# mmaker/c-lwe-snarks

Hardware: AMD Instinct MI355X
Metric: snark_proofs_per_sec (higher is better)
Workload: dtype u32 limbs (704-bit integers mod 2^704) + AES-256 bytes; int8 digits on the matrix cores, int32 accumulation (exact)

## Files before the change

c-lwe-snarks_amd/__init__.py:

```python
from __future__ import annotations

import ctypes
import os
from dataclasses import dataclass

import numpy as np

_HERE = os.path.dirname(os.path.abspath(__file__))
LIB_PATH = os.environ.get("MFHIP_LIB") or os.path.join(_HERE, "libmfhip.so")
P = 0xFFFFFFFB


class MfhError(RuntimeError):
    pass


@dataclass(frozen=True)
class Params:

    n: int = 1470
    logq: int = 736
    d: int = 1 << 15
    m: int = 21845

    @property
    def L(self):
        return (self.logq + 63) // 64

    @property
    def K(self):
        return self.logq // 64

    @property
    def lanes(self):
        return (64 * self.K + 55) // 56

    @property
    def ctb(self):
        return self.logq // 8

    @property
    def ctr_ct(self):
        return self.ctb * self.n

    @property
    def ctr_s(self):
        return 0

    @property
    def ctr_as(self):
        return self.ctr_ct * self.d

    @property
    def ctr_bt(self):
        return 2 * self.ctr_ct * self.d

    @property
    def ctr_bv(self):
        return 2 * self.ctr_ct * self.d + self.ctr_ct

    @property
    def ct_limbs(self):
        return (self.n + 1) * self.L


DEBUG = Params(d=256, m=64)
DEFAULT = Params()


class _CParams(ctypes.Structure):
    _fields_ = [("n", ctypes.c_uint32), ("logq", ctypes.c_uint32), ("d", ctypes.c_uint32), ("m", ctypes.c_uint32)]


_lib = None

EXPORTS = [
    "mfh_ctx_create", "mfh_ctx_destroy", "mfh_set_stream", "mfh_sync", "mfh_scrub_staging", "mfh_last_error", "mfh_set_seed",
    "mfh_keystream", "mfh_sample_rows", "mfh_ct_add", "mfh_ct_mul_ui", "mfh_ct_addmul_ui", "mfh_eval_rows",
    "mfh_encrypt_rows", "mfh_decrypt", "mfh_ct_smudge", "mfh_ssp_upload", "mfh_witness_poly", "mfh_version",
    "mfh_workspace_bytes", "mfh_last_kernel_ms", "mfh_set_timing", "mfh_set_overlap", "mfh_eval_rows_multi", "mfh_prove_batch", "mfh_crs_mm_image_bytes", "mfh_crs_expand_mm", "mfh_crs_set_resident_mm", "mfh_witness_poly_multi", "mfh_witness_poly_mm", "mfh_poly_h_multi", "mfh_poly_mul", "mfh_poly_add", "mfh_poly_prepare_t",
    "mfh_ssp_prepare", "mfh_poly_h", "mfh_setup_messages", "mfh_setup", "mfh_setup_image", "mfh_crs_image_set_b", "mfh_prove",
    "mfh_prove_partial", "mfh_prove_finish", "mfh_ct_to_lanes", "mfh_ct_from_lanes", "mfh_lanes_per_value", "mfh_digest128", "mfh_timing_drain", "mfh_timing_busy_ms", "mfh_timing_work_rows", "mfh_set_batch_image", "mfh_set_batch_slabs", "mfh_set_expand_path", "mfh_set_encrypt_path", "mfh_set_batch_launch", "mfh_set_batch_bw", "mfh_set_mm_chunk_rows", "mfh_set_mm_pack", "mfh_set_poly_exact", "mfh_poly_exact_fallbacks", "mfh_poly_exact_points", "mfh_set_poly_exact_points", "mfh_set_mm_stream", "mfh_add_dotp", "mfh_set_encrypt_chunks", "mfh_set_witness_per", "mfh_set_eval_path", "mfh_set_decrypt_path", "mfh_decrypt_rows",
    "mfh_crs_mm_share_bytes", "mfh_crs_expand_mm_share", "mfh_crs_set_resident_mm_share", "mfh_batch_chain", "mfh_batch_witness_cols", "mfh_batch_chain_from_w", "mfh_witness_poly_mm_cols", "mfh_prove_batch_partial", "mfh_prove_batch_finish",
    "mfh_resident_row_bytes", "mfh_crs_expand", "mfh_eval_rows_resident", "mfh_crs_set_resident",
    "mfh_witness_lanes", "mfh_witness_from_lanes", "mfh_prove_partial_w", "mfh_verify",
    "mfh_ssp_set_prg", "mfh_ssp_prg_make_t", "mfh_ssp_prg_fill",
    "mfh_resident_share_rows", "mfh_crs_expand_share", "mfh_crs_set_resident_share", "mfh_crs_set_resident_prefix",
    "mfh_prove_batch_supergroup", "mfh_prove_batch_stream_wait", "mfh_set_mm_width",
    "mfh_setup_public", "mfh_prove_public", "mfh_prove_batch_public", "mfh_vk_derive", "mfh_verify_public",
    "mfh_ssp_from_rows", "mfh_ssp_set_rows", "mfh_ssp_rows_fill", "mfh_ssp_rows_violations", "mfh_circuit_create", "mfh_circuit_destroy", "mfh_circuit_assign",
    "mfh_circuit_create_global", "mfh_circuit_create_ex", "mfh_circuit_create_out", "mfh_circuit_create_sum",
    "mfh_merkle_create", "mfh_merkle_destroy", "mfh_merkle_set_leaves", "mfh_merkle_root", "mfh_merkle_nodes", "mfh_merkle_paths",
    "mfh_sha256_records", "mfh_merkle_set_records", "mfh_merkle_update_rows",
]


def load_library():
    global _lib
    if _lib is not None:
        return _lib
    if not os.path.exists(LIB_PATH):
        raise MfhError(f"{LIB_PATH} is missing: run `python -c 'import __graft_entry__ as g; g.build()'` "
                       "(hipcc --offload-arch=gfx950).  There is no CPU fallback.")
    lib = ctypes.CDLL(LIB_PATH)
    vp, u64, sz, i32, u32 = ctypes.c_void_p, ctypes.c_uint64, ctypes.c_size_t, ctypes.c_int, ctypes.c_uint32
    sig = {
        "mfh_ctx_create": (i32, [ctypes.POINTER(vp), i32, ctypes.POINTER(_CParams)]),
        "mfh_ctx_destroy": (None, [vp]),
        "mfh_set_stream": (i32, [vp, vp]),
        "mfh_sync": (i32, [vp]),
        "mfh_scrub_staging": (i32, [vp]),
        "mfh_last_error": (ctypes.c_char_p, [vp]),
        "mfh_set_seed": (i32, [vp, ctypes.c_char_p]),
        "mfh_keystream": (i32, [vp, u64, vp, sz]),
        "mfh_sample_rows": (i32, [vp, u64, sz, vp]),
        "mfh_ct_add": (i32, [vp, vp, vp, vp, sz]),
        "mfh_ct_mul_ui": (i32, [vp, vp, vp, u32, sz]),
        "mfh_ct_addmul_ui": (i32, [vp, vp, vp, u32, sz]),
        "mfh_eval_rows": (i32, [vp, u64, sz, vp, vp, vp, vp, vp, i32]),
        "mfh_encrypt_rows": (i32, [vp, u64, sz, vp, vp, vp, vp]),
        "mfh_decrypt": (i32, [vp, vp, vp, sz, vp]),
        "mfh_ct_smudge": (i32, [vp, vp, sz, ctypes.c_char_p, sz, ctypes.c_char_p]),
        "mfh_ssp_upload": (i32, [vp, vp, vp, sz, sz]),
        "mfh_witness_poly": (i32, [vp, vp, ctypes.c_char_p, u32, vp]),
        "mfh_version": (ctypes.c_char_p, []),
        "mfh_workspace_bytes": (sz, [vp]),
        "mfh_last_kernel_ms": (ctypes.c_float, [vp, ctypes.c_char_p]),
        "mfh_set_timing": (i32, [vp, i32]),
        "mfh_set_overlap": (i32, [vp, i32]),
        "mfh_eval_rows_multi": (i32, [vp, u64, sz, vp, vp, u32, u32, vp, i32]),
        "mfh_poly_h_multi": (i32, [vp, vp, vp, u32]),
        "mfh_witness_poly_mm": (i32, [vp, vp, u32, ctypes.c_char_p, sz, vp, vp]),
        "mfh_witness_poly_multi": (i32, [vp, vp, u32, ctypes.c_char_p, sz, vp, vp]),
        "mfh_crs_mm_image_bytes": (sz, [vp]),
        "mfh_crs_expand_mm": (i32, [vp, vp, vp]),
        "mfh_crs_set_resident_mm": (i32, [vp, vp]),
        "mfh_prove_batch": (i32, [vp, vp, vp, u32, ctypes.c_char_p, sz, vp, ctypes.c_char_p, sz, ctypes.c_char_p, vp]),
        "mfh_prove_batch_supergroup": (u32, [vp]),
        "mfh_set_mm_width": (i32, [vp, u32, i32]),
        "mfh_prove_batch_stream_wait": (i32, [vp, u32, vp]),
        "mfh_poly_mul": (i32, [vp, vp, sz, vp, sz, vp]),
        "mfh_poly_add": (i32, [vp, vp, vp, sz, vp]),
        "mfh_poly_prepare_t": (i32, [vp, vp]),
        "mfh_ssp_prepare": (i32, [vp, vp]),
        "mfh_poly_h": (i32, [vp, vp, vp]),
        "mfh_setup_messages": (i32, [vp, vp, u32, u32, u32, vp]),
        "mfh_setup": (i32, [vp, vp, u32, u32, u32, vp, vp, vp]),
        "mfh_setup_image": (i32, [vp, vp, u32, u32, u32, vp, vp, vp, vp]),
        "mfh_prove": (i32, [vp, vp, vp, ctypes.c_char_p, u32, ctypes.c_char_p, sz, ctypes.c_char_p, vp]),
        "mfh_prove_partial": (i32, [vp, vp, vp, ctypes.c_char_p, u32, u32, u32, vp]),
        "mfh_prove_finish": (i32, [vp, vp, ctypes.c_char_p, sz, ctypes.c_char_p]),
        "mfh_lanes_per_value": (u32, [vp]),
        "mfh_digest128": (i32, [vp, vp, sz, vp]),
        "mfh_ct_to_lanes": (i32, [vp, vp, sz, vp]),
        "mfh_ct_from_lanes": (i32, [vp, vp, sz, vp]),
        "mfh_add_dotp": (i32, [vp, vp, vp, vp, sz]),
        "mfh_crs_set_resident_prefix": (i32, [vp, vp, sz]),
        "mfh_resident_share_rows": (sz, [vp, u32, u32]),
        "mfh_crs_expand_share": (i32, [vp, vp, u32, u32, vp]),
        "mfh_crs_set_resident_share": (i32, [vp, vp, u32, u32]),
        "mfh_ssp_set_prg": (i32, [vp, u64, vp]),
        "mfh_ssp_prg_make_t": (i32, [vp, u64, ctypes.c_char_p, vp]),
        "mfh_ssp_prg_fill": (i32, [vp, u64, sz, sz, vp]),
        "mfh_verify": (i32, [vp, vp, u32, u32, u32, vp, vp, sz, vp]),
        "mfh_witness_lanes": (i32, [vp, vp, ctypes.c_char_p, u32, u32, vp]),
        "mfh_witness_from_lanes": (i32, [vp, vp, vp, u32, vp]),
        "mfh_prove_partial_w": (i32, [vp, vp, vp, ctypes.c_char_p, u32, u32, u32, vp, vp]),
        "mfh_resident_row_bytes": (sz, [vp]),
        "mfh_crs_expand": (i32, [vp, u64, sz, vp, vp]),
        "mfh_crs_image_set_b": (i32, [vp, sz, sz, vp, vp]),
        "mfh_eval_rows_resident": (i32, [vp, vp, sz, sz, vp, vp, vp, vp, i32]),
        "mfh_crs_set_resident": (i32, [vp, vp]),
        "mfh_timing_drain": (i32, [vp, ctypes.c_char_p, ctypes.POINTER(u64), ctypes.POINTER(ctypes.c_double), ctypes.POINTER(u64),
                                   ctypes.POINTER(ctypes.c_float)]),
        "mfh_timing_busy_ms": (ctypes.c_double, [vp]),
        "mfh_timing_work_rows": (u64, [vp]),
        "mfh_set_batch_image": (i32, [vp, i32]),
        "mfh_set_mm_chunk_rows": (i32, [vp, u32]),
        "mfh_set_mm_pack": (i32, [vp, i32]),
        "mfh_set_poly_exact": (i32, [vp, i32]),
        "mfh_poly_exact_fallbacks": (ctypes.c_long, [vp]),
        "mfh_poly_exact_points": (i32, [vp, ctypes.POINTER(u32)]),
        "mfh_set_poly_exact_points": (i32, [vp, ctypes.POINTER(u32)]),
        "mfh_set_mm_stream": (i32, [vp, i32, i32, i32, u32]),
        "mfh_set_batch_launch": (i32, [vp, u32, i32]),
        "mfh_set_batch_bw": (i32, [vp, i32]),
        "mfh_set_encrypt_path": (i32, [vp, i32]),
        "mfh_set_expand_path": (i32, [vp, i32]),
        "mfh_set_batch_slabs": (i32, [vp, u32]),
        "mfh_set_encrypt_chunks": (i32, [vp, u32]),
        "mfh_set_eval_path": (i32, [vp, i32]),
        "mfh_set_decrypt_path": (i32, [vp, i32]),
        "mfh_decrypt_rows": (i32, [vp, u64, sz, vp, vp, vp]),
        "mfh_set_witness_per": (i32, [vp, u32]),
        "mfh_crs_mm_share_bytes": (sz, [vp, u32, u32]),
        "mfh_crs_expand_mm_share": (i32, [vp, vp, u32, u32, vp]),
        "mfh_crs_set_resident_mm_share": (i32, [vp, vp, u32, u32]),
        "mfh_batch_chain": (i32, [vp, vp, u32, ctypes.c_char_p, sz, vp, vp, vp, vp]),
        "mfh_batch_witness_cols": (i32, [vp, vp, u32, ctypes.c_char_p, sz, vp, u32, u32, vp, sz]),
        "mfh_batch_chain_from_w": (i32, [vp, vp, u32, vp, vp, vp]),
        "mfh_witness_poly_mm_cols": (i32, [vp, vp, u32, ctypes.c_char_p, sz, vp, u32, u32, vp, sz]),
        "mfh_prove_batch_partial": (i32, [vp, vp, u32, u32, u32, ctypes.c_char_p, sz, vp, vp, vp, sz, vp]),
        "mfh_prove_batch_finish": (i32, [vp, vp, u32, vp, ctypes.c_char_p, sz, ctypes.c_char_p, vp]),
        "mfh_setup_public": (i32, [vp, vp, u32, u32, u32, u32, vp, vp, vp, vp]),
        "mfh_prove_public": (i32, [vp, vp, vp, u32, ctypes.c_char_p, u32, ctypes.c_char_p, sz, ctypes.c_char_p, vp]),
        "mfh_prove_batch_public": (i32, [vp, vp, vp, u32, u32, ctypes.c_char_p, sz, vp, ctypes.c_char_p, sz, ctypes.c_char_p, vp]),
        "mfh_vk_derive": (i32, [vp, vp, u32, u32, vp]),
        "mfh_verify_public": (i32, [vp, vp, u32, u32, u32, vp, vp, ctypes.c_char_p, sz, sz, vp]),
        "mfh_ssp_from_rows": (i32, [vp, u32, vp, vp, vp, vp]),
        "mfh_ssp_set_rows": (i32, [vp, u32, vp, vp, vp, u32]),
        "mfh_ssp_rows_fill": (i32, [vp, sz, sz, vp]),
        "mfh_ssp_rows_violations": (i32, [vp, u32, vp, sz, vp, vp]),
        "mfh_circuit_create": (i32, [vp, u32, u32, vp, u32, vp, ctypes.POINTER(vp)]),
        "mfh_circuit_create_global": (i32, [vp, u32, u32, vp, u32, vp, ctypes.POINTER(vp)]),
        "mfh_circuit_create_ex": (i32, [vp, u32, u32, vp, u32, vp, u32, vp, u32, ctypes.POINTER(vp)]),
        "mfh_circuit_create_out": (i32, [vp, u32, u32, vp, u32, vp, u32, vp, u32, vp, u32, ctypes.POINTER(vp)]),
        "mfh_circuit_create_sum": (i32, [vp, u32, u32, vp, u32, vp, u32, vp, u32, vp, u32, vp, u32, ctypes.POINTER(vp)]),
        "mfh_circuit_destroy": (None, [vp]),
        "mfh_circuit_assign": (i32, [vp, vp, u32, vp, sz, vp, sz, vp]),
        "mfh_merkle_create": (i32, [vp, u32, ctypes.POINTER(vp)]),
        "mfh_merkle_destroy": (None, [vp]),
        "mfh_merkle_set_leaves": (i32, [vp, vp, u32, u32, vp]),
        "mfh_merkle_root": (i32, [vp, vp, vp]),
        "mfh_merkle_nodes": (i32, [vp, u32, ctypes.POINTER(vp)]),
        "mfh_merkle_paths": (i32, [vp, vp, u32, vp, vp, sz]),
        "mfh_sha256_records": (i32, [vp, vp, sz, u32, u32, vp]),
        "mfh_merkle_set_records": (i32, [vp, vp, u32, u32, vp, sz, u32]),
        "mfh_merkle_update_rows": (i32, [vp, vp, u32, vp, vp, vp, sz, vp]),
    }
    for name, (res, args) in sig.items():
        fn = getattr(lib, name)
        fn.restype = res
        fn.argtypes = args
    _lib = lib
    return lib


def rows_to_csr(rows):
    if isinstance(rows, tuple) and len(rows) == 3 and all(isinstance(a, np.ndarray) for a in rows):
        row_ptr, wire, coef = rows
    else:
        lens = [len(r) for r in rows]
        row_ptr = np.zeros(len(lens) + 1, dtype=np.int64)
        np.cumsum(lens, out=row_ptr[1:])
        flat = [(int(w), int(a) % P) for r in rows for (w, a) in r]
        wire = np.array([w for w, _ in flat], dtype=np.int64)
        coef = np.array([a for _, a in flat], dtype=np.int64)
    if len(row_ptr) == 0 or min(np.min(row_ptr), np.min(wire, initial=0), np.min(coef, initial=0)) < 0:
        raise MfhError("rows: row_ptr needs nrows + 1 entries, and no entry may be negative")
    if max(np.max(row_ptr), np.max(wire, initial=0), np.max(coef, initial=0)) > 0xFFFFFFFF:
        raise MfhError("rows: entries must fit 32 bits")
    return tuple(np.ascontiguousarray(a, dtype=np.uint32) for a in (row_ptr, wire, coef))


def _ptr(t):
    return ctypes.c_void_p(t.data_ptr()) if t is not None else ctypes.c_void_p(0)


CIRCUIT_MAX_WIRES = 32767
CIRCUIT_GLOBAL = 1


class CircuitProgram:

    def __init__(self, ctx, nin, ngates, handle, state="lds", extended=False, outputs=0, sums=False):
        self._ctx, self.nin, self.ngates, self._h, self.state, self.extended, self.outputs = ctx, nin, ngates, handle, state, extended, outputs
        self.sums = sums

    def close(self):
        if self._h:
            self._ctx.lib.mfh_circuit_destroy(self._h)
            self._h = ctypes.c_void_p()

    def __del__(self):
        try:
            self.close()
        except Exception:
            pass


class _DeviceBytes:

    def __init__(self, ptr, n, owner):
        self.owner = owner
        self.__cuda_array_interface__ = {"shape": (n, 32), "typestr": "|u1", "data": (ptr, False), "version": 2, "strides": None}


def _records(ctx, records, who):
    if isinstance(records, ctx.torch.Tensor):
        t = records
        if t.dtype != ctx.torch.uint8 or t.device != ctx.device or t.dim() != 2:
            raise MfhError(f"{who}: a device tensor of records is uint8 [n, length] on the context's device")
        n, length = int(t.shape[0]), int(t.shape[1])
        if (length > 1 and t.stride(1) != 1) or (n > 1 and t.stride(0) < length):
            raise MfhError(f"{who}: a device tensor of records has stride(1) == 1 and stride(0) >= length")
        return t, (int(t.stride(0)) if n > 1 else length), length, n, False
    a = np.asarray(records)
    if a.dtype != np.uint8 or a.ndim != 2:
        raise MfhError(f"{who}: records are a uint8 array [n, length]")
    n, length = a.shape
    return ctx.to_device(a).reshape(n, length), length, length, n, True


class MerkleTree:

    def __init__(self, ctx, depth, handle):
        self._ctx, self.depth, self._h = ctx, depth, handle
        self.nin = 256 + 256 * (depth + 1) + depth
        self._keep = []

    def close(self):
        if self._h:
            self._ctx.lib.mfh_merkle_destroy(self._h)
            self._h = ctypes.c_void_p()
            self._keep = []

    def __del__(self):
        try:
            self.close()
        except Exception:
            pass

    def set_leaves(self, first, leaves):
        c = self._ctx
        if isinstance(leaves, c.torch.Tensor):
            t = leaves
            if t.dtype != c.torch.uint8 or t.device != c.device or not t.is_contiguous():
                raise MfhError("set_leaves: a device tensor of leaves is contiguous uint8 on the context's device")
        else:
            a = np.frombuffer(leaves, dtype=np.uint8) if isinstance(leaves, (bytes, bytearray, memoryview)) else np.asarray(leaves)
            if a.dtype != np.uint8:
                raise MfhError("set_leaves: leaves are bytes or uint8")
            t = c.to_device(a)
            self._keep.append(t)
        if t.numel() % 32:
            raise MfhError("set_leaves: leaves are 32 bytes each")
        c._chk(c.lib.mfh_merkle_set_leaves(c._h, self._h, int(first), t.numel() // 32, _ptr(t)))

    def set_records(self, first, records):
        c = self._ctx
        t, stride, length, n, host = _records(c, records, "set_records")
        if host:
            self._keep.append(t)
        c._chk(c.lib.mfh_merkle_set_records(c._h, self._h, int(first), n, _ptr(t), stride, length))

    def root(self):
        out = (ctypes.c_uint8 * 32)()
        self._ctx._chk(self._ctx.lib.mfh_merkle_root(self._ctx._h, self._h, out))
        self._keep = []
        return bytes(out)

    def nodes(self, level):
        p = ctypes.c_void_p()
        self._ctx._chk(self._ctx.lib.mfh_merkle_nodes(self._h, int(level), ctypes.byref(p)))
# ... 15 lines not shown
        if isinstance(records, np.ndarray):
            rec = records
        else:
            rec = [np.frombuffer(bytes(r), dtype=np.uint8) for r in records]
            if len({len(r) for r in rec}) > 1:
                raise MfhError("record_rows: the records are of one length")
            rec = np.stack(rec) if rec else np.zeros((0, 0), dtype=np.uint8)
        if rec.dtype != np.uint8 or rec.ndim != 2 or len(rec) != len(paths):
            raise MfhError("record_rows: records are uint8 [nb, length], one per index")
        return np.concatenate([np.zeros((len(paths), 32), dtype=np.uint8), rec, paths[:, 64:]], axis=1)

    def record_bits(self, records, indices):
        rows = self.record_rows(records, indices)
        length = rows.shape[1] - 32 - 32 * self.depth - (self.depth + 7) // 8
        return np.unpackbits(rows, axis=1, bitorder="little")[:, : 256 + 8 * length + 257 * self.depth]

    def path_bits(self, indices):
        return np.unpackbits(self.path_rows(indices), axis=1, bitorder="little")[:, : self.nin]

    def update_rows(self, indices, new_leaves, roots=False):
        c = self._ctx
        idx = np.ascontiguousarray(indices, dtype=np.int64).reshape(-1)
        if len(idx) and (idx.min() < 0 or idx.max() > 0xFFFFFFFF):
            raise MfhError("update_rows: indices are in [0, 2^depth)")
        idx = idx.astype(np.uint32)
        if isinstance(new_leaves, c.torch.Tensor):
            t = new_leaves
            if t.dtype != c.torch.uint8 or t.device != c.device or not t.is_contiguous():
                raise MfhError("update_rows: a device tensor of leaves is contiguous uint8 on the context's device")
            if t.data_ptr() & 15:
                t = t.clone()
        else:
            a = np.frombuffer(new_leaves, dtype=np.uint8) if isinstance(new_leaves, (bytes, bytearray, memoryview)) else np.asarray(new_leaves)
            if a.dtype != np.uint8:
                raise MfhError("update_rows: leaves are bytes or uint8")
            t = c.to_device(a)
        if t.numel() != 32 * len(idx):
            raise MfhError("update_rows: one leaf of 32 bytes per index")
        rows = np.zeros((len(idx), 128 + 32 * self.depth + (self.depth + 7) // 8), dtype=np.uint8)
        r = np.zeros((len(idx) + 1, 32), dtype=np.uint8) if roots else None
        c._chk(c.lib.mfh_merkle_update_rows(c._h, self._h, len(idx), ctypes.c_void_p(idx.ctypes.data), _ptr(t) if len(idx) else None,
                                            ctypes.c_void_p(rows.ctypes.data), rows.shape[1], ctypes.c_void_p(r.ctypes.data) if roots else None))
        self._keep = []
        if roots and not len(idx):
            r[0] = np.frombuffer(self.root(), dtype=np.uint8)
        return (rows, r) if roots else rows

    def update_bits(self, indices, new_leaves, roots=False):
        out = self.update_rows(indices, new_leaves, roots)
        bits = np.unpackbits(out[0] if roots else out, axis=1, bitorder="little")[:, : 1024 + 257 * self.depth]
        return (bits, out[1]) if roots else bits


class Context:

    def __init__(self, params: Params = DEFAULT, device: int = 0, own_stream: bool = False):
        import torch

        if not torch.cuda.is_available():
            raise MfhError("no HIP device visible: the MI355X path has no CPU fallback")
        self.torch = torch
        self.lib = load_library()
        self.params = params
        self.device = torch.device("cuda", device)
        self._h = ctypes.c_void_p()
        cp = _CParams(params.n, params.logq, params.d, params.m)
        rc = self.lib.mfh_ctx_create(ctypes.byref(self._h), device, ctypes.byref(cp))
        if rc != 0:
            raise MfhError(f"mfh_ctx_create failed ({rc})")
        if not own_stream:
            self.set_stream(torch.cuda.current_stream(self.device))

    def close(self):
        if self._h:
            self.lib.mfh_ctx_destroy(self._h)
            self._h = ctypes.c_void_p()

    def __del__(self):
        try:
            self.close()
        except Exception:
            pass

    def _chk(self, rc):
        if rc != 0:
            raise MfhError(f"libmfhip error {rc}: {self.lib.mfh_last_error(self._h).decode()}")

    def empty(self, nbytes):
        return self.torch.empty(int(nbytes), dtype=self.torch.uint8, device=self.device)

    def zeros(self, nbytes):
        return self.torch.zeros(int(nbytes), dtype=self.torch.uint8, device=self.device)

    def to_device(self, arr):
        a = np.ascontiguousarray(arr)
        if not a.flags.writeable:
            import warnings

            with warnings.catch_warnings():
                warnings.simplefilter("ignore", UserWarning)
                return self.torch.from_numpy(a.view(np.uint8).reshape(-1)).to(self.device)
        return self.torch.from_numpy(a.view(np.uint8).reshape(-1)).to(self.device)

    def to_host(self, t, dtype=np.uint8):
        return t.cpu().numpy().view(dtype)

    def sync(self):
        self._chk(self.lib.mfh_sync(self._h))

    def set_stream(self, stream):
        self._chk(self.lib.mfh_set_stream(self._h, ctypes.c_void_p(stream.cuda_stream if stream is not None else 0)))

    def scrub_staging(self):
        rc = self.lib.mfh_scrub_staging(self._h)
        self._chk(rc)
        return rc

    def workspace_bytes(self):
        return int(self.lib.mfh_workspace_bytes(self._h))

    def set_timing(self, on=True):
        self._chk(self.lib.mfh_set_timing(self._h, 1 if on else 0))

    def set_overlap(self, mode=1):
        self._chk(self.lib.mfh_set_overlap(self._h, int(mode)))

    def set_batch_image(self, on=True):
        self._chk(self.lib.mfh_set_batch_image(self._h, 1 if on else 0))

    def set_batch_slabs(self, nslabs=0):
        self._chk(self.lib.mfh_set_batch_slabs(self._h, int(nslabs)))

    def set_expand_path(self, path=0):
        self._chk(self.lib.mfh_set_expand_path(self._h, int(path)))

    def set_encrypt_path(self, path=0):
        self._chk(self.lib.mfh_set_encrypt_path(self._h, int(path)))

    def set_eval_path(self, path=0):
        self._chk(self.lib.mfh_set_eval_path(self._h, int(path)))

    def set_encrypt_chunks(self, chunks=0):
        self._chk(self.lib.mfh_set_encrypt_chunks(self._h, int(chunks)))

    def set_witness_per(self, statements=0):
        self._chk(self.lib.mfh_set_witness_per(self._h, int(statements)))

    def set_batch_launch(self, groups_per_launch=4, merge_regions=True):
        self._chk(self.lib.mfh_set_batch_launch(self._h, int(groups_per_launch), 1 if merge_regions else 0))

    def set_batch_bw(self, merged=True):
        self._chk(self.lib.mfh_set_batch_bw(self._h, 1 if merged else 0))

    def set_mm_stream(self, map=0, persistent=False, sync_mode=0, spin_max=64):
        self._chk(self.lib.mfh_set_mm_stream(self._h, int(map), int(persistent), int(sync_mode), int(spin_max)))

    def set_mm_width(self, per_xcd=32, early_chain=False):
        self._chk(self.lib.mfh_set_mm_width(self._h, int(per_xcd), 1 if early_chain else 0))

    def set_mm_pack(self, on=True):
        self._chk(self.lib.mfh_set_mm_pack(self._h, 1 if on else 0))

    def set_poly_exact(self, mode=1):
        self._chk(self.lib.mfh_set_poly_exact(self._h, int(mode)))

    def poly_exact_fallbacks(self):
        return int(self.lib.mfh_poly_exact_fallbacks(self._h))

    def exact_points(self):
        out = (ctypes.c_uint32 * 4)()
        self._chk(self.lib.mfh_poly_exact_points(self._h, out))
        return [int(x) for x in out]

    def set_exact_points(self, pts):
        if pts is None:
            self._chk(self.lib.mfh_set_poly_exact_points(self._h, None))
            return
        pts = [int(x) for x in pts]
        if len(pts) != 4 or not all(0 <= x < 2**32 for x in pts):
            raise MfhError(f"set_exact_points: four uint32 values, got {pts!r}")
        self._chk(self.lib.mfh_set_poly_exact_points(self._h, (ctypes.c_uint32 * 4)(*pts)))

    def set_mm_chunk_rows(self, rows=0):
        self._chk(self.lib.mfh_set_mm_chunk_rows(self._h, int(rows)))

    def timing_drain(self, which):
        n, rows, ms, last = ctypes.c_uint64(), ctypes.c_uint64(), ctypes.c_double(), ctypes.c_float()
        self._chk(self.lib.mfh_timing_drain(self._h, which.encode(), ctypes.byref(n), ctypes.byref(ms), ctypes.byref(rows), ctypes.byref(last)))
        return n.value, ms.value, rows.value

    def timing_busy_ms(self):
        return float(self.lib.mfh_timing_busy_ms(self._h))

    def timing_work_rows(self):
        return int(self.lib.mfh_timing_work_rows(self._h))

    def last_kernel_ms(self, which):
        return float(self.lib.mfh_last_kernel_ms(self._h, which.encode()))

    def set_seed(self, seed: bytes):
        assert len(seed) == 40
        self._chk(self.lib.mfh_set_seed(self._h, bytes(seed)))

    def keystream(self, off, nbytes, out=None):
        out = self.empty(nbytes) if out is None else out
        self._chk(self.lib.mfh_keystream(self._h, off, _ptr(out), nbytes))
        return out

    def sample_rows(self, off, nrows):
        p = self.params
        out = self.empty(nrows * p.n * p.L * 8)
        self._chk(self.lib.mfh_sample_rows(self._h, off, nrows, _ptr(out)))
        return out

    def ct_add(self, a, b, count=1, out=None):
        out = self.empty(a.numel()) if out is None else out
        self._chk(self.lib.mfh_ct_add(self._h, _ptr(out), _ptr(a), _ptr(b), count))
        return out

    def ct_mul_ui(self, a, x, count=1, out=None):
        out = self.empty(a.numel()) if out is None else out
        self._chk(self.lib.mfh_ct_mul_ui(self._h, _ptr(out), _ptr(a), x, count))
        return out

    def ct_addmul_ui(self, rop, a, x, count=1):
        self._chk(self.lib.mfh_ct_addmul_ui(self._h, _ptr(rop), _ptr(a), x, count))
        return rop

    def eval_rows(self, off, nrows, c8, coeff0, coeff1=None, rop0=None, rop1=None, accumulate=False):
        p = self.params
        if rop0 is None:
            rop0 = self.empty(p.ct_limbs * 8)
        if coeff1 is not None and rop1 is None:
            rop1 = self.empty(p.ct_limbs * 8)
        self._chk(self.lib.mfh_eval_rows(self._h, off, nrows, _ptr(c8), _ptr(coeff0), _ptr(coeff1), _ptr(rop0), _ptr(rop1),
                                         1 if accumulate else 0))
        return rop0, rop1

    def eval_rows_multi(self, off, nrows, c8, coeffs, nvec, out=None, accumulate=False, coeff_bytes=4):
        out = self.empty(nvec * self.params.ct_limbs * 8) if out is None else out
        self._chk(self.lib.mfh_eval_rows_multi(self._h, off, nrows, _ptr(c8), _ptr(coeffs), nvec, coeff_bytes, _ptr(out), 1 if accumulate else 0))
        return out

    def encrypt_rows(self, off, nrows, sk, msg, err, out=None):
        p = self.params
        out = self.empty(nrows * p.ctb) if out is None else out
        self._chk(self.lib.mfh_encrypt_rows(self._h, off, nrows, _ptr(sk), _ptr(msg), _ptr(err), _ptr(out)))
        return out

    def decrypt(self, sk, cts, count, out=None):
        out = self.empty(4 * count) if out is None else out
        self._chk(self.lib.mfh_decrypt(self._h, _ptr(sk), _ptr(cts), count, _ptr(out)))
        return out

    def set_decrypt_path(self, path=0):
        self._chk(self.lib.mfh_set_decrypt_path(self._h, int(path)))

    def decrypt_rows(self, off, nrows, sk, c8, out=None):
        out = self.empty(4 * nrows) if out is None else out
        self._chk(self.lib.mfh_decrypt_rows(self._h, off, nrows, _ptr(sk), _ptr(c8), _ptr(out)))
        return out

    def ct_smudge(self, cts, count, mag: bytes, maglen, sign: bytes):
        self._chk(self.lib.mfh_ct_smudge(self._h, _ptr(cts), count, bytes(mag), maglen, bytes(sign)))
        return cts

    def ssp_upload(self, ssp_host_u64: np.ndarray, d_ssp=None, first_slot=0, nslots=None):
        p = self.params
        nslots = p.m + 3 if nslots is None else nslots
        if d_ssp is None:
            d_ssp = self.empty((p.m + 3) * p.d * 4)
        a = np.ascontiguousarray(ssp_host_u64)
        self._chk(self.lib.mfh_ssp_upload(self._h, ctypes.c_void_p(a.ctypes.data), _ptr(d_ssp), first_slot, nslots))
        return d_ssp

    def ssp_from_rows(self, rows, d_ssp=None):
        p = self.params
        row_ptr, wire, coef = rows_to_csr(rows)
        if d_ssp is None:
            d_ssp = self.empty((p.m + 3) * p.d * 4)
        self._chk(self.lib.mfh_ssp_from_rows(self._h, len(row_ptr) - 1, ctypes.c_void_p(row_ptr.ctypes.data), ctypes.c_void_p(wire.ctypes.data),
                                             ctypes.c_void_p(coef.ctypes.data), _ptr(d_ssp)))
        return d_ssp

    def ssp_set_rows(self, rows, lu_max=0):
        if rows is None:
            self._chk(self.lib.mfh_ssp_set_rows(self._h, 0, None, None, None, 0))
            return
        row_ptr, wire, coef = rows_to_csr(rows)
        self._chk(self.lib.mfh_ssp_set_rows(self._h, len(row_ptr) - 1, ctypes.c_void_p(row_ptr.ctypes.data), ctypes.c_void_p(wire.ctypes.data),
                                            ctypes.c_void_p(coef.ctypes.data), int(lu_max)))

    def ssp_rows_fill(self, first_slot, nslots):
        out = self.empty(max(nslots, 1) * self.params.d * 4)
        self._chk(self.lib.mfh_ssp_rows_fill(self._h, first_slot, nslots, _ptr(out)))
        return out

    def ssp_rows_violations(self, witness_bits_list):
        nb = len(witness_bits_list)
        count, first = np.zeros(nb, dtype=np.uint32), np.full(nb, 0xFFFFFFFF, dtype=np.uint32)
        bits, stride = self._pack_bits(witness_bits_list)
        self._chk(self.lib.mfh_ssp_rows_violations(self._h, nb, bits if nb else None, stride, ctypes.c_void_p(count.ctypes.data), ctypes.c_void_p(first.ctypes.data)))
        return count, first

    def circuit_load(self, compiled, state="lds"):
        if state not in ("lds", "global", "auto"):
            raise MfhError(f"circuit_load: state must be 'lds', 'global' or 'auto', got {state!r}")
        gates = np.ascontiguousarray(compiled.gates, dtype=np.uint32).reshape(-1, 3)
        asserts = np.ascontiguousarray(compiled.asserts, dtype=np.uint32).reshape(-1, 2)
        program = np.ascontiguousarray(getattr(compiled, "program", np.zeros((0, 4))), dtype=np.uint32).reshape(-1, 4)
        equal = np.ascontiguousarray(getattr(compiled, "equal", np.zeros((0, 2))), dtype=np.uint32).reshape(-1, 2)
        outputs = np.ascontiguousarray(getattr(compiled, "outputs", np.zeros((0, 2))), dtype=np.uint32).reshape(-1, 2)
        terms = np.ascontiguousarray(getattr(compiled, "terms", np.zeros((0, 2))), dtype=np.uint32).reshape(-1, 2)
        sums = bool((program[:, 0] == 8).any())
        extended = len(equal) > 0 or len(outputs) > 0 or bool((program[:, 0] > 3).any())
        nin = compiled.nwires - len(gates)
        if state == "auto":
            state = "lds" if compiled.nwires <= CIRCUIT_MAX_WIRES else "global"
        h = ctypes.c_void_p()

        def arr(x):
            return ctypes.c_void_p(x.ctypes.data)

        flags = CIRCUIT_GLOBAL if state == "global" else 0
        ex = [self._h, nin, len(program), arr(program), len(asserts), arr(asserts), len(equal), arr(equal)]
        if sums:
            self._chk(self.lib.mfh_circuit_create_sum(*ex, len(outputs), arr(outputs), len(terms), arr(terms), flags, ctypes.byref(h)))
        elif len(outputs):
            self._chk(self.lib.mfh_circuit_create_out(*ex, len(outputs), arr(outputs), flags, ctypes.byref(h)))
        elif extended:
            self._chk(self.lib.mfh_circuit_create_ex(*ex, flags, ctypes.byref(h)))
        else:
            create = self.lib.mfh_circuit_create if state == "lds" else self.lib.mfh_circuit_create_global
            self._chk(create(self._h, nin, len(gates), arr(gates), len(asserts), arr(asserts), ctypes.byref(h)))
        return CircuitProgram(self, nin, len(gates), h, state, extended, len(outputs), sums)

    def circuit_assign(self, prog, bits):
        bits = np.asarray(bits, dtype=np.uint8)
        if bits.ndim != 2 or bits.shape[1] != prog.nin:
            raise MfhError(f"circuit_assign: bits must be [nb, {prog.nin}] (public then private bits), got {bits.shape}")
        nb = bits.shape[0]
        packed = np.ascontiguousarray(np.packbits(bits & 1, axis=1, bitorder="little"))
        stride = (self.params.m + 7) // 8
        witness = np.zeros((nb, stride), dtype=np.uint8)
        holds = np.zeros(nb, dtype=np.uint8)
        self._chk(self.lib.mfh_circuit_assign(self._h, prog._h, nb, ctypes.c_void_p(packed.ctypes.data), packed.shape[1], ctypes.c_void_p(witness.ctypes.data),
                                              stride, ctypes.c_void_p(holds.ctypes.data)))
        return witness, holds.astype(bool)

    def sha256_records(self, records):
        t, stride, length, n, host = _records(self, records, "sha256_records")
        out = self.torch.empty((n, 32), dtype=self.torch.uint8, device=self.device)
        self._chk(self.lib.mfh_sha256_records(self._h, _ptr(t), stride, length, n, _ptr(out)))
        if host:
            self.sync()
        return out

    def merkle_tree(self, depth):
        h = ctypes.c_void_p()
        self._chk(self.lib.mfh_merkle_create(self._h, int(depth), ctypes.byref(h)))
        return MerkleTree(self, int(depth), h)

    def ssp_to_host_u64(self, d_ssp):
        p = self.params
        return self.to_host(d_ssp[: (p.m + 3) * p.d * 4], np.uint32).astype(np.uint64)

    def witness_poly(self, d_ssp, witness_bits: bytes, delta):
        out = self.empty(self.params.d * 4)
        self._chk(self.lib.mfh_witness_poly(self._h, _ptr(d_ssp), bytes(witness_bits), delta, _ptr(out)))
        return out

    def poly_mul(self, a, la, b, lb):
        out = self.empty((la + lb - 1) * 4)
        self._chk(self.lib.mfh_poly_mul(self._h, _ptr(a), la, _ptr(b), lb, _ptr(out)))
        return out

    def poly_add(self, a, b, count):
        out = self.empty(count * 4)
        self._chk(self.lib.mfh_poly_add(self._h, _ptr(a), _ptr(b), count, _ptr(out)))
        return out

    def ssp_prepare(self, d_ssp):
        self._chk(self.lib.mfh_ssp_prepare(self._h, _ptr(d_ssp)))

    def poly_prepare_t(self, d_t):
        self._chk(self.lib.mfh_poly_prepare_t(self._h, _ptr(d_t)))

    def poly_h(self, d_v):
        out = self.empty(self.params.d * 4)
        self._chk(self.lib.mfh_poly_h(self._h, _ptr(d_v), _ptr(out)))
        return out

    def poly_h_many(self, d_v, nb):
        out = self.empty(nb * self.params.d * 4)
        self._chk(self.lib.mfh_poly_h_multi(self._h, _ptr(d_v), _ptr(out), nb))
        return out

    def setup_messages(self, d_ssp, alpha, beta, s):
        p = self.params
        out = self.empty((2 * p.d + p.m) * 4)
        self._chk(self.lib.mfh_setup_messages(self._h, _ptr(d_ssp), alpha, beta, s, _ptr(out)))
        return out

    def setup(self, d_ssp, alpha, beta, s, d_sk, d_err, out=None):
        p = self.params
        out = self.empty((2 * p.d + p.m) * p.ctb) if out is None else out
        self._chk(self.lib.mfh_setup(self._h, _ptr(d_ssp), alpha, beta, s, _ptr(d_sk), _ptr(d_err), _ptr(out)))
        return out

    def setup_image(self, d_ssp, alpha, beta, s, d_sk, d_err, out=None, rows=None):
        p = self.params
        out = self.empty((2 * p.d + p.m) * p.ctb) if out is None else out
        rows = self.empty((2 * p.d + p.m) * self.resident_row_bytes()) if rows is None else rows
        self._chk(self.lib.mfh_setup_image(self._h, _ptr(d_ssp), alpha, beta, s, _ptr(d_sk), _ptr(d_err), _ptr(out), _ptr(rows)))
        return out, rows

    def prove(self, d_crs, d_ssp, witness_bits: bytes, delta, smudge_mag: bytes, smudge_sign: bytes, maglen=80, out=None):
        p = self.params
        out = self.empty(5 * p.ct_limbs * 8) if out is None else out
        assert len(smudge_mag) == 5 * maglen and len(smudge_sign) == 5
        self._chk(self.lib.mfh_prove(self._h, _ptr(d_crs), _ptr(d_ssp), bytes(witness_bits), delta, bytes(smudge_mag), maglen,
                                     bytes(smudge_sign), _ptr(out)))
        return out

    def crs_expand_mm(self, d_crs, out=None):
        out = self.empty(int(self.lib.mfh_crs_mm_image_bytes(self._h))) if out is None else out
        self._chk(self.lib.mfh_crs_expand_mm(self._h, _ptr(d_crs), _ptr(out)))
        return out

    def set_resident_mm(self, image):
        self._resident_mm = image
        self._chk(self.lib.mfh_crs_set_resident_mm(self._h, _ptr(image)))

    def witness_poly_many(self, d_ssp, witness_bits_list, deltas, mm=True):
        p = self.params
        nb = len(witness_bits_list)
        stride = (p.m + 6) // 8
        bits = b"".join(bytes(w[:stride]).ljust(stride, b"\0") for w in witness_bits_list)
        dl = (ctypes.c_uint32 * nb)(*[int(x) for x in deltas])
        out = self.empty(nb * p.d * 4)
        fn = self.lib.mfh_witness_poly_mm if mm else self.lib.mfh_witness_poly_multi
        self._chk(fn(self._h, _ptr(d_ssp), nb, bits, stride, ctypes.cast(dl, ctypes.c_void_p), _ptr(out)))
        return out

    def prove_batch(self, d_crs, d_ssp, witness_bits_list, deltas, smudge_mags, smudge_signs, maglen=80, out=None):
        p = self.params
        nb = len(witness_bits_list)
        stride = (p.m + 6) // 8
        bits = b"".join(bytes(w[:stride]).ljust(stride, b"\0") for w in witness_bits_list)
        dl = (ctypes.c_uint32 * nb)(*[int(x) for x in deltas])
        mags = b"".join(bytes(x) for x in smudge_mags)
        signs = b"".join(bytes(x) for x in smudge_signs)
        assert len(mags) == nb * 5 * maglen and len(signs) == nb * 5
        out = self.empty(nb * 5 * p.ct_limbs * 8) if out is None else out
        self._chk(self.lib.mfh_prove_batch(self._h, _ptr(d_crs), _ptr(d_ssp), nb, bits, stride, ctypes.cast(dl, ctypes.c_void_p), mags, maglen,
                                           signs, _ptr(out)))
        return out

    def prove_batch_supergroup(self):
        return int(self.lib.mfh_prove_batch_supergroup(self._h))

    def prove_batch_stream_wait(self, upto, stream):
        self._chk(self.lib.mfh_prove_batch_stream_wait(self._h, int(upto), ctypes.c_void_p(stream.cuda_stream)))

    def _pack_bits(self, witness_bits_list):
        stride = (self.params.m + 6) // 8
        return b"".join(bytes(w[:stride]).ljust(stride, b"\0") for w in witness_bits_list), stride

    def crs_expand_mm_share(self, d_crs, rank, world, out=None):
        out = self.empty(int(self.lib.mfh_crs_mm_share_bytes(self._h, rank, world))) if out is None else out
        self._chk(self.lib.mfh_crs_expand_mm_share(self._h, _ptr(d_crs), rank, world, _ptr(out)))
        return out

    def set_resident_mm_share(self, image, rank, world):
        self._resident_mm = image
        self._chk(self.lib.mfh_crs_set_resident_mm_share(self._h, _ptr(image), rank, world))

    def batch_chain(self, d_ssp, witness_bits_list, deltas, out=None):
        p = self.params
        nb = len(witness_bits_list)
        out = self.torch.empty((3, nb, p.d), dtype=self.torch.int32, device=self.device) if out is None else out
        if nb == 0:
            return out
        bits, stride = self._pack_bits(witness_bits_list)
        dl = (ctypes.c_uint32 * nb)(*[int(x) for x in deltas])
        self._chk(self.lib.mfh_batch_chain(self._h, _ptr(d_ssp), nb, bits, stride, ctypes.cast(dl, ctypes.c_void_p), _ptr(out[0]), _ptr(out[1]), _ptr(out[2])))
        return out

    def batch_witness_cols(self, d_ssp, witness_bits_list, deltas, col0, ncols, out=None):
        nb = len(witness_bits_list)
        out = self.torch.empty((nb, ncols), dtype=self.torch.int32, device=self.device) if out is None else out
        if nb == 0 or ncols == 0:
            return out
        bits, stride = self._pack_bits(witness_bits_list)
        dl = (ctypes.c_uint32 * nb)(*[int(x) for x in deltas])
        self._chk(self.lib.mfh_batch_witness_cols(self._h, _ptr(d_ssp), nb, bits, stride, ctypes.cast(dl, ctypes.c_void_p), int(col0), int(ncols), _ptr(out), int(ncols)))
        return out

    def batch_chain_from_w(self, d_ssp, whv):
        n = whv.shape[1]
        if n:
            self._chk(self.lib.mfh_batch_chain_from_w(self._h, _ptr(d_ssp), n, _ptr(whv[0]), _ptr(whv[1]), _ptr(whv[2])))
        return whv

    def prove_batch_partial(self, d_crs, rank, world, witness_bits_list, d_w, d_h, d_v, coef_stride, out=None):
        p = self.params
        nb = len(witness_bits_list)
        need = nb * 5 * p.ct_limbs * 8
        out = self.empty(need) if out is None else out
        if out.numel() * out.element_size() < need:
            raise MfhError(f"prove_batch_partial: `out` holds {out.numel() * out.element_size()} bytes, {nb} statements need {need}")
        bits, stride = self._pack_bits(witness_bits_list)
        self._chk(self.lib.mfh_prove_batch_partial(self._h, _ptr(d_crs), rank, world, nb, bits, stride, _ptr(d_w), _ptr(d_h), _ptr(d_v), int(coef_stride),
                                                   _ptr(out)))
        return out

    def prove_batch_finish(self, d_crs, deltas, smudge_mags, smudge_signs, d_proofs, maglen=80):
        nb = len(deltas)
        if nb == 0:
            return d_proofs
        dl = (ctypes.c_uint32 * nb)(*[int(x) for x in deltas])
        mags = b"".join(bytes(x) for x in smudge_mags)
        signs = b"".join(bytes(x) for x in smudge_signs)
        assert len(mags) == nb * 5 * maglen and len(signs) == nb * 5
        self._chk(self.lib.mfh_prove_batch_finish(self._h, _ptr(d_crs), nb, ctypes.cast(dl, ctypes.c_void_p), mags, maglen, signs, _ptr(d_proofs)))
        return d_proofs

    def prove_partial(self, d_crs, d_ssp, witness_bits: bytes, delta, rank, world, out=None):
        p = self.params
        out = self.empty(5 * p.ct_limbs * 8) if out is None else out
        self._chk(self.lib.mfh_prove_partial(self._h, _ptr(d_crs), _ptr(d_ssp), bytes(witness_bits), delta, rank, world, _ptr(out)))
        return out

    def prove_finish(self, d_proof, smudge_mag: bytes, smudge_sign: bytes, maglen=80):
        self._chk(self.lib.mfh_prove_finish(self._h, _ptr(d_proof), bytes(smudge_mag), maglen, bytes(smudge_sign)))
        return d_proof

    def digest128(self, d_buf, nbytes=None):
        h = (ctypes.c_uint64 * 2)()
        n = d_buf.numel() * d_buf.element_size() if nbytes is None else int(nbytes)
        self._chk(self.lib.mfh_digest128(self._h, _ptr(d_buf), n, ctypes.cast(h, ctypes.c_void_p)))
        return int(h[0]), int(h[1])

    def ct_to_lanes(self, d_cts, count, out=None):
        p = self.params
        out = self.torch.empty(count * (p.n + 1) * p.lanes, dtype=self.torch.int64, device=self.device) if out is None else out
        self._chk(self.lib.mfh_ct_to_lanes(self._h, _ptr(d_cts), count, _ptr(out)))
        return out

    def ct_from_lanes(self, d_lanes, count, out=None):
        p = self.params
        out = self.empty(count * p.ct_limbs * 8) if out is None else out
        self._chk(self.lib.mfh_ct_from_lanes(self._h, _ptr(d_lanes), count, _ptr(out)))
        return out

    def add_dotp(self, rop, a, b, length):
        self._chk(self.lib.mfh_add_dotp(self._h, _ptr(rop), _ptr(a), _ptr(b), length))
        return rop

    def resident_row_bytes(self):
        return int(self.lib.mfh_resident_row_bytes(self._h))

    def crs_expand(self, off, nrows, c8, out=None):
        out = self.empty(nrows * self.resident_row_bytes()) if out is None else out
        self._chk(self.lib.mfh_crs_expand(self._h, off, nrows, _ptr(c8), _ptr(out)))
        return out

    def crs_image_set_b(self, image, first_row, nrows, c8):
        self._chk(self.lib.mfh_crs_image_set_b(self._h, int(first_row), int(nrows), _ptr(c8), _ptr(image)))
        return image

    def eval_rows_resident(self, rows, first_row, nrows, coeff0, coeff1=None, rop0=None, rop1=None, accumulate=False):
        p = self.params
        if rop0 is None:
            rop0 = self.empty(p.ct_limbs * 8)
        if coeff1 is not None and rop1 is None:
            rop1 = self.empty(p.ct_limbs * 8)
        self._chk(self.lib.mfh_eval_rows_resident(self._h, _ptr(rows), first_row, nrows, _ptr(coeff0), _ptr(coeff1), _ptr(rop0), _ptr(rop1),
                                                  1 if accumulate else 0))
        return rop0, rop1

    def set_resident(self, rows):
        self._resident = rows
        self._chk(self.lib.mfh_crs_set_resident(self._h, _ptr(rows)))

    def witness_lanes(self, d_ssp, witness_bits: bytes, rank, world, out=None):
        out = self.torch.empty(self.params.d, dtype=self.torch.int64, device=self.device) if out is None else out
        self._chk(self.lib.mfh_witness_lanes(self._h, _ptr(d_ssp), bytes(witness_bits), rank, world, _ptr(out)))
        return out

    def prove_partial_w(self, d_crs, d_ssp, witness_bits: bytes, delta, rank, world, wlanes, out=None):
        p = self.params
        out = self.empty(5 * p.ct_limbs * 8) if out is None else out
        self._chk(self.lib.mfh_prove_partial_w(self._h, _ptr(d_crs), _ptr(d_ssp), bytes(witness_bits), delta, rank, world, _ptr(wlanes), _ptr(out)))
        return out

    def verify(self, d_ssp, alpha, beta, s, d_sk, d_proofs, count=1):
# ... 75 lines not shown
```

c-lwe-snarks_amd/csrc/ctx.hpp:

```cpp
#pragma once
#include <hip/hip_runtime.h>

#include <stdint.h>
#include <string.h>

#include <string>
#include <vector>

#include "aes_dev.hpp"
#include "mfhip.h"
#include "ssp_prg.hpp"

#define HIP_TRY(ctx, expr)                                                        \
  do {                                                                            \
    hipError_t e_ = (expr);                                                       \
    if (e_ != hipSuccess) {                                                       \
      (ctx)->err = std::string(#expr) + ": " + hipGetErrorString(e_);             \
      return MFH_EDEVICE;                                                         \
    }                                                                             \
  } while (0)

struct PolyState;
struct SspInterp;
struct SspRows;
struct RowsTree;

struct PinBuf {
  void *p = nullptr;
  size_t cap = 0;
  hipEvent_t ev = nullptr;
  bool pending = false;
  size_t used = 0;
};

struct DevBuf {
  void *p = nullptr;
  size_t cap = 0;
  template <class T> T *as() const { return static_cast<T *>(p); }
};

struct mfh_ctx {
  mfh_params P{};
  int device = 0;
  hipStream_t own_stream = nullptr;
  hipStream_t stream = nullptr;
  mf::AesKey key{};
  bool have_seed = false;
  uint32_t *d_t0 = nullptr;
  DevBuf ws;
  DevBuf ws2;
  int mm_ws_sel = 0;
  DevBuf ws3;
  std::vector<hipEvent_t> ev_cdone, ev_rdone, ev_wdone;
  std::vector<hipEvent_t> ev_round;
  std::vector<hipEvent_t> ev_sgdone;
  uint32_t last_batch_sg = 0, last_batch_n = 0;
  DevBuf wws;
  DevBuf lazy;
  uint32_t *lazy_cnt = nullptr;
  bool eval_dense = false;
  bool overlap = true;
  int overlap_mode = 1;
  hipStream_t side = nullptr, side2 = nullptr;
  hipEvent_t ev_fork = nullptr, ev_join = nullptr;
  hipEvent_t ev_chain = nullptr, ev_chain_done = nullptr;
  std::string err;
  bool timing = false;
  struct Timed {
    hipEvent_t e0, e1;
    int kind;
    uint64_t rows;
    uint64_t work;
    int sub;
  };
  std::vector<Timed> timed;
  double last_busy_ms = 0;
  uint64_t last_work_rows = 0;
  std::vector<hipEvent_t> ev_pool;
  PolyState *poly = nullptr;
  DevBuf aux;
  DevBuf d_msg;
  DevBuf d_prover;
  std::vector<uint32_t> h_cw;
  const uint8_t *mm_image = nullptr;
  uint32_t mm_rank = 0, mm_world = 1;
  uint64_t mm_off[3] = {0, 0, 0}, mm_rows[3] = {0, 0, 0};
  size_t mm_base[3] = {0, 0, 0};
  DevBuf ssp_frag;
  const uint32_t *ssp_frag_src = nullptr;
  SspInterp *interp = nullptr;
  DevBuf circ_io;
  DevBuf circ_state;
  DevBuf d_batch;
  DevBuf batch_img;
  int batch_image = 1;
  int mm_map = 1;
  bool mm_persist = true;
  bool mm_wave1 = false;
  uint32_t mm_sync_mode = 0, mm_spin = 64;
  uint32_t mm_width = 32;
  size_t early_ws_half = 0;
  bool batch_early_chain = false;
  uint32_t *mm_sync = nullptr;
  int poly_exact = 1;
  bool poly_pts_pinned = false;
  uint32_t poly_pts[4] = {0, 0, 0, 0};
  bool mm_pack = true;
  uint32_t mm_chunk_rows = 131071;
  int expand_path = 0;
  int enc_path = 0;
  uint32_t ncu = 256;
  int dec_path = 0;
  int eval_path = 0;
  uint32_t enc_chunks = 0;
  uint32_t witness_per = 0;
  uint32_t batch_slabs = 0;
  int batch_bw_merged = 1;
  int batch_merge = 1;
  uint32_t batch_ngl = 8;
  PinBuf pin_rows, pin_cw, pin_smudge;
  PinBuf pin_pub;
  DevBuf d_pub;
  PinBuf pin_wring[8];
  uint32_t pin_wnext = 0;
  hipEvent_t ev_sample = nullptr;
  DevBuf sample_tmp;
  void *uploader = nullptr;
  bool prg_on = false;
  uint64_t prg_seed = 0;
  const uint32_t *prg_t = nullptr;
  SspRows *rows = nullptr;
  RowsTree *rows_tree = nullptr;
  const uint32_t *rows_prefix = nullptr;
  uint32_t rows_lu_max = 0;
  const uint8_t *resident_rows = nullptr;
  uint64_t resident_nrows = ~0ull;
  bool resident_sharded = false;
  uint32_t res_rank = 0, res_world = 1;
};

struct Timer {
  mfh_ctx *c;
  mfh_ctx::Timed t{};
  bool on;
  Timer(mfh_ctx *c_, int kind, uint64_t rows, uint64_t work = 0, int sub = 0) : c(c_), on(c_->timing) {
    if (!on) return;
    auto get = [&]() {
      hipEvent_t e;
      if (!c->ev_pool.empty()) { e = c->ev_pool.back(); c->ev_pool.pop_back(); }
      else hipEventCreate(&e);
      return e;
    };
    t.e0 = get(); t.e1 = get(); t.kind = kind; t.rows = rows; t.work = work ? work : rows; t.sub = sub;
    hipEventRecord(t.e0, c->stream);
  }
  ~Timer() {
    if (!on) return;
    hipEventRecord(t.e1, c->stream);
    c->timed.push_back(t);
  }
};

inline void *pin_acquire(mfh_ctx *c, PinBuf &b, size_t bytes) {
  if (b.pending) { hipEventSynchronize(b.ev); b.pending = false; }
  if (bytes > b.cap) {
    if (b.p) hipHostFree(b.p);
    b.cap = (bytes + 4095) & ~(size_t)4095;
    if (hipHostMalloc(&b.p, b.cap, hipHostMallocDefault) != hipSuccess) { b.p = nullptr; b.cap = 0; c->err = "hipHostMalloc failed"; return nullptr; }
  }
  if (!b.ev) hipEventCreateWithFlags(&b.ev, hipEventDisableTiming);
  b.used = bytes;
  return b.p;
}
inline void pin_release(mfh_ctx *c, PinBuf &b) {
  hipEventRecord(b.ev, c->stream);
  b.pending = true;
}
inline void pin_scrub(PinBuf &b) {
  if (b.pending) { hipEventSynchronize(b.ev); b.pending = false; }
  if (b.p && b.used) {
    volatile unsigned char *q = (volatile unsigned char *)b.p;
    memset((void *)q, 0, b.used);
    __asm__ __volatile__("" : : "r"(b.p) : "memory");
  }
  b.used = 0;
}
inline void pin_free(PinBuf &b) {
  if (b.pending) hipEventSynchronize(b.ev);
  if (b.p) hipHostFree(b.p);
  if (b.ev) hipEventDestroy(b.ev);
  b = PinBuf();
}

enum class DevWait { stream, device };
inline void dev_free(DevBuf &b) {
  if (b.p) hipFree(b.p);
  b = DevBuf();
}
inline bool dev_alloc(DevBuf &b, size_t bytes) {
  if (hipMalloc(&b.p, bytes) != hipSuccess) {
    b = DevBuf();
    return false;
  }
  b.cap = bytes;
  return true;
}
inline int dev_reserve(mfh_ctx *c, DevBuf &b, size_t bytes, DevWait wait = DevWait::stream, size_t gran = 1) {
  if (bytes <= b.cap) return MFH_OK;
  if (b.p) {
    if (wait == DevWait::device) hipDeviceSynchronize();
    else hipStreamSynchronize(c->stream);
    dev_free(b);
  }
  if (!dev_alloc(b, (bytes + gran - 1) & ~(gran - 1))) {
    c->err = "hipMalloc(device scratch) failed";
    return MFH_ENOMEM;
  }
  return MFH_OK;
}
inline int batch_img_drop(mfh_ctx *c) {
  if (!c->batch_img.p) return MFH_OK;
  const hipError_t e = hipDeviceSynchronize();
  dev_free(c->batch_img);
  if (e != hipSuccess) {
    c->err = std::string("hipDeviceSynchronize(): ") + hipGetErrorString(e);
    return MFH_EDEVICE;
  }
  return MFH_OK;
}
inline int work_reserve(mfh_ctx *c, DevBuf &b, size_t bytes) { return dev_reserve(c, b, bytes, DevWait::stream, (size_t)1 << 20); }
inline int lazy_reserve(mfh_ctx *c, size_t bytes) {
  if (bytes + 256 <= c->lazy.cap || !bytes) return MFH_OK;
  bytes = ((bytes + 255) & ~(size_t)255) + 256;
  if (int rc = dev_reserve(c, c->lazy, bytes)) return rc;
  if (hipMemsetAsync(c->lazy.p, 0, bytes, c->stream) != hipSuccess) return MFH_EDEVICE;
  c->lazy_cnt = reinterpret_cast<uint32_t *>(c->lazy.as<uint8_t>() + bytes - 256);
  return MFH_OK;
}
inline int ws_reserve(mfh_ctx *c, size_t bytes) { return work_reserve(c, c->ws, bytes); }
inline int wws_reserve(mfh_ctx *c, size_t bytes) { return work_reserve(c, c->wws, bytes); }
inline int ws2_reserve(mfh_ctx *c, size_t bytes) { return work_reserve(c, c->ws2, bytes); }
inline int aux_reserve(mfh_ctx *c, size_t bytes) { return dev_reserve(c, c->aux, bytes); }

inline int ssp_src(mfh_ctx *c, const uint32_t *d_ssp, mf::SspSrc &src, bool rows_ok = false) {
  if (d_ssp) { src = mf::SspSrc{d_ssp, d_ssp, 0}; return MFH_OK; }
  if (c->rows_prefix) {
    if (!rows_ok) { c->err = "this entry point does not take the row SSP (mfh_ssp_set_rows): pass a dense d_ssp"; return MFH_EUNSUPPORTED; }
    src = mf::SspSrc{c->rows_prefix, c->rows_prefix, 0, c->rows_lu_max + 2};
    return MFH_OK;
  }
  if (!c->prg_on || !c->prg_t) { c->err = "d_ssp is NULL and no generator-defined SSP is registered (mfh_ssp_set_prg)"; return MFH_EINVAL; }
  src = mf::SspSrc{nullptr, c->prg_t, c->prg_seed};
  return MFH_OK;
}

void mfh_poly_destroy(mfh_ctx *c);
void ssp_interp_free(mfh_ctx *c);
void ssp_rows_free(mfh_ctx *c, bool tree);
int ssp_rows_check(mfh_ctx *c, const char *who, uint32_t nrows, const uint32_t *h_row_ptr, const uint32_t *h_wire, const uint32_t *h_coef);
int ssp_rows_tree(mfh_ctx *c, const char *who, const uint32_t *&d_t, const uint32_t *&h_w);
int ssp_rows_witness(mfh_ctx *c, uint32_t nstmt, const uint8_t *h_bits, size_t bits_stride, const uint32_t *h_delta, uint32_t *d_w, size_t w_stride);
int ssp_rows_msg_evals(mfh_ctx *c, uint32_t s, uint32_t beta, uint32_t *d_msg_evals);
inline bool ssp_is_rows(const mfh_ctx *c, const uint32_t *d_ssp) { return !d_ssp && c->rows_prefix; }
inline int ssp_rows_lu_check(mfh_ctx *c, const uint32_t *d_ssp, uint32_t lu) {
  if (ssp_is_rows(c, d_ssp) && lu > c->rows_lu_max) { c->err = "lu exceeds the lu_max the row SSP was registered with (mfh_ssp_set_rows)"; return MFH_EINVAL; }
  return MFH_OK;
}
extern "C" int mfh_witness_poly_mm(mfh_ctx *c, const uint32_t *d_ssp, uint32_t nstmt, const uint8_t *h_bits, size_t bits_stride, const uint32_t *h_delta,
                                   uint32_t *d_w);
extern "C" int mfh_witness_poly_mm_cols(mfh_ctx *c, const uint32_t *d_ssp, uint32_t nstmt, const uint8_t *h_bits, size_t bits_stride, const uint32_t *h_delta,
                                        uint32_t col0, uint32_t ncols, uint32_t *d_w, size_t w_stride);
extern "C" int mfh_poly_h_multi(mfh_ctx *c, const uint32_t *d_v, uint32_t *d_h, uint32_t nb);
int expand_mm_region(mfh_ctx *c, uint64_t off, uint32_t nrows, const uint8_t *c8, uint8_t *image);
int encrypt_rows_mm(mfh_ctx *c, uint64_t off, size_t nrows, const uint64_t *sk, const uint32_t *msg, const uint64_t *err, uint8_t *c8);
int decrypt_mm(mfh_ctx *c, const uint64_t *sk, const uint64_t *cts, size_t count, uint32_t *out);
int decrypt_rows_mm(mfh_ctx *c, uint64_t off, size_t nrows, const uint64_t *sk, const uint8_t *c8, uint32_t *out);

struct MmIo {
  const uint32_t *coef[2];
  uint32_t csplit;
  uint64_t *out[2];
  uint32_t osplit;
  uint64_t ostride;
  const uint8_t *bits;
  uint32_t bits_stride;
  int64_t *sc_zeroed;
  uint64_t cstride;
  uint32_t bits_row0;
  const uint64_t *add_ct;
  const uint32_t *add_scale;
  uint32_t sa_from1;
};
int eval_rows_multi_io(mfh_ctx *c, uint64_t off, size_t nrows, const uint8_t *d_c8, const MmIo &io, uint32_t nvec, uint32_t coeff_bytes, int accumulate);
int eval_rows_multi_io_set(mfh_ctx *c, uint64_t off, size_t nrows, const uint8_t *d_c8, const MmIo *ios, const uint32_t *nvecs, uint32_t ng,
                           uint32_t coeff_bytes);
struct MmRegion { uint64_t off; const uint8_t *c8; };
int eval_rows_multi_io_regions(mfh_ctx *c, const MmRegion *regs, uint32_t nreg, size_t nrows, const MmIo *ios, const uint32_t *nvecs, uint32_t ng,
                               uint32_t coeff_bytes, int accumulate);
bool mm_image_covers(const mfh_ctx *c, uint64_t off, size_t nrows);
struct MmsPlan {
  uint32_t ng, ngt, ND, nrows, nchunks, rpc, rpad, ntiles, mtiles;
  size_t cd_bytes, part_bytes;
  const uint8_t *img[2];
  int8_t *cd;
  int *part;
};
bool mms_plan(mfh_ctx *c, const MmRegion *regs, uint32_t nreg, size_t nrows, const MmIo *ios, const uint32_t *nvecs, uint32_t ng, uint32_t coeff_bytes,
              MmsPlan &P);
size_t mms_ws_bytes(const MmsPlan &P);
void mms_bind(MmsPlan &P, void *ws);
int mms_digits(mfh_ctx *c, const MmsPlan &P, const MmIo *ios, const uint32_t *nvecs);
int mms_stream(mfh_ctx *c, const MmsPlan &P);
int mms_finish(mfh_ctx *c, const MmsPlan &P, const MmIo *ios, const uint32_t *nvecs, int accumulate);
```

c-lwe-snarks_amd/csrc/mfhip.hip:

```cpp
#include <hip/hip_runtime.h>

#include <stdint.h>
#include <stdio.h>
#include <string.h>

#include <algorithm>
#include <string>
#include <thread>
#include <vector>

#include "aes_dev.hpp"
#include "mfhip.h"

using mf::AesKey;

template <int LOGQ>
struct PS {
  static constexpr int CTB = LOGQ / 8;
  static constexpr int EW = CTB / 4;
  static constexpr int L = (LOGQ + 63) / 64;
  static constexpr int K = LOGQ / 64;
  static constexpr int KW = 2 * K;
  static constexpr int TILE = LOGQ == 736 ? 512 : 256;
  static constexpr int ROWS = 2;
// ... 806 lines not shown
__global__ void k_ssp_reduce(const uint64_t *__restrict__ in, uint32_t *__restrict__ out, uint64_t ncoef) {
  for (uint64_t i = (uint64_t)blockIdx.x * blockDim.x + threadIdx.x; i < ncoef; i += (uint64_t)gridDim.x * blockDim.x)
    out[i] = (uint32_t)(in[i] % MFH_P);
}

extern "C" {

const char *mfh_version(void) { return "mfhip 0.1 (gfx950)"; }

int mfh_ctx_create(mfh_ctx **out, int device, const mfh_params *P) {
  if (!out || !P) return MFH_EINVAL;
  *out = nullptr;
  if (P->logq != 736 && P->logq != 1472) return MFH_EUNSUPPORTED;
  if (P->n == 0 || P->n > (1u << 20)) return MFH_EINVAL;
  int ndev = 0;
  if (hipGetDeviceCount(&ndev) != hipSuccess || ndev <= 0 || device < 0 || device >= ndev) return MFH_EDEVICE;
  if (hipSetDevice(device) != hipSuccess) return MFH_EDEVICE;
  mfh_ctx *c = new mfh_ctx();
  c->P = *P;
  c->device = device;
  {
    int ncu = 0;
    if (hipDeviceGetAttribute(&ncu, hipDeviceAttributeMultiprocessorCount, device) == hipSuccess && ncu > 0) c->ncu = (uint32_t)ncu;
  }
  if (hipStreamCreateWithFlags(&c->own_stream, hipStreamNonBlocking) != hipSuccess) {
    delete c;
    return MFH_EDEVICE;
  }
  c->stream = c->own_stream;
  uint32_t t0[512];
  mf::make_t0_le(t0);
  for (int a = 0; a < 256; a++) t0[256 + a] = (t0[a] << 24) | (t0[a] >> 8);
  if (hipMalloc(&c->d_t0, sizeof t0) != hipSuccess || hipMemcpy(c->d_t0, t0, sizeof t0, hipMemcpyHostToDevice) != hipSuccess) {
    mfh_ctx_destroy(c);
    return MFH_EDEVICE;
  }
  *out = c;
  return MFH_OK;
}

void mfh_ctx_destroy(mfh_ctx *c) {
  if (!c) return;
  hipSetDevice(c->device);
  if (c->stream) hipStreamSynchronize(c->stream);
  mfh_poly_destroy(c);
  ssp_interp_free(c);
  ssp_rows_free(c, true);
  upload_free(c);
  if (c->ev_sample) hipEventDestroy(c->ev_sample);
  pin_free(c->pin_rows);
  for (auto &b : c->pin_wring) pin_free(b);
  pin_free(c->pin_cw);
  pin_free(c->pin_smudge);
  pin_free(c->pin_pub);
  if (c->side) hipStreamSynchronize(c->side);
  if (c->mm_sync) hipFree(c->mm_sync);
  for (hipEvent_t e : c->ev_round) hipEventDestroy(e);
  for (hipEvent_t e : c->ev_sgdone) hipEventDestroy(e);
  for (hipEvent_t e : c->ev_cdone) hipEventDestroy(e);
  for (hipEvent_t e : c->ev_rdone) hipEventDestroy(e);
  for (hipEvent_t e : c->ev_wdone) hipEventDestroy(e);
  if (c->ev_fork) hipEventDestroy(c->ev_fork);
  if (c->ev_join) hipEventDestroy(c->ev_join);
  if (c->ev_chain) hipEventDestroy(c->ev_chain);
  if (c->ev_chain_done) hipEventDestroy(c->ev_chain_done);
  if (c->side) hipStreamDestroy(c->side);
  if (c->side2) hipStreamDestroy(c->side2);
  for (DevBuf *b : {&c->ws, &c->ws2, &c->ws3, &c->wws, &c->lazy, &c->aux, &c->d_msg, &c->d_prover, &c->d_pub, &c->d_batch, &c->batch_img, &c->circ_io,
                    &c->circ_state, &c->ssp_frag, &c->sample_tmp})
    dev_free(*b);
  if (c->d_t0) hipFree(c->d_t0);
  for (auto &t : c->timed) { hipEventDestroy(t.e0); hipEventDestroy(t.e1); }
  for (auto e : c->ev_pool) hipEventDestroy(e);
  if (c->own_stream) hipStreamDestroy(c->own_stream);
  delete c;
}

int mfh_set_stream(mfh_ctx *c, void *s) {
  if (!c) return MFH_EINVAL;
  c->stream = (hipStream_t)s;
  return MFH_OK;
}

int mfh_sync(mfh_ctx *c) {
  if (!c) return MFH_EINVAL;
  HIP_TRY(c, hipStreamSynchronize(c->stream));
  return MFH_OK;
}

int mfh_scrub_staging(mfh_ctx *c) {
  if (!c) return MFH_EINVAL;
  pin_scrub(c->pin_rows);
  pin_scrub(c->pin_cw);
  pin_scrub(c->pin_smudge);
  for (auto &b : c->pin_wring) pin_scrub(b);
  return MFH_OK;
}

const char *mfh_last_error(const mfh_ctx *c) { return c ? c->err.c_str() : "null context"; }
size_t mfh_workspace_bytes(const mfh_ctx *c) { return c ? c->ws.cap : 0; }
int mfh_set_overlap(mfh_ctx *c, int en) {
  if (!c) return MFH_EINVAL;
  c->overlap = en != 0;
  c->overlap_mode = en > 1 ? en : 1;
  return MFH_OK;
}

int mfh_set_expand_path(mfh_ctx *c, int path) {
  if (!c || path < 0 || path > 1) return MFH_EINVAL;
  c->expand_path = path;
  return MFH_OK;
}

int mfh_set_encrypt_path(mfh_ctx *c, int path) {
  if (!c || path < 0 || path > 2) return MFH_EINVAL;
  c->enc_path = path;
  return MFH_OK;
}

int mfh_set_eval_path(mfh_ctx *c, int path) {
  if (!c || path < 0 || path > 1) return MFH_EINVAL;
  c->eval_path = path;
  return MFH_OK;
}
int mfh_set_encrypt_chunks(mfh_ctx *c, uint32_t chunks) {
  if (!c || chunks > 64) return MFH_EINVAL;
  c->enc_chunks = chunks;
  return MFH_OK;
}
int mfh_set_witness_per(mfh_ctx *c, uint32_t statements) {
  if (!c || (statements && (statements < 32 || statements > 256))) return MFH_EINVAL;
  c->witness_per = statements;
  return MFH_OK;
}
int mfh_set_batch_slabs(mfh_ctx *c, uint32_t nslabs) {
  if (!c || nslabs > 256) return MFH_EINVAL;
  c->batch_slabs = nslabs;
  return MFH_OK;
}

int mfh_set_batch_launch(mfh_ctx *c, uint32_t groups_per_launch, int merge_regions) {
  if (!c || groups_per_launch < 1 || groups_per_launch > 8) return MFH_EINVAL;
  c->batch_ngl = groups_per_launch;
  c->batch_merge = merge_regions != 0;
  return MFH_OK;
}

int mfh_set_batch_bw(mfh_ctx *c, int merged) {
  if (!c) return MFH_EINVAL;
  c->batch_bw_merged = merged != 0;
  return MFH_OK;
}

int mfh_set_batch_image(mfh_ctx *c, int en) {
  if (!c) return MFH_EINVAL;
  c->batch_image = en != 0;
  return en ? MFH_OK : batch_img_drop(c);
}

int mfh_set_timing(mfh_ctx *c, int en) {
  if (!c) return MFH_EINVAL;
  c->timing = en != 0;
  return MFH_OK;
}
static int timing_kind(const char *which) {
  if (!strcmp(which, "keystream")) return 0;
  if (!strcmp(which, "eval1")) return 1;
  if (!strcmp(which, "eval2")) return 2;
  if (!strcmp(which, "encrypt")) return 3;
  if (!strcmp(which, "eval")) return 12;
  if (!strcmp(which, "expand")) return 4;
  if (!strcmp(which, "mac1")) return 5;
  if (!strcmp(which, "mac2")) return 6;
  if (!strcmp(which, "evalmm")) return 7;
  if (!strcmp(which, "evalmm_resident")) return 8;
  if (!strcmp(which, "expandmm")) return 9;
  if (!strcmp(which, "decrypt")) return 11;
  if (!strcmp(which, "decrypt_rows")) return 13;
  if (!strcmp(which, "mmstream_bw")) return 14;
  if (!strcmp(which, "mmstream_rounds")) return 10;
  if (!strcmp(which, "mmstream_rounds_persistent")) return 110;
  if (!strcmp(which, "mmstream_bw_persistent")) return 114;
  if (!strcmp(which, "ssp_interp")) return 15;
  if (!strcmp(which, "circuit_assign")) return 16;
  if (!strcmp(which, "circuit_assign_global")) return 17;
  if (!strcmp(which, "circuit_assign_ex")) return 18;
  if (!strcmp(which, "circuit_assign_global_ex")) return 19;
  if (!strcmp(which, "circuit_assign_out")) return 20;
  if (!strcmp(which, "circuit_assign_global_out")) return 21;
  if (!strcmp(which, "circuit_assign_sum")) return 22;
  if (!strcmp(which, "circuit_assign_global_sum")) return 23;
  if (!strcmp(which, "ssp_rows_violations")) return 24;
  if (!strcmp(which, "merkle_level")) return 25;
  if (!strcmp(which, "merkle_paths")) return 26;
  if (!strcmp(which, "sha256_records")) return 27;
  if (!strcmp(which, "merkle_updates")) return 28;
  return -1;
}

int mfh_timing_drain(mfh_ctx *c, const char *which, uint64_t *count, double *total_ms, uint64_t *total_rows, float *last_ms) {
  if (!c || !which) return MFH_EINVAL;
  const int kind = timing_kind(which);
  if (kind < 0) return MFH_EINVAL;
  HIP_TRY(c, hipStreamSynchronize(c->stream));
  if (c->side) HIP_TRY(c, hipStreamSynchronize(c->side));
  uint64_t n = 0, rows = 0, work = 0;
  double tot = 0;
  float last = -1.f;
  std::vector<mfh_ctx::Timed> keep;
  std::vector<std::pair<float, float>> spans;
  hipEvent_t base = nullptr;
  for (auto &t : c->timed) {
    const bool match = t.kind == kind || (kind == 12 && (t.kind == 1 || t.kind == 2)) || (kind == 8 && (t.kind == 10 || t.kind == 14)) || (kind >= 100 && t.kind == kind - 100 && t.sub == 1);
    if (!match) { keep.push_back(t); continue; }
    float ms = 0;
    if (hipEventElapsedTime(&ms, t.e0, t.e1) == hipSuccess) {
      n++; tot += ms; rows += t.rows; work += t.work; last = ms;
      if (!base) base = t.e0;
      float s0 = 0;
      if (hipEventElapsedTime(&s0, base, t.e0) == hipSuccess) spans.emplace_back(s0, s0 + ms);
    }
  }
  std::sort(spans.begin(), spans.end());
  double busy = 0;
  float hi = -1e30f;
  for (auto &sp : spans) {
    if (sp.second <= hi) continue;
    busy += sp.second - std::max(sp.first, hi);
    hi = sp.second;
  }
  c->last_busy_ms = busy;
  c->last_work_rows = work;
  for (auto &t : c->timed) {
    const bool match = t.kind == kind || (kind == 12 && (t.kind == 1 || t.kind == 2)) || (kind == 8 && (t.kind == 10 || t.kind == 14)) || (kind >= 100 && t.kind == kind - 100 && t.sub == 1);
    if (!match) continue;
    c->ev_pool.push_back(t.e0);
    c->ev_pool.push_back(t.e1);
  }
  c->timed.swap(keep);
  if (count) *count = n;
  if (total_ms) *total_ms = tot;
  if (total_rows) *total_rows = rows;
  if (last_ms) *last_ms = last;
  return MFH_OK;
}

double mfh_timing_busy_ms(const mfh_ctx *c) { return c ? c->last_busy_ms : -1.0; }
uint64_t mfh_timing_work_rows(const mfh_ctx *c) { return c ? c->last_work_rows : 0; }

float mfh_last_kernel_ms(mfh_ctx *c, const char *which) {
  float last = -1.f;
  if (mfh_timing_drain(c, which, nullptr, nullptr, nullptr, &last) != MFH_OK) return -1.f;
  return last;
}

int mfh_set_seed(mfh_ctx *c, const uint8_t seed[40]) {
  if (!c || !seed) return MFH_EINVAL;
  mf::expand_key(c->key, seed);
  c->have_seed = true;
  return MFH_OK;
}

#define NEED_SEED(c)                                  \
  do {                                                \
    if (!(c)->have_seed) {                            \
      (c)->err = "mfh_set_seed has not been called";  \
      return MFH_EINVAL;                              \
    }                                                 \
  } while (0)

#define DISPATCH_LOGQ(c, CALL736, CALL1472) \
  do {                                      \
    if ((c)->P.logq == 736) {               \
      CALL736;                              \
    } else {                                \
      CALL1472;                             \
    }                                       \
  } while (0)

int mfh_digest128(mfh_ctx *c, const void *d_buf, size_t nbytes, uint64_t h_digest[2]) {
  if (!c || (!d_buf && nbytes) || !h_digest || (reinterpret_cast<uintptr_t>(d_buf) & 3)) return MFH_EINVAL;
  HIP_TRY(c, hipSetDevice(c->device));
  int rc = aux_reserve(c, 16);
  if (rc) return rc;
  HIP_TRY(c, hipMemsetAsync(c->aux.p, 0, 16, c->stream));
  const uint64_t nwords = (nbytes + 3) / 4;
  const uint32_t grid = (uint32_t)std::min<uint64_t>(2048, (nwords + 255) / 256);
  if (grid) hipLaunchKernelGGL(k_digest128, dim3(grid), dim3(256), 0, c->stream, (const uint8_t *)d_buf, (uint64_t)nbytes, c->aux.as<unsigned long long>());
  HIP_TRY(c, hipGetLastError());
  HIP_TRY(c, hipMemcpyAsync(h_digest, c->aux.p, 16, hipMemcpyDeviceToHost, c->stream));
  HIP_TRY(c, hipStreamSynchronize(c->stream));
  return MFH_OK;
}

int mfh_keystream(mfh_ctx *c, uint64_t off, void *d_out, size_t nbytes) {
  if (!c || (!d_out && nbytes)) return MFH_EINVAL;
  NEED_SEED(c);
  if (!nbytes) return MFH_OK;
  HIP_TRY(c, hipSetDevice(c->device));
  uint64_t nblk = ((off & 15) + nbytes + 15) >> 4;
  uint32_t grid = (uint32_t)std::min<uint64_t>((nblk + 1023) / 1024, 256 * 2);
  {
    Timer t(c, 0, nblk);
    hipLaunchKernelGGL(k_keystream, dim3(grid), dim3(1024), 0, c->stream, c->key, c->d_t0, off, (uint8_t *)d_out, (uint64_t)nbytes);
  }
  HIP_TRY(c, hipGetLastError());
// ... 521 lines not shown
```

c-lwe-snarks_amd/csrc/snark.hip:

```cpp
#include <algorithm>
#include <cstdlib>
#include <cstring>
#include <vector>

#include "ctx.hpp"
#include "p32.hpp"

namespace {

__device__ __forceinline__ uint32_t ssp_coef(const mf::SspSrc &src, uint32_t slot, uint32_t rowkey, uint32_t d, uint32_t k) {
  if (src.dense) return src.dense[(uint64_t)slot * d + k];
  return slot == 0 ? src.t[k] : mf::ssp_prg_coeff(rowkey, k);
}

__global__ void k_powers(uint32_t s, uint32_t d, uint32_t *__restrict__ pw) {
  uint32_t k = blockIdx.x * blockDim.x + threadIdx.x;
  if (k >= d) return;
  uint32_t r = 1, b = s, e = k;
  while (e) {
    if (e & 1) r = mulp(r, b);
    b = mulp(b, b);
    e >>= 1;
  }
  pw[k] = r;
// ... 772 lines not shown
    }
    for (uint32_t r = 0; r < R; r++) {
      rc = mms_stream(c, plan[r]);
      if (rc) return rc;
      if (early) {
        while (c->ev_round.size() <= r) {
          hipEvent_t e;
          HIP_TRY(c, hipEventCreateWithFlags(&e, hipEventDisableTiming));
          c->ev_round.push_back(e);
        }
        HIP_TRY(c, hipEventRecord(c->ev_round[r], main_stream));
        HIP_TRY(c, hipStreamWaitEvent(side_stream, c->ev_round[r], 0));
        OnStream side(c, side_stream);
        rc = mms_finish(c, plan[r], io[r], nv[r], accumulate);
        if (rc) return rc;
        continue;
      }
      rc = mms_finish(c, plan[r], io[r], nv[r], accumulate);
      if (rc) return rc;
    }
    if (early) {
      *tail_on_side = true;
      return MFH_OK;
    }
  } else {
    for (uint32_t g0 = 0; g0 < sg; g0 += NGL * BG) {
      MmIo io[2 * NGLMAX];
      uint32_t nv[2 * NGLMAX], ng = 0;
      for (uint32_t k = 0; k < NGL && g0 + k * BG < sg; k++) ng++;
      for (uint32_t k = 0; k < ng; k++) {
        const uint32_t gg = g0 + k * BG, g = std::min(BG, sg - gg);
        uint64_t *proofs = sproofs + (size_t)gg * 5 * ctl;
        const uint64_t o = (uint64_t)gg * co.stride;
        io[k] = MmIo{{co.w + o, co.h + o}, g, {proofs + 3 * ctl, proofs}, g, pstride, nullptr, 0, B.SCZ + 256 * slot++, co.stride, 0};
        io[ng + k] = MmIo{{co.h + o, co.v + o}, g, {proofs + ctl, proofs + 2 * ctl}, g, pstride, nullptr, 0, B.SCZ + 256 * slot++, co.stride, 0};
        nv[k] = nv[ng + k] = 2 * g;
      }
      rc = eval_rows_multi_io_regions(c, regs, 1, cS, io, nv, ng, 4, accumulate);
      if (rc) return rc;
      {
        OnSide side(c, side_stream);
        rc = eval_rows_multi_io_regions(c, regs + 1, 1, cS, io + ng, nv + ng, ng, 4, accumulate);
        if (rc) return rc;
      }
    }
  }
  HIP_TRY(c, hipEventRecord(c->ev_join, side_stream));
  HIP_TRY(c, hipStreamWaitEvent(main_stream, c->ev_join, 0));
  return MFH_OK;
}

int batch_smudge(mfh_ctx *c, uint64_t *sproofs, uint32_t sg, const uint8_t *h_smudge_mag, size_t maglen, const uint8_t *h_smudge_sign) {
  std::vector<uint8_t> mags((size_t)sg * 5 * maglen), signs((size_t)sg * 5);
  for (int pass = 0; pass < 2; pass++) {
    std::fill(mags.begin(), mags.end(), 0);
    std::fill(signs.begin(), signs.end(), 0);
    for (uint32_t b = 0; b < sg; b++) {
      const uint8_t *pm = h_smudge_mag + (size_t)b * 5 * maglen, *ps = h_smudge_sign + (size_t)b * 5;
      if (pass == 0) {
        memcpy(&mags[(size_t)b * 5 * maglen], pm, 4 * maglen);
        memcpy(&signs[(size_t)b * 5], ps, 4);
      } else {
        memcpy(&mags[((size_t)b * 5 + 3) * maglen], pm + 4 * maglen, maglen);
        signs[(size_t)b * 5 + 3] = ps[4];
      }
    }
    int rc = mfh_ct_smudge(c, sproofs, (size_t)sg * 5, mags.data(), maglen, signs.data());
    if (rc) return rc;
  }
  return MFH_OK;
}

int batch_ct_t(mfh_ctx *c, const uint8_t *d_crs_c8, const BatchScratch &B) {
  const uint32_t d = c->P.d, ctb = c->P.logq / 8;
  HIP_TRY(c, hipMemsetD32Async((hipDeviceptr_t)B.ONE, 1, 1, c->stream));
  return mfh_eval_rows(c, (uint64_t)ctb * c->P.n * 2 * d, 1, d_crs_c8 + (size_t)2 * d * ctb, B.ONE, nullptr, B.CT_T, nullptr, 0);
}

struct ImageGuard {
  mfh_ctx *c;
  bool on;
  ~ImageGuard() { if (on) mfh_crs_set_resident_mm(c, nullptr); }
};
int batch_transient_image(mfh_ctx *c, const uint8_t *d_crs_c8, uint32_t nproofs, uint32_t rank, uint32_t world, ImageGuard &guard) {
  const uint32_t ctb = c->P.logq / 8;
  if (c->mm_image || !c->batch_image || nproofs <= BG || (((uint64_t)c->P.n * ctb) & 7)) return MFH_OK;
  const size_t ib = mfh_crs_mm_share_bytes(c, rank, world);
  if (c->batch_img.cap < ib) {
    (void)batch_img_drop(c);
    size_t mem_free = 0, mem_total = 0;
    if (hipMemGetInfo(&mem_free, &mem_total) != hipSuccess) mem_free = 0;
    if (ib > mem_free / 4 * 3 || !dev_alloc(c->batch_img, ib)) (void)hipGetLastError();
  }
  if (!c->batch_img.p) return MFH_OK;
  int rc = mfh_crs_expand_mm_share(c, d_crs_c8, rank, world, c->batch_img.as<uint8_t>());
  if (rc) return rc;
  mfh_crs_set_resident_mm_share(c, c->batch_img.as<uint8_t>(), rank, world);
  guard.on = true;
  return MFH_OK;
}

int prove_batch_impl(mfh_ctx *c, const uint8_t *d_crs_c8, const uint32_t *d_ssp, uint32_t nproofs, const uint8_t *h_witness_bits,
                     size_t bits_stride, const uint32_t *h_delta, const uint8_t *h_smudge_mag, size_t maglen, const uint8_t *h_smudge_sign,
                     uint64_t *d_proofs, const PubBatch *pub) {
  if (!c) return MFH_EINVAL;
  if (!nproofs) return MFH_OK;
  if (!d_crs_c8 || !h_witness_bits || !h_delta || !h_smudge_mag || !h_smudge_sign || !d_proofs) return MFH_EINVAL;
  if (c->resident_rows) { c->err = "mfh_prove_batch regenerates the keystream: clear the resident CRS image first"; return MFH_EUNSUPPORTED; }
  if (c->mm_image && c->mm_world != 1) { c->err = "mfh_prove_batch: the registered matrix-core image holds one rank's row shares (use mfh_prove_batch_partial)"; return MFH_EINVAL; }
  mf::SspSrc src;
  {
    int rc0 = ssp_src(c, d_ssp, src, true);
    if (rc0) return rc0;
    if (pub && (rc0 = ssp_rows_lu_check(c, d_ssp, pub->lu))) return rc0;
  }
  const uint32_t d = c->P.d, m = c->P.m, n = c->P.n;
  if (bits_stride < (m + 6) / 8) { c->err = "bits_stride shorter than the m - 1 witness bits"; return MFH_EINVAL; }
  for (uint32_t b = 0; b < nproofs; b++)
    if (h_delta[b] >= P32) { c->err = "delta must be < p"; return MFH_EINVAL; }
  if (maglen + 4 > (size_t)(c->P.logq / 64) * 8) { c->err = "smudge magnitude too wide"; return MFH_EINVAL; }
  const size_t ctl = (size_t)(n + 1) * ((c->P.logq + 63) / 64);
  HIP_TRY(c, hipSetDevice(c->device));
  const bool will_stream = c->mm_image || (c->batch_image && nproofs > BG && (((uint64_t)n * (c->P.logq / 8)) & 7) == 0);
  const uint32_t SG = will_stream ? BSG : BSG_REGEN;
  const uint32_t nsg = (nproofs + SG - 1) / SG;
  uint32_t nsl = 1;
  const uint32_t ctb0 = c->P.logq / 8;
  const bool slabs_ok = !c->mm_image && c->batch_image && nproofs > BG && (((uint64_t)n * ctb0) & 7) == 0;
  if (slabs_ok && c->batch_slabs) nsl = std::min(c->batch_slabs, std::max(1u, std::min(d, m)));
  else if (slabs_ok) {
    size_t mem_free = 0, mem_total = 0;
    if (hipMemGetInfo(&mem_free, &mem_total) == hipSuccess) {
      const size_t ib = mfh_crs_mm_image_bytes(c), avail = mem_free + c->batch_img.cap + c->d_batch.cap;
      if (ib > avail / 4 * 3) {
        const size_t budget = std::max<size_t>(avail / 3, (size_t)1 << 30);
        nsl = (uint32_t)std::min<size_t>(256, (ib + budget - 1) / budget);
        const size_t area = (size_t)3 * BSG * d * 4, maxsg = std::max<size_t>(1, avail / 4 / area);
        if (nsg > maxsg) {
          const size_t ctl0 = (size_t)(n + 1) * ((c->P.logq + 63) / 64);
          for (uint32_t s0 = 0; s0 < nproofs; s0 += (uint32_t)maxsg * SG) {
            const uint32_t cnt = std::min<uint32_t>((uint32_t)maxsg * SG, nproofs - s0);
            const PubBatch sub = pub ? pub->at(s0) : PubBatch{};
            int r = prove_batch_impl(c, d_crs_c8, d_ssp, cnt, h_witness_bits + (size_t)s0 * bits_stride, bits_stride, h_delta + s0,
                                     h_smudge_mag + (size_t)s0 * 5 * maglen, maglen, h_smudge_sign + (size_t)s0 * 5, d_proofs + (size_t)s0 * 5 * ctl0,
                                     pub ? &sub : nullptr);
            if (r) return r;
          }
          c->last_batch_sg = 0;
          return MFH_OK;
        }
      }
    }
  }
  const uint32_t nbuf = nsl > 1 ? nsg : 2;
  while (c->ev_sgdone.size() < nsg) {
    hipEvent_t e;
    HIP_TRY(c, hipEventCreateWithFlags(&e, hipEventDisableTiming));
    c->ev_sgdone.push_back(e);
  }
  c->last_batch_sg = 0;
  BatchScratch B;
  int rc = batch_scratch(c, nproofs, nbuf, B, nsl > 1 ? 1 : nsg, nsl > 1 ? 0 : nproofs);
  if (rc) return rc;
  size_t slot = 0;
  HIP_TRY(c, hipMemsetAsync(B.SCZ, 0, B.nslots * 2048, c->stream));
  rc = batch_streams(c);
  if (rc) return rc;
  while (c->ev_cdone.size() < nbuf) {
    hipEvent_t e0, e1, e2;
    HIP_TRY(c, hipEventCreateWithFlags(&e0, hipEventDisableTiming));
    HIP_TRY(c, hipEventCreateWithFlags(&e1, hipEventDisableTiming));
    HIP_TRY(c, hipEventCreateWithFlags(&e2, hipEventDisableTiming));
    c->ev_cdone.push_back(e0);
    c->ev_rdone.push_back(e1);
    c->ev_wdone.push_back(e2);
  }
  hipStream_t const main_stream = c->stream, chain_stream = c->side2;
  auto whv_of = [&](uint32_t sgi, uint32_t *&W, uint32_t *&H, uint32_t *&V) {
    W = B.WHV + (size_t)(sgi % nbuf) * 3 * BSG * d;
    H = W + (size_t)BSG * d;
    V = H + (size_t)BSG * d;
  };
  auto launch_chain = [&](uint32_t sgi) -> int {
    const uint32_t s0 = sgi * SG, sg = std::min(SG, nproofs - s0);
    uint32_t *WALL, *HALL, *VALL;
    whv_of(sgi, WALL, HALL, VALL);
    OnStream chain(c, chain_stream);
    const PubBatch psg = pub ? pub->at(s0) : PubBatch{};
    int r = batch_chain_launch(c, src, d_ssp, sg, h_witness_bits + (size_t)s0 * bits_stride, bits_stride, h_delta + s0, WALL, HALL, VALL, c->ev_wdone[sgi % nbuf],
                               pub ? &psg : nullptr);
    if (r) return r;
    HIP_TRY(c, hipEventRecord(c->ev_cdone[sgi % nbuf], chain_stream));
    return MFH_OK;
  };
  HIP_TRY(c, hipEventRecord(c->ev_chain, main_stream));
  HIP_TRY(c, hipStreamWaitEvent(chain_stream, c->ev_chain, 0));
  rc = launch_chain(0);
  if (rc) return rc;
  if (nsl > 1) {
    for (uint32_t k = 1; k < nsg; k++) {
      rc = launch_chain(k);
      if (rc) return rc;
    }
    for (;;) {
      size_t ib = 0;
      for (uint32_t r = 0; r < nsl; r++) ib = std::max(ib, mfh_crs_mm_share_bytes(c, r, nsl));
      if (c->batch_img.cap >= ib) break;
      (void)batch_img_drop(c);
      size_t mem_free = 0, mem_total = 0;
      const bool fits = hipMemGetInfo(&mem_free, &mem_total) != hipSuccess || ib + ((size_t)8 << 30) <= mem_free;
      if (fits && dev_alloc(c->batch_img, ib)) break;
      (void)hipGetLastError();
      const uint32_t cap = std::min<uint32_t>(256u, std::max(1u, std::min(d, m)));
      if (nsl >= cap || c->batch_slabs) { c->err = "mfh_prove_batch: no room for a row slab of the CRS image"; return MFH_ENOMEM; }
      nsl = std::min(cap, nsl * 2);
    }
    rc = batch_ct_t(c, d_crs_c8, B);
    if (rc) return rc;
    ImageGuard slab{c, true};
    for (uint32_t r = 0; r < nsl; r++) {
      rc = mfh_crs_expand_mm_share(c, d_crs_c8, r, nsl, c->batch_img.as<uint8_t>());
      if (rc) return rc;
      mfh_crs_set_resident_mm_share(c, c->batch_img.as<uint8_t>(), r, nsl);
      HIP_TRY(c, hipMemsetAsync(B.SCZ, 0, B.nslots * 2048, c->stream));
      slot = 0;
      const uint32_t loS = (uint32_t)((uint64_t)d * r / nsl);
      for (uint32_t s0 = 0, sgi = 0; s0 < nproofs; s0 += SG, sgi++) {
        const uint32_t sg = std::min(SG, nproofs - s0);
        uint32_t *WALL, *HALL, *VALL;
        whv_of(sgi, WALL, HALL, VALL);
        const BatchCoef co = {WALL + loS, HALL + loS, VALL + loS, d};
        rc = batch_rows_supergroup(c, d_crs_c8, r, nsl, sg, h_witness_bits + (size_t)s0 * bits_stride, bits_stride, co, d_proofs + (size_t)s0 * 5 * ctl, B, slot,
                                   r == 0 ? h_delta + s0 : nullptr, r == 0 ? c->ev_cdone[sgi % nbuf] : nullptr, r > 0);
        if (rc) return rc;
      }
    }
    for (uint32_t s0 = 0; s0 < nproofs; s0 += SG) {
      rc = batch_smudge(c, d_proofs + (size_t)s0 * 5 * ctl, std::min(SG, nproofs - s0), h_smudge_mag + (size_t)s0 * 5 * maglen, maglen, h_smudge_sign + (size_t)s0 * 5);
      if (rc) return rc;
      HIP_TRY(c, hipEventRecord(c->ev_sgdone[s0 / SG], c->stream));
    }
    c->last_batch_sg = SG;
    c->last_batch_n = nproofs;
    return MFH_OK;
  }
  ImageGuard transient{c, false};
  rc = batch_transient_image(c, d_crs_c8, nproofs, 0, 1, transient);
  if (rc) return rc;
  rc = batch_stage_host(c, B, nproofs, h_witness_bits, bits_stride, h_delta, h_smudge_mag, maglen, h_smudge_sign, SG);
  if (rc) return rc;
  rc = batch_ct_t(c, d_crs_c8, B);
  if (rc) return rc;
  bool bw_done = false;
  if (c->batch_bw_merged && nsg > 1 && mm_image_covers(c, (uint64_t)ctb0 * n * 2 * d, m)) {
    const uint64_t ctr_ct = (uint64_t)ctb0 * n, pstride = 5 * ctl;
    const uint32_t bstride = (m + 6) / 8;
    const MmRegion reg = {ctr_ct * 2 * d, d_crs_c8 + (size_t)2 * d * ctb0};
    for (uint32_t g0 = 0; g0 < nsg; g0 += 8) {
      MmIo ios[8];
      uint32_t nvs[8];
      const uint32_t ng = std::min(8u, nsg - g0);
      for (uint32_t k = 0; k < ng; k++) {
        const uint32_t sgi = g0 + k, s0 = sgi * SG, sg = std::min(SG, nproofs - s0);
        const uint8_t *d_cw = B.CW + (size_t)sgi * B.cw_stride;
        ios[k] = MmIo{{nullptr, nullptr}, sg, {d_proofs + (size_t)s0 * 5 * ctl + 4 * ctl, nullptr}, sg, pstride, d_cw, bstride, B.SCZ + 256 * slot++};
        ios[k].add_ct = B.CT_T;
        ios[k].add_scale = (const uint32_t *)(d_cw + B.cw_delta_off);
        nvs[k] = sg;
      }
      rc = ng > 1 ? eval_rows_multi_io_regions(c, &reg, 1, m, ios, nvs, ng, 1, 0) : eval_rows_multi_io(c, reg.off, m, reg.c8, ios[0], nvs[0], 1, 0);
      if (rc) return rc;
    }
    bw_done = true;
  }
  const bool early = c->batch_early_chain && bw_done;
  bool any_on_side = false;
  for (uint32_t s0 = 0, sgi = 0; s0 < nproofs; s0 += SG, sgi++) {
    const uint32_t sg = std::min(SG, nproofs - s0);
    uint64_t *sproofs = d_proofs + (size_t)s0 * 5 * ctl;
    uint32_t *WALL, *HALL, *VALL;
    whv_of(sgi, WALL, HALL, VALL);
    const BatchCoef co = {WALL, HALL, VALL, d};
    if (early && sgi + 1 < nsg) {
      if (sgi >= 1) HIP_TRY(c, hipStreamWaitEvent(chain_stream, c->ev_rdone[(sgi - 1) % nbuf], 0));
      rc = launch_chain(sgi + 1);
      if (rc) return rc;
    }
    if (early && sgi >= 2) HIP_TRY(c, hipStreamWaitEvent(main_stream, c->ev_sgdone[sgi - 2], 0));
    HIP_TRY(c, hipStreamWaitEvent(main_stream, c->ev_wdone[sgi % nbuf], 0));
    bool on_side = false;
    rc = batch_rows_supergroup(c, d_crs_c8, 0, 1, sg, h_witness_bits + (size_t)s0 * bits_stride, bits_stride, co, sproofs, B, slot, h_delta + s0,
                               c->ev_cdone[sgi % nbuf], 0, B.CW + (size_t)sgi * B.cw_stride, bw_done, sgi, early ? &on_side : nullptr);
    if (rc) return rc;
    if (early) HIP_TRY(c, hipEventRecord(c->ev_rdone[sgi % nbuf], main_stream));
    else if (sgi + 1 < nsg) {
      HIP_TRY(c, hipEventRecord(c->ev_rdone[sgi % nbuf], main_stream));
      HIP_TRY(c, hipStreamWaitEvent(chain_stream, c->ev_rdone[sgi % nbuf], 0));
      rc = launch_chain(sgi + 1);
      if (rc) return rc;
    }
    {
      OnStream tail(c, on_side ? c->side : main_stream);
      rc = batch_smudge_staged(c, B, sproofs, s0, sg);
      if (rc) return rc;
      HIP_TRY(c, hipEventRecord(c->ev_sgdone[sgi], c->stream));
    }
    any_on_side = any_on_side || on_side;
  }
  if (any_on_side) {
    HIP_TRY(c, hipEventRecord(c->ev_join, c->side));
    HIP_TRY(c, hipStreamWaitEvent(main_stream, c->ev_join, 0));
  }
  c->last_batch_sg = SG;
  c->last_batch_n = nproofs;
  return MFH_OK;
}

}

extern "C" {

int mfh_prove_batch(mfh_ctx *c, const uint8_t *d_crs_c8, const uint32_t *d_ssp, uint32_t nproofs, const uint8_t *h_witness_bits,
                    size_t bits_stride, const uint32_t *h_delta, const uint8_t *h_smudge_mag, size_t maglen, const uint8_t *h_smudge_sign,
                    uint64_t *d_proofs) {
  return prove_batch_impl(c, d_crs_c8, d_ssp, nproofs, h_witness_bits, bits_stride, h_delta, h_smudge_mag, maglen, h_smudge_sign, d_proofs, nullptr);
}

int mfh_prove_batch_public(mfh_ctx *c, const uint8_t *d_crs_c8, const uint32_t *d_ssp, uint32_t lu, uint32_t nproofs, const uint8_t *h_bits,
                           size_t bits_stride, const uint32_t *h_delta, const uint8_t *h_smudge_mag, size_t maglen, const uint8_t *h_smudge_sign,
                           uint64_t *d_proofs) {
  if (!c) return MFH_EINVAL;
  if (lu >= c->P.m) { c->err = "lu must be < m (the m - 1 wires of the SSP)"; return MFH_EINVAL; }
  if (!lu) return mfh_prove_batch(c, d_crs_c8, d_ssp, nproofs, h_bits, bits_stride, h_delta, h_smudge_mag, maglen, h_smudge_sign, d_proofs);
  if (!nproofs) return MFH_OK;
  if (!h_bits) return MFH_EINVAL;
  const uint32_t m = c->P.m, bstride = (m + 6) / 8, ub = (lu + 7) / 8;
  if (bits_stride < bstride) { c->err = "bits_stride shorter than the m - 1 witness bits"; return MFH_EINVAL; }
  std::vector<uint8_t> priv((size_t)nproofs * bstride), pubb;
  std::vector<uint32_t> zero;
  for (uint32_t b = 0; b < nproofs; b++) {
    uint8_t *x = priv.data() + (size_t)b * bstride;
    memcpy(x, h_bits + (size_t)b * bits_stride, bstride);
    memset(x, 0, lu >> 3);
    if (lu & 7) x[lu >> 3] &= (uint8_t)(0xffu << (lu & 7));
  }
  if (lu > kPubDirect) {
    pubb.assign((size_t)nproofs * bstride, 0);
    zero.assign(nproofs, 0);
    for (uint32_t b = 0; b < nproofs; b++) {
      uint8_t *x = pubb.data() + (size_t)b * bstride;
      memcpy(x, h_bits + (size_t)b * bits_stride, ub);
      if (lu & 7) x[ub - 1] &= (uint8_t)((1u << (lu & 7)) - 1);
    }
  }
  HIP_TRY(c, hipSetDevice(c->device));
  const size_t need = (size_t)nproofs * ub;
  if (int rc = dev_reserve(c, c->d_pub, need, DevWait::device)) return rc;
  uint8_t *st = (uint8_t *)pin_acquire(c, c->pin_pub, need);
  if (!st) return MFH_ENOMEM;
  for (uint32_t b = 0; b < nproofs; b++) memcpy(st + (size_t)b * ub, h_bits + (size_t)b * bits_stride, ub);
  HIP_TRY(c, hipMemcpyAsync(c->d_pub.p, st, need, hipMemcpyHostToDevice, c->stream));
  pin_release(c, c->pin_pub);
  const PubBatch pb{lu, c->d_pub.as<uint8_t>(), ub, lu > kPubDirect ? pubb.data() : nullptr, bstride, lu > kPubDirect ? zero.data() : nullptr};
  return prove_batch_impl(c, d_crs_c8, d_ssp, nproofs, priv.data(), bstride, h_delta, h_smudge_mag, maglen, h_smudge_sign, d_proofs, &pb);
}

uint32_t mfh_prove_batch_supergroup(const mfh_ctx *c) { return c ? c->last_batch_sg : 0; }

int mfh_prove_batch_stream_wait(mfh_ctx *c, uint32_t upto, void *hip_stream) {
  if (!c) return MFH_EINVAL;
  if (!c->last_batch_sg || !upto || upto > c->last_batch_n) { c->err = "mfh_prove_batch_stream_wait: no such statements in the last mfh_prove_batch call"; return MFH_EINVAL; }
  HIP_TRY(c, hipStreamWaitEvent((hipStream_t)hip_stream, c->ev_sgdone[(upto - 1) / c->last_batch_sg], 0));
  return MFH_OK;
}

int mfh_batch_chain(mfh_ctx *c, const uint32_t *d_ssp, uint32_t nstmt, const uint8_t *h_witness_bits, size_t bits_stride, const uint32_t *h_delta,
                    uint32_t *d_w, uint32_t *d_h, uint32_t *d_v) {
  if (!c) return MFH_EINVAL;
  if (!nstmt) return MFH_OK;
  if (!h_witness_bits || !h_delta || !d_w || !d_h || !d_v) return MFH_EINVAL;
  mf::SspSrc src;
  int rc = ssp_src(c, d_ssp, src, true);
  if (rc) return rc;
  const uint32_t d = c->P.d, m = c->P.m;
  if (bits_stride < (m + 6) / 8) { c->err = "bits_stride shorter than the m - 1 witness bits"; return MFH_EINVAL; }
  for (uint32_t b = 0; b < nstmt; b++)
    if (h_delta[b] >= P32) { c->err = "delta must be < p"; return MFH_EINVAL; }
  HIP_TRY(c, hipSetDevice(c->device));
  for (uint32_t s0 = 0; s0 < nstmt; s0 += BSG) {
    const size_t o = (size_t)s0 * d;
    rc = batch_chain_launch(c, src, d_ssp, std::min(BSG, nstmt - s0), h_witness_bits + (size_t)s0 * bits_stride, bits_stride, h_delta + s0, d_w + o, d_h + o,
                            d_v + o);
    if (rc) return rc;
  }
  return MFH_OK;
}

int mfh_batch_witness_cols(mfh_ctx *c, const uint32_t *d_ssp, uint32_t nstmt, const uint8_t *h_witness_bits, size_t bits_stride, const uint32_t *h_delta,
                           uint32_t col0, uint32_t ncols, uint32_t *d_w, size_t w_stride) {
  if (!c) return MFH_EINVAL;
  if (!nstmt || !ncols) return MFH_OK;
  if (!h_witness_bits || !h_delta || !d_w) return MFH_EINVAL;
  if (bits_stride < (c->P.m + 6) / 8) { c->err = "bits_stride shorter than the m - 1 witness bits"; return MFH_EINVAL; }
  for (uint32_t s0 = 0; s0 < nstmt; s0 += BSG) {
    int rc = mfh_witness_poly_mm_cols(c, d_ssp, std::min(BSG, nstmt - s0), h_witness_bits + (size_t)s0 * bits_stride, bits_stride, h_delta + s0, col0, ncols,
                                      d_w + (size_t)s0 * w_stride, w_stride);
    if (rc) return rc;
  }
  return MFH_OK;
}
int mfh_batch_chain_from_w(mfh_ctx *c, const uint32_t *d_ssp, uint32_t nstmt, const uint32_t *d_w, uint32_t *d_h, uint32_t *d_v) {
  if (!c) return MFH_EINVAL;
  if (!nstmt) return MFH_OK;
  if (!d_w || !d_h || !d_v) return MFH_EINVAL;
  mf::SspSrc src;
  int rc = ssp_src(c, d_ssp, src, true);
  if (rc) return rc;
  const uint32_t d = c->P.d;
  HIP_TRY(c, hipSetDevice(c->device));
  for (uint32_t s0 = 0; s0 < nstmt; s0 += BSG) {
    const uint32_t sg = std::min(BSG, nstmt - s0);
    const size_t o = (size_t)s0 * d;
    hipLaunchKernelGGL(k_add_slot_multi, dim3((d + 255) / 256, sg), dim3(256), 0, c->stream, d_w + o, src, 1u, d, d_v + o);
    HIP_TRY(c, hipGetLastError());
    rc = mfh_poly_h_multi(c, d_v + o, d_h + o, sg);
    if (rc) return rc;
  }
  return MFH_OK;
}

int mfh_prove_batch_partial(mfh_ctx *c, const uint8_t *d_crs_c8, uint32_t rank, uint32_t world, uint32_t nstmt, const uint8_t *h_witness_bits,
                            size_t bits_stride, const uint32_t *d_w, const uint32_t *d_h, const uint32_t *d_v, size_t coef_stride, uint64_t *d_partial) {
  if (!c || !world || rank >= world) return MFH_EINVAL;
  if (!nstmt) return MFH_OK;
  if (!d_crs_c8 || !h_witness_bits || !d_w || !d_h || !d_v || !d_partial) return MFH_EINVAL;
  if (c->resident_rows) { c->err = "mfh_prove_batch_partial: clear the single-proof resident CRS image first"; return MFH_EUNSUPPORTED; }
  if (c->mm_image && (c->mm_rank != rank || c->mm_world != world)) {
    c->err = "the registered matrix-core image holds the row shares of a different (rank, world)";
    return MFH_EINVAL;
  }
  const uint32_t d = c->P.d, m = c->P.m, n = c->P.n;
  const uint32_t cS = (uint32_t)((uint64_t)d * (rank + 1) / world) - (uint32_t)((uint64_t)d * rank / world);
  if (bits_stride < (m + 6) / 8) { c->err = "bits_stride shorter than the m - 1 witness bits"; return MFH_EINVAL; }
  if (coef_stride < cS) { c->err = "coef_stride shorter than the rank's share of the S / AS rows"; return MFH_EINVAL; }
  const size_t ctl = (size_t)(n + 1) * ((c->P.logq + 63) / 64);
  HIP_TRY(c, hipSetDevice(c->device));
  BatchScratch B;
// ... 76 lines not shown
```

c-lwe-snarks_amd/csrc/witness.hip:

```cpp
#include <algorithm>
#include <type_traits>

#include "ctx.hpp"

namespace {

typedef int v4i __attribute__((ext_vector_type(4)));
typedef int v16i __attribute__((ext_vector_type(16)));

__device__ __forceinline__ uint64_t partial_sum(const uint64_t *__restrict__ partial, uint32_t G, uint32_t d, uint32_t k, uint64_t s) {
  for (uint32_t g = 0; g < G; g++) s = (s + partial[(uint64_t)g * d + k] % MFH_P) % MFH_P;
  return s;
}
__device__ __forceinline__ uint32_t byte_plane(uint32_t x0, uint32_t x1, uint32_t x2, uint32_t x3, int w) {
  return __builtin_amdgcn_perm(x1, x0, 0x0c0c0400u + 0x00000101u * w)
         | __builtin_amdgcn_perm(x3, x2, 0x04000c0cu + 0x01010000u * w);
}
__device__ __forceinline__ constexpr uint32_t acc_row(uint32_t e, uint32_t h) { return (e & 3) + 8 * (e >> 2) + 4 * h; }

__global__ __launch_bounds__(256) void k_witness_partial(const uint32_t *__restrict__ ssp, const uint32_t *__restrict__ rows, uint32_t nsel,
                                                         uint32_t d, uint64_t *__restrict__ partial) {
  const uint32_t k4 = blockIdx.x * blockDim.x + threadIdx.x;
  if (k4 * 4 >= d) return;
  const uint32_t G = gridDim.y, g = blockIdx.y;
  uint64_t s0 = 0, s1 = 0, s2 = 0, s3 = 0;
  for (uint32_t i = g; i < nsel; i += G) {
    const uint4 v = *reinterpret_cast<const uint4 *>(ssp + (uint64_t)rows[i] * d + (uint64_t)k4 * 4);
    s0 += v.x; s1 += v.y; s2 += v.z; s3 += v.w;
  }
  uint64_t *o = partial + (uint64_t)g * d + (uint64_t)k4 * 4;
  o[0] = s0; o[1] = s1; o[2] = s2; o[3] = s3;
}

__global__ __launch_bounds__(256) void k_witness_partial_prg(uint64_t seed, const uint32_t *__restrict__ rows, uint32_t nsel, uint32_t d,
                                                             uint64_t *__restrict__ partial) {
  const uint32_t k4 = blockIdx.x * blockDim.x + threadIdx.x;
  if (k4 * 4 >= d) return;
  const uint32_t G = gridDim.y, g = blockIdx.y;
  const uint32_t k = k4 * 4;
  uint64_t s0 = 0, s1 = 0, s2 = 0, s3 = 0;
  for (uint32_t i = g; i < nsel; i += G) {
    const uint32_t rk = mf::ssp_prg_rowkey(seed, rows[i]);
    s0 += mf::ssp_prg_raw(rk, k);
    s1 += mf::ssp_prg_raw(rk, k + 1);
    s2 += mf::ssp_prg_raw(rk, k + 2);
    s3 += mf::ssp_prg_raw(rk, k + 3);
  }
  uint64_t *o = partial + (uint64_t)g * d + k;
  o[0] = s0; o[1] = s1; o[2] = s2; o[3] = s3;
}
template <int NB>
__global__ __launch_bounds__(256) void k_witness_partial_multi(const uint32_t *__restrict__ ssp, const uint2 *__restrict__ list, uint32_t nsel,
                                                               uint32_t d, uint64_t *__restrict__ partial) {
  const uint32_t k4 = blockIdx.x * blockDim.x + threadIdx.x;
  if (k4 * 4 >= d) return;
  const uint32_t G = gridDim.y, g = blockIdx.y;
  uint64_t acc[NB][4];
#pragma unroll
  for (int b = 0; b < NB; b++) acc[b][0] = acc[b][1] = acc[b][2] = acc[b][3] = 0;
  auto add = [&](const uint4 &v, uint32_t mask) {
#pragma unroll
    for (int b = 0; b < NB; b++)
      if ((mask >> b) & 1) { acc[b][0] += v.x; acc[b][1] += v.y; acc[b][2] += v.z; acc[b][3] += v.w; }
  };
  const uint32_t *col = ssp + (uint64_t)k4 * 4;
  uint32_t i = g;
  for (; i + 3 * G < nsel; i += 4 * G) {
    const uint2 e0 = list[i], e1 = list[i + G], e2 = list[i + 2 * G], e3 = list[i + 3 * G];
    const uint4 v0 = *reinterpret_cast<const uint4 *>(col + (uint64_t)e0.x * d), v1 = *reinterpret_cast<const uint4 *>(col + (uint64_t)e1.x * d);
    const uint4 v2 = *reinterpret_cast<const uint4 *>(col + (uint64_t)e2.x * d), v3 = *reinterpret_cast<const uint4 *>(col + (uint64_t)e3.x * d);
    add(v0, e0.y); add(v1, e1.y); add(v2, e2.y); add(v3, e3.y);
  }
  for (; i < nsel; i += G) {
    const uint2 e = list[i];
    add(*reinterpret_cast<const uint4 *>(col + (uint64_t)e.x * d), e.y);
  }
#pragma unroll
  for (int b = 0; b < NB; b++) {
    uint64_t *o = partial + ((uint64_t)b * G + g) * d + (uint64_t)k4 * 4;
    o[0] = acc[b][0]; o[1] = acc[b][1]; o[2] = acc[b][2]; o[3] = acc[b][3];
  }
}
template <int NB>
__global__ __launch_bounds__(256) void k_witness_partial_multi_prg(uint64_t seed, const uint2 *__restrict__ list, uint32_t nsel, uint32_t d,
                                                                   uint64_t *__restrict__ partial) {
  const uint32_t k4 = blockIdx.x * blockDim.x + threadIdx.x;
  if (k4 * 4 >= d) return;
  const uint32_t G = gridDim.y, g = blockIdx.y, k = k4 * 4;
  uint64_t acc[NB][4];
#pragma unroll
  for (int b = 0; b < NB; b++) acc[b][0] = acc[b][1] = acc[b][2] = acc[b][3] = 0;
  for (uint32_t i = g; i < nsel; i += G) {
    const uint2 e = list[i];
    const uint32_t rk = mf::ssp_prg_rowkey(seed, e.x);
    const uint32_t v0 = mf::ssp_prg_raw(rk, k), v1 = mf::ssp_prg_raw(rk, k + 1), v2 = mf::ssp_prg_raw(rk, k + 2), v3 = mf::ssp_prg_raw(rk, k + 3);
#pragma unroll
    for (int b = 0; b < NB; b++)
      if ((e.y >> b) & 1) { acc[b][0] += v0; acc[b][1] += v1; acc[b][2] += v2; acc[b][3] += v3; }
  }
#pragma unroll
  for (int b = 0; b < NB; b++) {
    uint64_t *o = partial + ((uint64_t)b * G + g) * d + k;
    o[0] = acc[b][0]; o[1] = acc[b][1]; o[2] = acc[b][2]; o[3] = acc[b][3];
  }
}
__global__ void k_ssp_prg_fill(uint64_t seed, uint32_t first_slot, uint32_t d, uint64_t total, uint32_t *__restrict__ out) {
  for (uint64_t i = (uint64_t)blockIdx.x * blockDim.x + threadIdx.x; i < total; i += (uint64_t)gridDim.x * blockDim.x) {
    const uint32_t slot = first_slot + (uint32_t)(i / d), k = (uint32_t)(i % d);
    out[i] = mf::ssp_prg_coeff(mf::ssp_prg_rowkey(seed, slot), k);
  }
}
__global__ void k_ssp_prg_make_t(uint64_t seed, const uint64_t *__restrict__ partial, uint32_t G, uint32_t d, uint32_t *__restrict__ t) {
  uint32_t k = blockIdx.x * blockDim.x + threadIdx.x;
  if (k >= d) return;
  uint64_t s = partial_sum(partial, G, d, k, mf::ssp_prg_coeff(mf::ssp_prg_rowkey(seed, 1), k));
  if (k == 0) s = (s + MFH_P - 1) % MFH_P;
  t[k] = (uint32_t)s;
}
__global__ void k_witness_finish(const uint32_t *__restrict__ ssp, const uint64_t *__restrict__ partial, uint32_t G, uint32_t d, uint32_t delta,
                                 uint32_t *__restrict__ w) {
  uint32_t k = blockIdx.x * blockDim.x + threadIdx.x;
  if (k >= d) return;
  w[k] = (uint32_t)partial_sum(partial, G, d, k, ((uint64_t)ssp[k] * delta) % MFH_P);
}
__global__ void k_witness_lanes(const uint64_t *__restrict__ partial, uint32_t G, uint32_t d, uint64_t *__restrict__ lanes) {
  uint32_t k = blockIdx.x * blockDim.x + threadIdx.x;
  if (k >= d) return;
  lanes[k] = partial_sum(partial, G, d, k, 0);
}

__global__ void k_ssp_frag(const uint32_t *__restrict__ ssp, uint32_t nrowsel, uint32_t d, uint32_t *__restrict__ frag) {
  const uint64_t gid = (uint64_t)blockIdx.x * blockDim.x + threadIdx.x;
  const uint32_t KT = d / 32;
  const uint32_t lane = gid & 63, eg = (gid >> 6) & 3;
  const uint64_t tile = gid >> 8;
  const uint32_t kt = (uint32_t)(tile % KT), K = (uint32_t)(tile / KT);
  const uint32_t KSt = (nrowsel + 31) / 32;
  if (K >= KSt) return;
  const uint32_t k = kt * 32 + (lane & 31), rb = K * 32 + 16 * (lane >> 5) + 4 * eg;
  uint32_t x[4];
#pragma unroll
  for (int e = 0; e < 4; e++) x[e] = rb + e < nrowsel ? ssp[(uint64_t)(rb + e + 2) * d + k] ^ 0x80808080u : 0u;
#pragma unroll
  for (int w = 0; w < 4; w++) frag[(((((uint64_t)kt * KSt + K) * 4 + w) * 64 + lane) << 2) + eg] = byte_plane(x[0], x[1], x[2], x[3], w);
}
struct WCols {
  uint32_t kt0;
  uint32_t KS;
  uint64_t wstride;
};
template <int MT>
__global__ __launch_bounds__(256) void k_witness_mm(const v4i *__restrict__ sspfrag, const v4i *__restrict__ bitfrag, uint32_t nrowsel ,
                                                    uint32_t ksteps_per_chunk, uint32_t d, int *__restrict__ part, WCols wc) {
  const uint32_t lane = threadIdx.x & 63, wave = threadIdx.x >> 6;
  const uint32_t r32 = lane & 31, h = lane >> 5;
  const uint32_t ktl = blockIdx.x * 4 + wave, kt = wc.kt0 + ktl;
  const uint32_t k = ktl * 32 + r32;
  const uint32_t K0 = blockIdx.y * ksteps_per_chunk, K1 = min((nrowsel + 31) / 32, K0 + ksteps_per_chunk);
  v16i acc[MT][4];
#pragma unroll
  for (int t = 0; t < MT; t++)
#pragma unroll
    for (int w = 0; w < 4; w++)
#pragma unroll
      for (int e = 0; e < 16; e++) acc[t][w][e] = 0;
  if (K0 >= K1) return;
  constexpr int PF = 3;
  v4i bq[PF][4], aq[PF][MT];
  auto fetch = [&](int slot, uint32_t K) {
    K = min(K, K1 - 1);
    const v4i *src = sspfrag + (((uint64_t)kt * wc.KS + K) * 4) * 64 + lane;
#pragma unroll
    for (int w = 0; w < 4; w++) bq[slot][w] = src[64 * w];
#pragma unroll
    for (int t = 0; t < MT; t++) aq[slot][t] = bitfrag[((uint64_t)K * MT + t) * 64 + lane];
  };
#pragma unroll
  for (int i = 0; i < PF; i++) fetch(i, K0 + i);
  for (uint32_t K = K0; K < K1; K += PF) {
#pragma unroll
    for (int i = 0; i < PF; i++) {
      if (K + i < K1) {
#pragma unroll
        for (int t = 0; t < MT; t++)
#pragma unroll
          for (int w = 0; w < 4; w++) acc[t][w] = __builtin_amdgcn_mfma_i32_32x32x32_i8(aq[i][t], bq[i][w], acc[t][w], 0, 0, 0);
        fetch(i, K + i + PF);
      }
    }
  }
#pragma unroll
  for (int t = 0; t < MT; t++)
#pragma unroll
    for (int w = 0; w < 4; w++)
#pragma unroll
      for (int e = 0; e < 16; e++) {
        const uint32_t stmt = 32 * t + acc_row(e, h);
        part[(((uint64_t)blockIdx.y * 4 + w) * (32 * MT) + stmt) * d + k] = acc[t][w][e];
      }
}
__global__ void k_prg_rowkeys(uint64_t seed, uint32_t nrows_pad, uint32_t *__restrict__ rk) {
  const uint32_t r = blockIdx.x * blockDim.x + threadIdx.x;
  if (r < nrows_pad) rk[r] = mf::ssp_prg_rowkey(seed, r + 2);
}
template <int MT>
__global__ __launch_bounds__(256) void k_witness_mm_prg(const uint32_t *__restrict__ rowkeys, const v4i *__restrict__ bitfrag, uint32_t nrowsel ,
                                                        uint32_t ksteps_per_chunk, uint32_t d, int *__restrict__ part, WCols wc) {
  const uint32_t lane = threadIdx.x & 63, wave = threadIdx.x >> 6;
  const uint32_t r32 = lane & 31, h = lane >> 5;
  const uint32_t kt = blockIdx.x * 4 + wave;
  const uint32_t k = kt * 32 + r32;
  const uint32_t K0 = blockIdx.y * ksteps_per_chunk, K1 = min((nrowsel + 31) / 32, K0 + ksteps_per_chunk);
  v16i acc[MT][4];
#pragma unroll
  for (int t = 0; t < MT; t++)
#pragma unroll
    for (int w = 0; w < 4; w++)
#pragma unroll
      for (int e = 0; e < 16; e++) acc[t][w][e] = 0;
  if (K0 >= K1) return;
  const uint32_t kc = wc.kt0 * 32 + k + mf::SSP_PRG_K0;
  constexpr int PF = 2;
  v4i aqr[PF][MT];
  uint4 rkr[PF][4];
  auto fetch = [&](uint32_t K, int slot) {
    K = min(K, K1 - 1);
#pragma unroll
    for (int t = 0; t < MT; t++) aqr[slot][t] = bitfrag[((uint64_t)K * MT + t) * 64 + lane];
    const uint4 *rk4 = reinterpret_cast<const uint4 *>(rowkeys + 32 * (uint64_t)K + 16 * h);
#pragma unroll
    for (int q = 0; q < 4; q++) rkr[slot][q] = rk4[q];
  };
  fetch(K0, 0);
  fetch(K0 + 1, 1);
  auto step = [&](uint32_t K, int slot) {
    v4i aq[MT];
#pragma unroll
    for (int t = 0; t < MT; t++) aq[t] = aqr[slot][t];
    uint32_t x[16];
#pragma unroll
    for (int q = 0; q < 4; q++) {
      const uint4 r = rkr[slot][q];
      x[4 * q] = r.x; x[4 * q + 1] = r.y; x[4 * q + 2] = r.z; x[4 * q + 3] = r.w;
    }
    fetch(K + PF, slot);
#pragma unroll
    for (int e = 0; e < 16; e++) x[e] = mf::ssp_prg_mix(kc * x[e]);
    v4i bq[4];
#pragma unroll
    for (int w = 0; w < 4; w++)
#pragma unroll
      for (int j = 0; j < 4; j++) bq[w][j] = (int)(byte_plane(x[4 * j], x[4 * j + 1], x[4 * j + 2], x[4 * j + 3], w) ^ 0x80808080u);
#pragma unroll
    for (int t = 0; t < MT; t++)
#pragma unroll
      for (int w = 0; w < 4; w++) acc[t][w] = __builtin_amdgcn_mfma_i32_32x32x32_i8(aq[t], bq[w], acc[t][w], 0, 0, 0);
  };
  uint32_t K = K0;
  for (; K + 2 <= K1; K += 2) {
    step(K, 0);
    step(K + 1, 1);
  }
  if (K < K1) step(K, 0);
#pragma unroll
  for (int t = 0; t < MT; t++)
#pragma unroll
    for (int w = 0; w < 4; w++)
#pragma unroll
      for (int e = 0; e < 16; e++) {
        const uint32_t stmt = 32 * t + acc_row(e, h);
        part[(((uint64_t)blockIdx.y * 4 + w) * (32 * MT) + stmt) * d + k] = acc[t][w][e];
      }
}
__global__ __launch_bounds__(512) void k_witness_mm8q_prg(const uint32_t *__restrict__ rowkeys, const v4i *__restrict__ bitfrag, uint32_t nrowsel ,
                                                          uint32_t ksteps_per_chunk, uint32_t d, int *__restrict__ part, WCols wc) {
  constexpr int MT = 8, RING = 4;
  __shared__ v4i bits[RING][MT][64];
  __shared__ uint32_t xch[3][2][4][64][4];
  const uint32_t tid = threadIdx.x, lane = tid & 63, wave = tid >> 6;
  const uint32_t r32 = lane & 31, h = lane >> 5;
  const uint32_t tile = wave >> 2, pl = wave & 3;
  const uint32_t sh = pl >> 1, pp = pl & 1;
  const uint32_t pos = (pl + (lane >> 4)) & 3;
  const uint32_t ktl = blockIdx.x * 2 + tile, kt = wc.kt0 + ktl;
  const uint32_t kc = kt * 32 + r32 + mf::SSP_PRG_K0;
  const uint32_t K0 = blockIdx.y * ksteps_per_chunk, K1 = min((nrowsel + 31) / 32, K0 + ksteps_per_chunk);
  v16i acc[4][2];
#pragma unroll
  for (int t = 0; t < 4; t++)
#pragma unroll
    for (int q = 0; q < 2; q++)
#pragma unroll
      for (int e = 0; e < 16; e++) acc[t][q][e] = 0;
  if (K0 >= K1) return;
  auto bits_load = [&](uint32_t K) -> v4i { return bitfrag[(uint64_t)min(K, K1 - 1) * MT * 64 + tid]; };
  auto bits_store = [&](uint32_t K, v4i st) { (&bits[K % RING][0][0])[tid] = st; };
  auto rk_load = [&](uint32_t K) -> uint4 { return *reinterpret_cast<const uint4 *>(rowkeys + 32 * (uint64_t)min(K, K1 - 1) + 16 * h + 4 * pos); };
  auto hash1 = [&](uint32_t rowkey) -> uint32_t {
#ifdef WPRG_NOHASH
    return kc ^ rowkey;
#endif
    return mf::ssp_prg_mix(kc * rowkey);
  };
  auto publish = [&](uint32_t K, const uint32_t (&x)[4]) {
#pragma unroll
    for (int w = 0; w < 4; w++) xch[K % 3][tile][w][lane][pos] = byte_plane(x[0], x[1], x[2], x[3], w) ^ 0x80808080u;
  };
  auto fragment = [&](uint32_t K, uint32_t q) -> v4i { return *reinterpret_cast<const v4i *>(&xch[K % 3][tile][2 * pp + q][lane][0]); };
  uint4 rkr[4];
  v4i sta, stb;
  sta = bits_load(K0);
  bits_store(K0, sta);
  sta = bits_load(K0 + 1);
  stb = bits_load(K0 + 2);
  {
    const uint4 r0 = rk_load(K0), r1 = rk_load(K0 + 1);
    const uint32_t x0[4] = {hash1(r0.x), hash1(r0.y), hash1(r0.z), hash1(r0.w)};
    const uint32_t x1[4] = {hash1(r1.x), hash1(r1.y), hash1(r1.z), hash1(r1.w)};
    publish(K0, x0);
    publish(K0 + 1, x1);
  }
#pragma unroll
  for (int i = 2; i <= 5; i++) rkr[i & 3] = rk_load(K0 + i);
  __syncthreads();
  v4i bq0 = fragment(K0, 0), bq1 = fragment(K0, 1);
  uint32_t K = K0;
  auto step = [&](int slot, v4i &st) {
    const v4i bn0 = fragment(K + 1, 0), bn1 = fragment(K + 1, 1);
    const uint4 rk = rkr[(slot + 2) & 3];
    const uint32_t hr[4] = {rk.x, rk.y, rk.z, rk.w};
    uint32_t hx[4];
    bits_store(K + 1, st);
    const v4i *aq = &bits[K % RING][4 * sh][lane];
#pragma unroll
    for (int t = 0; t < 4; t++) {
      const v4i a = aq[t * 64];
#ifdef WPRG_NOMFMA
      acc[t][0][0] += a[0] ^ bq0[t];
      acc[t][1][0] += a[1] ^ bq1[t];
#else
      acc[t][0] = __builtin_amdgcn_mfma_i32_32x32x32_i8(a, bq0, acc[t][0], 0, 0, 0);
      acc[t][1] = __builtin_amdgcn_mfma_i32_32x32x32_i8(a, bq1, acc[t][1], 0, 0, 0);
#endif
      hx[t] = hash1(hr[t]);
    }
    publish(K + 2, hx);
    rkr[(slot + 2) & 3] = rk_load(K + 6);
    bq0 = bn0;
    bq1 = bn1;
    st = bits_load(K + 3);
#ifndef WPRG_NOSYNC
    __syncthreads();
#endif
    K++;
  };
  while (K + 4 <= K1) {
    step(0, sta);
    step(1, stb);
    step(2, sta);
    step(3, stb);
  }
  if (K < K1) step(0, sta);
  if (K < K1) step(1, stb);
  if (K < K1) step(2, sta);
  uint32_t dd = d;
  asm volatile("" : "+s"(dd));
#pragma unroll
  for (int q = 0; q < 2; q++) {
    int *dst = part + (((uint64_t)blockIdx.y * 4 + 2 * pp + q) * (32 * MT) + 128 * sh) * dd + ktl * 32 + r32 + (uint64_t)(4 * h) * dd;
#pragma unroll
    for (int t = 0; t < 4; t++) {
#pragma unroll
      for (int e = 0; e < 16; e++) dst[(uint64_t)acc_row(e, 0) * dd] = acc[t][q][e];
      dst += (uint64_t)32 * dd;
    }
  }
}
__global__ __launch_bounds__(512) void k_witness_mm8q(const v4i *__restrict__ sspfrag, const v4i *__restrict__ bitfrag, uint32_t nrowsel ,
                                                      uint32_t ksteps_per_chunk, uint32_t d, int *__restrict__ part, const uint32_t *__restrict__ tpoly ,
                                                      const uint32_t *__restrict__ cnt_delta, uint32_t nstmt, uint32_t *__restrict__ w_out, WCols wc) {
  constexpr int MT = 8, RING = 4, PF = 4;
  __shared__ v4i bits[RING][MT][64];
  __shared__ uint32_t xch[2][3][16][64];
  const uint32_t tid = threadIdx.x, lane = tid & 63, wave = tid >> 6;
  const uint32_t r32 = lane & 31, h = lane >> 5;
  const uint32_t tile = wave >> 2, pl = wave & 3;
  const uint32_t ktl = blockIdx.x * 2 + tile, kt = wc.kt0 + ktl;
  const uint32_t K0 = blockIdx.y * ksteps_per_chunk, K1 = min((nrowsel + 31) / 32, K0 + ksteps_per_chunk);
  v16i acc[MT];
#pragma unroll
  for (int t = 0; t < MT; t++)
#pragma unroll
    for (int e = 0; e < 16; e++) acc[t][e] = 0;
  if (K0 >= K1) return;
  auto bits_load = [&](uint32_t K) -> v4i { return bitfrag[(uint64_t)min(K, K1 - 1) * MT * 64 + tid]; };
  auto bits_store = [&](uint32_t K, v4i st) { (&bits[K % RING][0][0])[tid] = st; };
  auto ssp_load = [&](uint32_t K) -> v4i { return sspfrag[(((uint64_t)kt * wc.KS + min(K, K1 - 1)) * 4 + pl) * 64 + lane]; };
  v4i stg[PF], bq[PF];
  {
    const v4i s0 = bits_load(K0), s1 = bits_load(K0 + 1);
    __builtin_amdgcn_sched_barrier(0);
#pragma unroll
    for (int i = 0; i < PF; i++) {
      bq[i] = ssp_load(K0 + i);
      stg[i] = bits_load(K0 + 2 + i);
      __builtin_amdgcn_sched_barrier(0);
    }
    bits_store(K0, s0);
    bits_store(K0 + 1, s1);
  }
  __syncthreads();
  v4i acur[MT];
#pragma unroll
  for (int t = 0; t < MT; t++) acur[t] = bits[K0 % RING][t][lane];
  uint32_t K = K0;
  auto step = [&](int slot) {
    bits_store(K + 2, stg[slot]);
    v4i anext[MT];
    const v4i *aq = &bits[(K + 1) % RING][0][lane];
#pragma unroll
    for (int t = 0; t < MT; t++) anext[t] = aq[t * 64];
    __builtin_amdgcn_sched_barrier(0);
#pragma unroll
    for (int t = 0; t < MT; t++) acc[t] = __builtin_amdgcn_mfma_i32_32x32x32_i8(acur[t], bq[slot], acc[t], 0, 0, 0);
    __builtin_amdgcn_sched_barrier(0);
    bq[slot] = ssp_load(K + PF);
    stg[slot] = bits_load(K + 2 + PF);
#pragma unroll
    for (int t = 0; t < MT; t++) acur[t] = anext[t];
    __syncthreads();
    K++;
  };
  while (K + PF <= K1) {
#pragma unroll
    for (int i = 0; i < PF; i++) step(i);
  }
#pragma unroll
  for (int i = 0; i + 1 < PF; i++)
    if (K < K1) step(i);
  uint32_t dd = d;
  asm volatile("" : "+s"(dd));
  if (part) {
    int *dst = part + ((uint64_t)blockIdx.y * 4 + pl) * (32 * MT) * dd + ktl * 32 + r32 + (uint64_t)(4 * h) * dd;
#pragma unroll
    for (int t = 0; t < MT; t++) {
#pragma unroll
      for (int e = 0; e < 16; e++) dst[(uint64_t)acc_row(e, 0) * dd] = acc[t][e];
      dst += (uint64_t)32 * dd;
    }
    return;
  }
  asm volatile("" : "+s"(cnt_delta), "+s"(tpoly));
  const uint32_t k = ktl * 32 + r32;
  const uint64_t tk = tpoly[k], ws = wc.wstride, P = MFH_P;
#pragma unroll
  for (int t = 0; t < MT; t++) {
    const uint32_t owner = t >> 1;
    uint32_t mine[16];
#pragma unroll
    for (int e = 0; e < 16; e++) {
      const uint32_t b = 32 * t + acc_row(e, h);
      mine[e] = (uint32_t)acc[t][e] + (b < nstmt ? 128u * cnt_delta[2 * b] : 0u);
    }
    if (pl != owner) {
      const uint32_t sidx = pl - (pl > owner);
#pragma unroll
      for (int e = 0; e < 16; e++) xch[tile][sidx][e][lane] = mine[e];
    }
    __syncthreads();
    if (pl == owner) {
#pragma unroll
      for (int e = 0; e < 16; e++) {
        const uint32_t b = 32 * t + acc_row(e, h);
        if (b < nstmt) {
          uint64_t val = (uint64_t)mine[e] << (8 * owner);
#pragma unroll
          for (int o = 0; o < 4; o++)
            if (o != (int)owner) val += (uint64_t)xch[tile][o - (o > (int)owner)][e][lane] << (8 * o);
          w_out[(uint64_t)b * ws + k] = (uint32_t)((val % P + tk * cnt_delta[2 * b + 1] % P) % P);
        }
      }
    }
    __syncthreads();
  }
}
__global__ void k_witness_bits(const uint8_t *__restrict__ bits, size_t bits_stride, uint32_t nstmt, uint32_t nrowsel, uint32_t ksteps, uint32_t MT,
                               int8_t *__restrict__ bitfrag) {
  const uint32_t i = blockIdx.x * blockDim.x + threadIdx.x;
  if (i >= ksteps * MT * 64) return;
  const uint32_t lane = i & 63, t = (i >> 6) % MT, K = (i >> 6) / MT, stmt = 32 * t + (lane & 31), h = lane >> 5;
  const uint32_t r0 = K * 32 + 16 * h;
  uint32_t w = 0;
  if (stmt < nstmt && r0 < nrowsel) {
    const uint8_t *b = bits + (size_t)stmt * bits_stride + (r0 >> 3);
    w = b[0];
    if (r0 + 8 < nrowsel) w |= (uint32_t)b[1] << 8;
    if (nrowsel - r0 < 16) w &= (1u << (nrowsel - r0)) - 1;
  }
  uint32_t o[4];
#pragma unroll
  for (int q = 0; q < 4; q++) {
    const uint32_t n4 = (w >> (4 * q)) & 15;
    o[q] = (n4 & 1) | ((n4 & 2) << 7) | ((n4 & 4) << 14) | ((n4 & 8) << 21);
  }
  reinterpret_cast<uint4 *>(bitfrag)[i] = uint4{o[0], o[1], o[2], o[3]};
}
__global__ void k_witness_mm_finish(const int *__restrict__ part, uint32_t nchunks, const uint32_t *__restrict__ t, const uint32_t *__restrict__ cnt_delta,
                                    uint32_t nstmt, uint32_t mrows , uint32_t d, uint32_t *__restrict__ w_out, uint64_t wstride) {
  const uint32_t k = blockIdx.x * blockDim.x + threadIdx.x, b = blockIdx.y;
  if (k >= d || b >= nstmt) return;
  const uint64_t corr = 128ull * cnt_delta[2 * b];
  const uint32_t delta = cnt_delta[2 * b + 1];
  uint64_t val = 0;
#pragma unroll
  for (int w = 0; w < 4; w++) {
    int64_t g = 0;
    for (uint32_t ch = 0; ch < nchunks; ch++) g += part[(((uint64_t)ch * 4 + w) * mrows + b) * d + k];
    val += (uint64_t)(g + (int64_t)corr) << (8 * w);
  }
  const uint64_t P = MFH_P;
  w_out[(uint64_t)b * wstride + k] = (uint32_t)((val % P + (uint64_t)t[k] * delta % P) % P);
}

bool witness_args_ok(const mfh_ctx *c, uint32_t nstmt, uint32_t nmax, const void *in, const uint32_t *h_delta, const uint32_t *d_w) {
  return c && in && h_delta && d_w && nstmt && nstmt <= nmax;
}
int witness_deltas(mfh_ctx *c, uint32_t nstmt, const uint32_t *h_delta) {
  for (uint32_t b = 0; b < nstmt; b++)
    if (h_delta[b] >= MFH_P) { c->err = "delta must be < p"; return MFH_EINVAL; }
  return MFH_OK;
}
inline uint32_t witness_bit(const uint8_t *h_bits, uint32_t i) { return (h_bits[(i - 1) >> 3] >> ((i - 1) & 7)) & 1u; }
uint32_t witness_count(const uint8_t *h_bits, uint32_t m) {
  uint32_t cnt = 0, i = 1;
  for (; i + 8 <= m; i += 8) cnt += (uint32_t)__builtin_popcount(h_bits[(i - 1) >> 3]);
  for (; i < m; i++) cnt += witness_bit(h_bits, i);
  return cnt;
}
constexpr size_t up256(size_t x) { return (x + 255) & ~(size_t)255; }
template <int N> struct WwsCarve {
  size_t off[N + 1] = {0};
  WwsCarve(const size_t (&bytes)[N]) { for (int i = 0; i < N; i++) off[i + 1] = off[i] + bytes[i]; }
  size_t bytes(int i) const { return off[i + 1] - off[i]; }
  int reserve(mfh_ctx *c) const { return wws_reserve(c, off[N]); }
  template <class T> T *at(const mfh_ctx *c, int i) const { return reinterpret_cast<T *>(c->wws.as<uint8_t>() + off[i]); }
};

template <class F> int witness_partials(mfh_ctx *c, const mf::SspSrc &src, const uint8_t *h_bits, uint32_t rank, uint32_t world, F &&finish) {
  const uint32_t d = c->P.d, m = c->P.m;
  if (d % 4) { c->err = "d must be a multiple of 4"; return MFH_EINVAL; }
  uint32_t *rows = (uint32_t *)pin_acquire(c, c->pin_rows, (size_t)m * 4 + 4);
  if (!rows) return MFH_ENOMEM;
  uint32_t nall = 0;
  for (uint32_t i = 1; i < m; i++)
    if (witness_bit(h_bits, i)) rows[nall++] = i + 1;
  const uint32_t lo = (uint32_t)((uint64_t)nall * rank / world), hi = (uint32_t)((uint64_t)nall * (rank + 1) / world);
  const uint32_t nsel = hi - lo, G = std::max(1u, std::min(64u, nsel / 8 + 1));
  const WwsCarve<2> ws({up256((size_t)m * 4), (size_t)G * d * 8});
  if (int rc = ws.reserve(c)) return rc;
  uint32_t *d_rows = ws.at<uint32_t>(c, 0);
  uint64_t *partial = ws.at<uint64_t>(c, 1);
  if (nsel) HIP_TRY(c, hipMemcpyAsync(d_rows, rows + lo, (size_t)nsel * 4, hipMemcpyHostToDevice, c->stream));
  pin_release(c, c->pin_rows);
  if (src.dense)
    hipLaunchKernelGGL(k_witness_partial, dim3((d / 4 + 255) / 256, G), dim3(256), 0, c->stream, src.dense, d_rows, nsel, d, partial);
  else
    hipLaunchKernelGGL(k_witness_partial_prg, dim3((d / 4 + 255) / 256, G), dim3(256), 0, c->stream, src.seed, d_rows, nsel, d, partial);
  HIP_TRY(c, hipGetLastError());
  finish(partial, G);
  HIP_TRY(c, hipGetLastError());
  return MFH_OK;
}

struct MmPlan {
  uint32_t MT;
  uint32_t nrowsel, ksteps;
  bool fused;
  uint32_t nchunks, kpc, ychunks;
  size_t packed, cd_off;
  enum { HEAD, BITFRAG, PART, ROWKEYS };
  WwsCarve<4> ws;
  MmPlan(const mfh_ctx *c, bool dense, uint32_t nstmt, size_t bits_stride, uint32_t nc)
      : MT(nstmt > 128 ? 8 : nstmt > 64 ? 4 : nstmt > 32 ? 2 : 1), nrowsel(c->P.m - 1), ksteps((nrowsel + 31) / 32),
        fused(MT == 8 && dense && c->P.m < 65536 && (nc >= 16384 || ksteps <= 64)), nchunks(fused ? 1u : std::min(ksteps, 4u)),
        kpc((ksteps + nchunks - 1) / nchunks), ychunks((ksteps + kpc - 1) / kpc), packed((size_t)nstmt * bits_stride), cd_off(packed + (8 - packed % 8) % 8),
        ws({up256(packed + 8 + 256 * 8), (size_t)ksteps * MT * 1024, (size_t)nchunks * 4 * 32 * MT * nc * 4, dense ? 0 : up256((size_t)ksteps * 32 * 4)}) {}
};
template <class F> void with_mt(uint32_t MT, F &&f) {
  if (MT == 1) f(std::integral_constant<int, 1>{});
  else if (MT == 2) f(std::integral_constant<int, 2>{});
  else f(std::integral_constant<int, 4>{});
}

}

extern "C" {

int mfh_ssp_set_prg(mfh_ctx *c, uint64_t seed, const uint32_t *d_t) {
  if (!c) return MFH_EINVAL;
  if (d_t) ssp_rows_free(c, false);
  c->prg_on = d_t != nullptr;
  c->prg_seed = seed;
  c->prg_t = d_t;
  return MFH_OK;
}

int mfh_ssp_prg_fill(mfh_ctx *c, uint64_t seed, size_t first_slot, size_t nslots, uint32_t *d_out) {
  if (!c || !d_out) return MFH_EINVAL;
  HIP_TRY(c, hipSetDevice(c->device));
  const uint64_t total = (uint64_t)nslots * c->P.d;
  if (!total) return MFH_OK;
  hipLaunchKernelGGL(k_ssp_prg_fill, dim3((uint32_t)std::min<uint64_t>((total + 255) / 256, 4096)), dim3(256), 0, c->stream, seed, (uint32_t)first_slot,
                     c->P.d, total, d_out);
  HIP_TRY(c, hipGetLastError());
  return MFH_OK;
}

int mfh_ssp_prg_make_t(mfh_ctx *c, uint64_t seed, const uint8_t *h_bits, uint32_t *d_t) {
  if (!c || !h_bits || !d_t) return MFH_EINVAL;
  HIP_TRY(c, hipSetDevice(c->device));
  return witness_partials(c, mf::SspSrc{nullptr, d_t, seed}, h_bits, 0, 1, [&](const uint64_t *partial, uint32_t G) {
    hipLaunchKernelGGL(k_ssp_prg_make_t, dim3((c->P.d + 255) / 256), dim3(256), 0, c->stream, seed, partial, G, c->P.d, d_t);
  });
}

int mfh_witness_poly(mfh_ctx *c, const uint32_t *d_ssp, const uint8_t *h_bits, uint32_t delta, uint32_t *d_w) {
  if (!witness_args_ok(c, 1, 1, h_bits, &delta, d_w)) return MFH_EINVAL;
  if (int rc = witness_deltas(c, 1, &delta)) return rc;
  HIP_TRY(c, hipSetDevice(c->device));
  if (ssp_is_rows(c, d_ssp)) return ssp_rows_witness(c, 1, h_bits, (c->P.m + 6) / 8, &delta, d_w, c->P.d);
  mf::SspSrc src;
  if (int rc = ssp_src(c, d_ssp, src)) return rc;
  return witness_partials(c, src, h_bits, 0, 1, [&](const uint64_t *partial, uint32_t G) {
    hipLaunchKernelGGL(k_witness_finish, dim3((c->P.d + 255) / 256), dim3(256), 0, c->stream, src.t, partial, G, c->P.d, delta, d_w);
  });
}

int mfh_witness_poly_multi(mfh_ctx *c, const uint32_t *d_ssp, uint32_t nstmt, const uint8_t *h_bits, size_t bits_stride, const uint32_t *h_delta, uint32_t *d_w) {
  constexpr int NB = 12;
  if (!witness_args_ok(c, nstmt, NB, h_bits, h_delta, d_w)) return MFH_EINVAL;
  if (ssp_is_rows(c, d_ssp)) return ssp_rows_witness(c, nstmt, h_bits, bits_stride, h_delta, d_w, c->P.d);
  mf::SspSrc src;
  if (int rc = ssp_src(c, d_ssp, src)) return rc;
  const uint32_t d = c->P.d, m = c->P.m;
  if (d % 4) { c->err = "d must be a multiple of 4"; return MFH_EINVAL; }
  if (int rc = witness_deltas(c, nstmt, h_delta)) return rc;
  HIP_TRY(c, hipSetDevice(c->device));
  uint2 *list = (uint2 *)pin_acquire(c, c->pin_rows, (size_t)m * 8 + 8);
  if (!list) return MFH_ENOMEM;
  uint32_t nsel = 0;
  for (uint32_t i = 1; i < m; i++) {
    uint32_t mask = 0;
    for (uint32_t b = 0; b < nstmt; b++) mask |= witness_bit(h_bits + b * bits_stride, i) << b;
    if (mask) list[nsel++] = make_uint2(i + 1, mask);
  }
  const uint32_t G = std::max(1u, std::min(16u, nsel / 8 + 1));
  const WwsCarve<2> ws({up256((size_t)m * 8), (size_t)NB * G * d * 8});
  if (int rc = ws.reserve(c)) return rc;
  uint2 *d_list = ws.at<uint2>(c, 0);
  uint64_t *partial = ws.at<uint64_t>(c, 1);
  if (nsel) HIP_TRY(c, hipMemcpyAsync(d_list, list, (size_t)nsel * 8, hipMemcpyHostToDevice, c->stream));
  pin_release(c, c->pin_rows);
  if (src.dense)
    hipLaunchKernelGGL(k_witness_partial_multi<NB>, dim3((d / 4 + 255) / 256, G), dim3(256), 0, c->stream, src.dense, d_list, nsel, d, partial);
  else
    hipLaunchKernelGGL(k_witness_partial_multi_prg<NB>, dim3((d / 4 + 255) / 256, G), dim3(256), 0, c->stream, src.seed, d_list, nsel, d, partial);
  HIP_TRY(c, hipGetLastError());
  for (uint32_t b = 0; b < nstmt; b++)
    hipLaunchKernelGGL(k_witness_finish, dim3((d + 255) / 256), dim3(256), 0, c->stream, src.t, partial + (size_t)b * G * d, G, d, h_delta[b],
                       d_w + (size_t)b * d);
  HIP_TRY(c, hipGetLastError());
  return MFH_OK;
}

int mfh_witness_lanes(mfh_ctx *c, const uint32_t *d_ssp, const uint8_t *h_bits, uint32_t rank, uint32_t world, uint64_t *d_lanes) {
  if (!c || !h_bits || !d_lanes || world == 0 || rank >= world) return MFH_EINVAL;
  HIP_TRY(c, hipSetDevice(c->device));
  mf::SspSrc src;
  if (int rc = ssp_src(c, d_ssp, src)) return rc;
  return witness_partials(c, src, h_bits, rank, world, [&](const uint64_t *partial, uint32_t G) {
    hipLaunchKernelGGL(k_witness_lanes, dim3((c->P.d + 255) / 256), dim3(256), 0, c->stream, partial, G, c->P.d, d_lanes);
  });
}

int mfh_witness_from_lanes(mfh_ctx *c, const uint32_t *d_ssp, const uint64_t *d_lanes, uint32_t delta, uint32_t *d_w) {
  if (!witness_args_ok(c, 1, 1, d_lanes, &delta, d_w)) return MFH_EINVAL;
  if (int rc = witness_deltas(c, 1, &delta)) return rc;
  HIP_TRY(c, hipSetDevice(c->device));
  mf::SspSrc src;
  if (int rc = ssp_src(c, d_ssp, src)) return rc;
  hipLaunchKernelGGL(k_witness_finish, dim3((c->P.d + 255) / 256), dim3(256), 0, c->stream, src.t, d_lanes, 1u, c->P.d, delta, d_w);
  HIP_TRY(c, hipGetLastError());
  return MFH_OK;
}

int mfh_witness_poly_mm_cols(mfh_ctx *c, const uint32_t *d_ssp, uint32_t nstmt, const uint8_t *h_bits, size_t bits_stride, const uint32_t *h_delta,
                             uint32_t col0, uint32_t ncols, uint32_t *d_w, size_t w_stride) {
  if (!witness_args_ok(c, nstmt, 256, h_bits, h_delta, d_w)) return MFH_EINVAL;
  mf::SspSrc src;
  if (int rc = ssp_src(c, d_ssp, src)) return rc;
  const uint32_t d = c->P.d, m = c->P.m, nc = ncols;
  if (d % 128 || m < 2) { c->err = "mfh_witness_poly_mm: d must be a multiple of 128"; return MFH_EUNSUPPORTED; }
  if ((uint64_t)col0 + ncols > d || w_stride < ncols) return MFH_EINVAL;
  if (ncols == 0) return MFH_OK;
  if (col0 % 128 || ncols % 128) { c->err = "mfh_witness_poly_mm_cols: the coefficient range must start and end at multiples of 128"; return MFH_EUNSUPPORTED; }
  if (int rc = witness_deltas(c, nstmt, h_delta)) return rc;
  HIP_TRY(c, hipSetDevice(c->device));
  const MmPlan P(c, src.dense != nullptr, nstmt, bits_stride, nc);
  const WCols wc = {col0 / 32, P.ksteps, (uint64_t)w_stride};
  const uint32_t *tpoly = src.t + col0;
  const size_t sfrag_b = (size_t)P.ksteps * 32 * d * 4;
  if (src.dense && (c->ssp_frag_src != d_ssp || c->ssp_frag.cap < sfrag_b)) {
    if (int rc = dev_reserve(c, c->ssp_frag, sfrag_b)) return rc;
    hipLaunchKernelGGL(k_ssp_frag, dim3(P.ksteps * (d / 32)), dim3(256), 0, c->stream, d_ssp, P.nrowsel, d, c->ssp_frag.as<uint32_t>());
    HIP_TRY(c, hipGetLastError());
    c->ssp_frag_src = d_ssp;
  }
  if (int rc = P.ws.reserve(c)) return rc;
  const size_t head_b = P.ws.bytes(MmPlan::HEAD);
  PinBuf &wpin = c->pin_wring[c->pin_wnext++ % 8];
  uint8_t *stage = (uint8_t *)pin_acquire(c, wpin, head_b);
  if (!stage) return MFH_ENOMEM;
  memcpy(stage, h_bits, P.packed);
  uint32_t *cd = (uint32_t *)(stage + P.cd_off);
  for (uint32_t b = 0; b < nstmt; b++) {
    cd[2 * b] = witness_count(h_bits + (size_t)b * bits_stride, m);
    cd[2 * b + 1] = h_delta[b];
  }
  uint8_t *dev = P.ws.at<uint8_t>(c, MmPlan::HEAD);
  HIP_TRY(c, hipMemcpyAsync(dev, stage, head_b, hipMemcpyHostToDevice, c->stream));
  pin_release(c, wpin);
  const uint32_t *d_cd = (const uint32_t *)(dev + P.cd_off), *d_rk = P.ws.at<uint32_t>(c, MmPlan::ROWKEYS);
  const v4i *bitfrag = P.ws.at<v4i>(c, MmPlan::BITFRAG), *sspfrag = c->ssp_frag.as<const v4i>();
  int *d_part = P.ws.at<int>(c, MmPlan::PART);
  hipLaunchKernelGGL(k_witness_bits, dim3((P.ksteps * P.MT * 64 + 255) / 256), dim3(256), 0, c->stream, dev, bits_stride, nstmt, P.nrowsel, P.ksteps, P.MT, (int8_t *)bitfrag);
  if (!src.dense) hipLaunchKernelGGL(k_prg_rowkeys, dim3((P.ksteps * 32 + 255) / 256), dim3(256), 0, c->stream, src.seed, P.ksteps * 32, (uint32_t *)d_rk);
  const dim3 grid(nc / (P.MT == 8 ? 64 : 128), P.ychunks);
  if (P.MT == 8 && src.dense)
    hipLaunchKernelGGL(k_witness_mm8q, grid, dim3(512), 0, c->stream, sspfrag, bitfrag, P.nrowsel, P.kpc, nc, P.fused ? (int *)nullptr : d_part, tpoly, d_cd, nstmt,
                       d_w, wc);
  else if (P.MT == 8)
    hipLaunchKernelGGL(k_witness_mm8q_prg, grid, dim3(512), 0, c->stream, d_rk, bitfrag, P.nrowsel, P.kpc, nc, d_part, wc);
  else
    with_mt(P.MT, [&](auto mt) {
      constexpr int M = decltype(mt)::value;
      if (src.dense) hipLaunchKernelGGL(k_witness_mm<M>, grid, dim3(256), 0, c->stream, sspfrag, bitfrag, P.nrowsel, P.kpc, nc, d_part, wc);
      else hipLaunchKernelGGL(k_witness_mm_prg<M>, grid, dim3(256), 0, c->stream, d_rk, bitfrag, P.nrowsel, P.kpc, nc, d_part, wc);
    });
  if (!P.fused)
    hipLaunchKernelGGL(k_witness_mm_finish, dim3((nc + 255) / 256, nstmt), dim3(256), 0, c->stream, d_part, P.ychunks, tpoly, d_cd, nstmt, 32 * P.MT, nc, d_w,
                       (uint64_t)w_stride);
  HIP_TRY(c, hipGetLastError());
  return MFH_OK;
}

int mfh_witness_poly_mm(mfh_ctx *c, const uint32_t *d_ssp, uint32_t nstmt, const uint8_t *h_bits, size_t bits_stride, const uint32_t *h_delta, uint32_t *d_w) {
  if (!witness_args_ok(c, nstmt, 256, h_bits, h_delta, d_w)) return MFH_EINVAL;
  if (ssp_is_rows(c, d_ssp)) return ssp_rows_witness(c, nstmt, h_bits, bits_stride, h_delta, d_w, c->P.d);
  return mfh_witness_poly_mm_cols(c, d_ssp, nstmt, h_bits, bits_stride, h_delta, 0, c->P.d, d_w, c->P.d);
}

}
```

include/mfhip.h:

```cpp
#pragma once
#include <stddef.h>
#include <stdint.h>

#ifdef __cplusplus
extern "C" {
#endif

#define MFH_P 0xfffffffbu

enum {
  MFH_OK = 0,
  MFH_EINVAL = -1,
  MFH_EDEVICE = -2,
  MFH_ENOMEM = -3,
  MFH_EUNSUPPORTED = -4
};

typedef struct {
  uint32_t n;
  uint32_t logq;
  uint32_t d;
  uint32_t m;
} mfh_params;

typedef struct mfh_ctx mfh_ctx;

int mfh_ctx_create(mfh_ctx **out, int device, const mfh_params *P);
void mfh_ctx_destroy(mfh_ctx *ctx);
int mfh_set_stream(mfh_ctx *ctx, void *hip_stream);
int mfh_sync(mfh_ctx *ctx);
int mfh_scrub_staging(mfh_ctx *ctx);
const char *mfh_last_error(const mfh_ctx *ctx);
int mfh_set_seed(mfh_ctx *ctx, const uint8_t h_seed[40]);

int mfh_keystream(mfh_ctx *ctx, uint64_t off, void *d_out, size_t nbytes);
int mfh_sample_rows(mfh_ctx *ctx, uint64_t off, size_t nrows, uint64_t *d_out);

int mfh_ct_add(mfh_ctx *ctx, uint64_t *d_rop, const uint64_t *d_a, const uint64_t *d_b, size_t count);
int mfh_ct_mul_ui(mfh_ctx *ctx, uint64_t *d_rop, const uint64_t *d_a, uint32_t b, size_t count);
int mfh_ct_addmul_ui(mfh_ctx *ctx, uint64_t *d_rop, const uint64_t *d_a, uint32_t b, size_t count);

int mfh_eval_rows(mfh_ctx *ctx, uint64_t off, size_t nrows, const uint8_t *d_c8, const uint32_t *d_coeff0,
                  const uint32_t *d_coeff1, uint64_t *d_rop0, uint64_t *d_rop1, int accumulate);

size_t mfh_resident_row_bytes(const mfh_ctx *ctx);
int mfh_crs_expand(mfh_ctx *ctx, uint64_t off, size_t nrows, const uint8_t *d_c8, void *d_rows_out);
int mfh_crs_image_set_b(mfh_ctx *ctx, size_t first_row, size_t nrows, const uint8_t *d_c8, void *d_rows);
int mfh_eval_rows_resident(mfh_ctx *ctx, const void *d_rows, size_t first_row, size_t nrows, const uint32_t *d_coeff0,
                           const uint32_t *d_coeff1, uint64_t *d_rop0, uint64_t *d_rop1, int accumulate);
int mfh_crs_set_resident(mfh_ctx *ctx, const void *d_rows);
int mfh_crs_set_resident_prefix(mfh_ctx *ctx, const void *d_rows, size_t nrows_resident);
size_t mfh_resident_share_rows(const mfh_ctx *ctx, uint32_t rank, uint32_t world);
int mfh_crs_expand_share(mfh_ctx *ctx, const uint8_t *d_crs_c8, uint32_t rank, uint32_t world, void *d_image);
int mfh_crs_set_resident_share(mfh_ctx *ctx, const void *d_image, uint32_t rank, uint32_t world);

int mfh_encrypt_rows(mfh_ctx *ctx, uint64_t off, size_t nrows, const uint64_t *d_sk, const uint32_t *d_msg,
                     const uint64_t *d_err, uint8_t *d_c8_out);
int mfh_set_encrypt_path(mfh_ctx *ctx, int path);

int mfh_decrypt(mfh_ctx *ctx, const uint64_t *d_sk, const uint64_t *d_cts, size_t count, uint32_t *d_out);
int mfh_set_decrypt_path(mfh_ctx *ctx, int path);
int mfh_decrypt_rows(mfh_ctx *ctx, uint64_t off, size_t nrows, const uint64_t *d_sk, const uint8_t *d_c8, uint32_t *d_out);

int mfh_add_dotp(mfh_ctx *ctx, uint64_t *d_rop, const uint64_t *d_a, const uint64_t *d_b, size_t len);

int mfh_ct_smudge(mfh_ctx *ctx, uint64_t *d_cts, size_t count, const uint8_t *h_mag, size_t maglen, const uint8_t *h_sign);

int mfh_ssp_upload(mfh_ctx *ctx, const void *h_ssp_u64, uint32_t *d_ssp, size_t first_slot, size_t nslots);
int mfh_witness_poly(mfh_ctx *ctx, const uint32_t *d_ssp, const uint8_t *h_witness_bits, uint32_t delta, uint32_t *d_w);

int mfh_ssp_set_prg(mfh_ctx *ctx, uint64_t seed, const uint32_t *d_t);
int mfh_ssp_prg_make_t(mfh_ctx *ctx, uint64_t seed, const uint8_t *h_witness_bits, uint32_t *d_t);
int mfh_ssp_prg_fill(mfh_ctx *ctx, uint64_t seed, size_t first_slot, size_t nslots, uint32_t *d_out);

int mfh_ssp_from_rows(mfh_ctx *ctx, uint32_t nrows, const uint32_t *h_row_ptr, const uint32_t *h_wire, const uint32_t *h_coef, uint32_t *d_ssp);

int mfh_ssp_set_rows(mfh_ctx *ctx, uint32_t nrows, const uint32_t *h_row_ptr, const uint32_t *h_wire, const uint32_t *h_coef, uint32_t lu_max);
int mfh_ssp_rows_fill(mfh_ctx *ctx, size_t first_slot, size_t nslots, uint32_t *d_out);

int mfh_ssp_rows_violations(mfh_ctx *ctx, uint32_t nstmt, const uint8_t *h_bits, size_t bits_stride, uint32_t *h_count, uint32_t *h_first);

#define MFH_GATE_XOR 0u
#define MFH_GATE_AND 1u
#define MFH_GATE_OR 2u
#define MFH_GATE_NOT 3u
#define MFH_GATE_MAJ 4u
#define MFH_GATE_SUM3 5u
#define MFH_GATE_CONST0 6u
#define MFH_GATE_CONST1 7u
#define MFH_GATE_WSUM 8u
#define MFH_GATE_WSUM_BIT 9u
#define MFH_GATE_LUT2(tt) (16u + (tt))
#define MFH_CIRCUIT_MAX_WIRES 32767u
#define MFH_CIRCUIT_GLOBAL 1u
typedef struct mfh_circuit mfh_circuit;
int mfh_circuit_create(mfh_ctx *ctx, uint32_t nin, uint32_t ngates, const uint32_t *h_gates, uint32_t nasserts, const uint32_t *h_asserts,
                       mfh_circuit **out);
int mfh_circuit_create_global(mfh_ctx *ctx, uint32_t nin, uint32_t ngates, const uint32_t *h_gates, uint32_t nasserts, const uint32_t *h_asserts,
                              mfh_circuit **out);
int mfh_circuit_create_ex(mfh_ctx *ctx, uint32_t nin, uint32_t ngates, const uint32_t *h_gates, uint32_t nasserts, const uint32_t *h_asserts,
                          uint32_t nequal, const uint32_t *h_equal, uint32_t flags, mfh_circuit **out);
int mfh_circuit_create_out(mfh_ctx *ctx, uint32_t nin, uint32_t ngates, const uint32_t *h_gates, uint32_t nasserts, const uint32_t *h_asserts,
                           uint32_t nequal, const uint32_t *h_equal, uint32_t nout, const uint32_t *h_outputs, uint32_t flags, mfh_circuit **out);
int mfh_circuit_create_sum(mfh_ctx *ctx, uint32_t nin, uint32_t ngates, const uint32_t *h_gates, uint32_t nasserts, const uint32_t *h_asserts,
                           uint32_t nequal, const uint32_t *h_equal, uint32_t nout, const uint32_t *h_outputs, uint32_t nterms_total,
                           const uint32_t *h_terms, uint32_t flags, mfh_circuit **out);
void mfh_circuit_destroy(mfh_circuit *c);
int mfh_circuit_assign(mfh_ctx *ctx, const mfh_circuit *c, uint32_t nstmt, const uint8_t *h_inputs, size_t in_stride, uint8_t *h_witness_bits,
                       size_t bits_stride, uint8_t *h_holds);

typedef struct mfh_merkle mfh_merkle;
int mfh_merkle_create(mfh_ctx *ctx, uint32_t depth, mfh_merkle **out);
void mfh_merkle_destroy(mfh_merkle *t);
int mfh_merkle_set_leaves(mfh_ctx *ctx, mfh_merkle *t, uint32_t first, uint32_t count, const uint8_t *d_leaves);
int mfh_merkle_root(mfh_ctx *ctx, const mfh_merkle *t, uint8_t h_root[32]);
int mfh_merkle_nodes(const mfh_merkle *t, uint32_t level, const uint8_t **d_nodes);
int mfh_merkle_paths(mfh_ctx *ctx, const mfh_merkle *t, uint32_t nstmt, const uint32_t *h_index, uint8_t *h_inputs, size_t in_stride);

int mfh_sha256_records(mfh_ctx *ctx, const uint8_t *d_records, size_t stride, uint32_t length, uint32_t count, uint8_t *d_digests);
int mfh_merkle_set_records(mfh_ctx *ctx, mfh_merkle *t, uint32_t first, uint32_t count, const uint8_t *d_records, size_t stride, uint32_t length);

int mfh_merkle_update_rows(mfh_ctx *ctx, mfh_merkle *t, uint32_t nupd, const uint32_t *h_index, const uint8_t *d_new_leaves, uint8_t *h_inputs, size_t in_stride,
                           uint8_t *h_roots);

int mfh_poly_mul(mfh_ctx *ctx, const uint32_t *d_a, size_t la, const uint32_t *d_b, size_t lb, uint32_t *d_c);
int mfh_poly_add(mfh_ctx *ctx, const uint32_t *d_a, const uint32_t *d_b, size_t count, uint32_t *d_out);
int mfh_poly_prepare_t(mfh_ctx *ctx, const uint32_t *d_t);
int mfh_ssp_prepare(mfh_ctx *ctx, const uint32_t *d_ssp);
int mfh_poly_h(mfh_ctx *ctx, const uint32_t *d_v, uint32_t *d_h);
int mfh_poly_h_multi(mfh_ctx *ctx, const uint32_t *d_v, uint32_t *d_h, uint32_t nb);
int mfh_set_poly_exact(mfh_ctx *ctx, int mode);
long mfh_poly_exact_fallbacks(mfh_ctx *ctx);
int mfh_poly_exact_points(mfh_ctx *ctx, uint32_t *out);
int mfh_set_poly_exact_points(mfh_ctx *ctx, const uint32_t *pts);

int mfh_setup_messages(mfh_ctx *ctx, const uint32_t *d_ssp, uint32_t alpha, uint32_t beta, uint32_t s, uint32_t *d_msg);
int mfh_setup(mfh_ctx *ctx, const uint32_t *d_ssp, uint32_t alpha, uint32_t beta, uint32_t s, const uint64_t *d_sk,
              const uint64_t *d_err, uint8_t *d_crs_c8);
int mfh_setup_image(mfh_ctx *ctx, const uint32_t *d_ssp, uint32_t alpha, uint32_t beta, uint32_t s, const uint64_t *d_sk,
                    const uint64_t *d_err, uint8_t *d_crs_c8, void *d_rows_image);
int mfh_prove(mfh_ctx *ctx, const uint8_t *d_crs_c8, const uint32_t *d_ssp, const uint8_t *h_witness_bits, uint32_t delta,
              const uint8_t *h_smudge_mag, size_t maglen, const uint8_t *h_smudge_sign, uint64_t *d_proof);

int mfh_verify(mfh_ctx *ctx, const uint32_t *d_ssp, uint32_t alpha, uint32_t beta, uint32_t s, const uint64_t *d_sk,
               const uint64_t *d_proofs, size_t count, uint8_t *d_ok);

int mfh_setup_public(mfh_ctx *ctx, const uint32_t *d_ssp, uint32_t alpha, uint32_t beta, uint32_t s, uint32_t lu, const uint64_t *d_sk,
                     const uint64_t *d_err, uint8_t *d_crs_c8, void *d_rows_image);
int mfh_prove_public(mfh_ctx *ctx, const uint8_t *d_crs_c8, const uint32_t *d_ssp, uint32_t lu, const uint8_t *h_bits, uint32_t delta,
                     const uint8_t *h_smudge_mag, size_t maglen, const uint8_t *h_smudge_sign, uint64_t *d_proof);
int mfh_prove_batch_public(mfh_ctx *ctx, const uint8_t *d_crs_c8, const uint32_t *d_ssp, uint32_t lu, uint32_t nproofs, const uint8_t *h_bits,
                           size_t bits_stride, const uint32_t *h_delta, const uint8_t *h_smudge_mag, size_t maglen, const uint8_t *h_smudge_sign,
                           uint64_t *d_proofs);
int mfh_vk_derive(mfh_ctx *ctx, const uint32_t *d_ssp, uint32_t s, uint32_t lu, uint32_t *d_vk);
int mfh_verify_public(mfh_ctx *ctx, const uint32_t *d_vk, uint32_t lu, uint32_t alpha, uint32_t beta, const uint64_t *d_sk, const uint64_t *d_proofs,
                      const uint8_t *h_statements, size_t stmt_stride, size_t count, uint8_t *d_ok);

size_t mfh_crs_mm_image_bytes(const mfh_ctx *ctx);
int mfh_crs_expand_mm(mfh_ctx *ctx, const uint8_t *d_crs_c8, uint8_t *d_image);
int mfh_crs_set_resident_mm(mfh_ctx *ctx, const uint8_t *d_image);
int mfh_set_expand_path(mfh_ctx *ctx, int path);
int mfh_set_batch_image(mfh_ctx *ctx, int enabled);
int mfh_set_batch_slabs(mfh_ctx *ctx, uint32_t nslabs);
int mfh_set_encrypt_chunks(mfh_ctx *ctx, uint32_t chunks);
int mfh_set_eval_path(mfh_ctx *ctx, int path);
int mfh_set_witness_per(mfh_ctx *ctx, uint32_t statements);
int mfh_set_batch_launch(mfh_ctx *ctx, uint32_t groups_per_launch, int merge_regions);
int mfh_set_batch_bw(mfh_ctx *ctx, int merged);
int mfh_set_mm_stream(mfh_ctx *ctx, int map, int persistent, int sync_mode, uint32_t spin_max);
int mfh_set_mm_width(mfh_ctx *ctx, uint32_t per_xcd, int early_chain);
int mfh_set_mm_chunk_rows(mfh_ctx *ctx, uint32_t rows);
int mfh_set_mm_pack(mfh_ctx *ctx, int on);
int mfh_prove_batch(mfh_ctx *ctx, const uint8_t *d_crs_c8, const uint32_t *d_ssp, uint32_t nproofs, const uint8_t *h_witness_bits,
                    size_t bits_stride, const uint32_t *h_delta, const uint8_t *h_smudge_mag, size_t maglen, const uint8_t *h_smudge_sign,
                    uint64_t *d_proofs);
uint32_t mfh_prove_batch_supergroup(const mfh_ctx *ctx);
int mfh_prove_batch_stream_wait(mfh_ctx *ctx, uint32_t upto, void *hip_stream);
size_t mfh_crs_mm_share_bytes(const mfh_ctx *ctx, uint32_t rank, uint32_t world);
int mfh_crs_expand_mm_share(mfh_ctx *ctx, const uint8_t *d_crs_c8, uint32_t rank, uint32_t world, uint8_t *d_image);
int mfh_crs_set_resident_mm_share(mfh_ctx *ctx, const uint8_t *d_image, uint32_t rank, uint32_t world);
int mfh_batch_chain(mfh_ctx *ctx, const uint32_t *d_ssp, uint32_t nstmt, const uint8_t *h_witness_bits, size_t bits_stride, const uint32_t *h_delta,
                    uint32_t *d_w, uint32_t *d_h, uint32_t *d_v);
int mfh_batch_witness_cols(mfh_ctx *ctx, const uint32_t *d_ssp, uint32_t nstmt, const uint8_t *h_witness_bits, size_t bits_stride, const uint32_t *h_delta,
                           uint32_t col0, uint32_t ncols, uint32_t *d_w, size_t w_stride);
int mfh_batch_chain_from_w(mfh_ctx *ctx, const uint32_t *d_ssp, uint32_t nstmt, const uint32_t *d_w, uint32_t *d_h, uint32_t *d_v);
int mfh_prove_batch_partial(mfh_ctx *ctx, const uint8_t *d_crs_c8, uint32_t rank, uint32_t world, uint32_t nstmt, const uint8_t *h_witness_bits,
                            size_t bits_stride, const uint32_t *d_w, const uint32_t *d_h, const uint32_t *d_v, size_t coef_stride, uint64_t *d_partial);
int mfh_prove_batch_finish(mfh_ctx *ctx, const uint8_t *d_crs_c8, uint32_t nstmt, const uint32_t *h_delta, const uint8_t *h_smudge_mag, size_t maglen,
                           const uint8_t *h_smudge_sign, uint64_t *d_proofs);

int mfh_prove_partial(mfh_ctx *ctx, const uint8_t *d_crs_c8, const uint32_t *d_ssp, const uint8_t *h_witness_bits, uint32_t delta,
                      uint32_t rank, uint32_t world, uint64_t *d_partial);
int mfh_prove_finish(mfh_ctx *ctx, uint64_t *d_proof, const uint8_t *h_smudge_mag, size_t maglen, const uint8_t *h_smudge_sign);
int mfh_witness_poly_multi(mfh_ctx *ctx, const uint32_t *d_ssp, uint32_t nstmt, const uint8_t *h_bits, size_t bits_stride, const uint32_t *h_delta,
                           uint32_t *d_w);
int mfh_witness_poly_mm(mfh_ctx *ctx, const uint32_t *d_ssp, uint32_t nstmt, const uint8_t *h_bits, size_t bits_stride, const uint32_t *h_delta,
                        uint32_t *d_w);
int mfh_witness_poly_mm_cols(mfh_ctx *ctx, const uint32_t *d_ssp, uint32_t nstmt, const uint8_t *h_bits, size_t bits_stride, const uint32_t *h_delta,
                             uint32_t col0, uint32_t ncols, uint32_t *d_w, size_t w_stride);
int mfh_witness_lanes(mfh_ctx *ctx, const uint32_t *d_ssp, const uint8_t *h_witness_bits, uint32_t rank, uint32_t world, uint64_t *d_lanes);
int mfh_witness_from_lanes(mfh_ctx *ctx, const uint32_t *d_ssp, const uint64_t *d_lanes, uint32_t delta, uint32_t *d_w);
int mfh_prove_partial_w(mfh_ctx *ctx, const uint8_t *d_crs_c8, const uint32_t *d_ssp, const uint8_t *h_witness_bits, uint32_t delta,
                        uint32_t rank, uint32_t world, const uint64_t *d_wlanes, uint64_t *d_partial);
uint32_t mfh_lanes_per_value(const mfh_ctx *ctx);
int mfh_ct_to_lanes(mfh_ctx *ctx, const uint64_t *d_cts, size_t count, uint64_t *d_lanes);
int mfh_ct_from_lanes(mfh_ctx *ctx, const uint64_t *d_lanes, size_t count, uint64_t *d_cts);

const char *mfh_version(void);
int mfh_digest128(mfh_ctx *ctx, const void *d_buf, size_t nbytes, uint64_t h_digest[2]);
size_t mfh_workspace_bytes(const mfh_ctx *ctx);
int mfh_eval_rows_multi(mfh_ctx *ctx, uint64_t off, size_t nrows, const uint8_t *d_c8, const uint32_t *d_coeffs, uint32_t nvec,
                        uint32_t coeff_bytes, uint64_t *d_rops, int accumulate);

int mfh_set_timing(mfh_ctx *ctx, int enabled);
int mfh_set_overlap(mfh_ctx *ctx, int mode);
int mfh_timing_drain(mfh_ctx *ctx, const char *which, uint64_t *count, double *total_ms, uint64_t *total_rows, float *last_ms);
float mfh_last_kernel_ms(mfh_ctx *ctx, const char *which);
double mfh_timing_busy_ms(const mfh_ctx *ctx);
uint64_t mfh_timing_work_rows(const mfh_ctx *ctx);

#ifdef __cplusplus
}
#endif
```

Measured before the change: 13510.

## Batch witness/H chain across eight supergroups in one multi-group launch

Adds a batched chain mode, on by default, for the dense single-slab prove path. The witness-polynomial kernel and the H computation now run once for up to eight supergroups, using a grouped k_witness_mm8q launch whose grid spans all groups. The V = W + v0 addition is fused into the witness epilogue, so fewer launches and event handoffs are needed per supergroup. In exchange the W/H/V buffers are enlarged to eight supergroups, and the chain for each batch of eight waits for the previous row work, which can reduce overlap at batch boundaries.

```diff
diff --git a/c-lwe-snarks_amd/__init__.py b/c-lwe-snarks_amd/__init__.py
--- a/c-lwe-snarks_amd/__init__.py
+++ b/c-lwe-snarks_amd/__init__.py
@@ -81,7 +81,7 @@
     "mfh_workspace_bytes", "mfh_last_kernel_ms", "mfh_set_timing", "mfh_set_overlap", "mfh_eval_rows_multi", "mfh_prove_batch", "mfh_crs_mm_image_bytes", "mfh_crs_expand_mm", "mfh_crs_set_resident_mm", "mfh_witness_poly_multi", "mfh_witness_poly_mm", "mfh_poly_h_multi", "mfh_poly_mul", "mfh_poly_add", "mfh_poly_prepare_t",
     "mfh_ssp_prepare", "mfh_poly_h", "mfh_setup_messages", "mfh_setup", "mfh_setup_image", "mfh_crs_image_set_b", "mfh_prove",
     "mfh_prove_partial", "mfh_prove_finish", "mfh_ct_to_lanes", "mfh_ct_from_lanes", "mfh_lanes_per_value", "mfh_digest128", "mfh_timing_drain", "mfh_timing_busy_ms", "mfh_timing_work_rows", "mfh_set_batch_image", "mfh_set_batch_slabs", "mfh_set_expand_path", "mfh_set_encrypt_path", "mfh_set_batch_launch", "mfh_set_batch_bw", "mfh_set_mm_chunk_rows", "mfh_set_mm_pack", "mfh_set_poly_exact", "mfh_poly_exact_fallbacks", "mfh_poly_exact_points", "mfh_set_poly_exact_points", "mfh_set_mm_stream", "mfh_add_dotp", "mfh_set_encrypt_chunks", "mfh_set_witness_per", "mfh_set_eval_path", "mfh_set_decrypt_path", "mfh_decrypt_rows",
-    "mfh_crs_mm_share_bytes", "mfh_crs_expand_mm_share", "mfh_crs_set_resident_mm_share", "mfh_batch_chain", "mfh_batch_witness_cols", "mfh_batch_chain_from_w", "mfh_witness_poly_mm_cols", "mfh_prove_batch_partial", "mfh_prove_batch_finish",
+    "mfh_crs_mm_share_bytes", "mfh_crs_expand_mm_share", "mfh_crs_set_resident_mm_share", "mfh_batch_chain", "mfh_batch_witness_cols", "mfh_batch_chain_from_w", "mfh_witness_poly_mm_cols", "mfh_witness_poly_mm_groups", "mfh_set_batch_chain", "mfh_prove_batch_partial", "mfh_prove_batch_finish",
     "mfh_resident_row_bytes", "mfh_crs_expand", "mfh_eval_rows_resident", "mfh_crs_set_resident",
     "mfh_witness_lanes", "mfh_witness_from_lanes", "mfh_prove_partial_w", "mfh_verify",
     "mfh_ssp_set_prg", "mfh_ssp_prg_make_t", "mfh_ssp_prg_fill",
@@ -185,6 +185,7 @@
         "mfh_set_mm_stream": (i32, [vp, i32, i32, i32, u32]),
         "mfh_set_batch_launch": (i32, [vp, u32, i32]),
         "mfh_set_batch_bw": (i32, [vp, i32]),
+        "mfh_set_batch_chain": (i32, [vp, i32]),
         "mfh_set_encrypt_path": (i32, [vp, i32]),
         "mfh_set_expand_path": (i32, [vp, i32]),
         "mfh_set_batch_slabs": (i32, [vp, u32]),
@@ -200,6 +201,7 @@
         "mfh_batch_witness_cols": (i32, [vp, vp, u32, ctypes.c_char_p, sz, vp, u32, u32, vp, sz]),
         "mfh_batch_chain_from_w": (i32, [vp, vp, u32, vp, vp, vp]),
         "mfh_witness_poly_mm_cols": (i32, [vp, vp, u32, ctypes.c_char_p, sz, vp, u32, u32, vp, sz]),
+        "mfh_witness_poly_mm_groups": (i32, [vp, vp, u32, vp, ctypes.c_char_p, sz, vp, vp, vp]),
         "mfh_prove_batch_partial": (i32, [vp, vp, u32, u32, u32, ctypes.c_char_p, sz, vp, vp, vp, sz, vp]),
         "mfh_prove_batch_finish": (i32, [vp, vp, u32, vp, ctypes.c_char_p, sz, ctypes.c_char_p, vp]),
         "mfh_setup_public": (i32, [vp, vp, u32, u32, u32, u32, vp, vp, vp, vp]),
@@ -521,6 +523,9 @@
     def set_batch_bw(self, merged=True):
         self._chk(self.lib.mfh_set_batch_bw(self._h, 1 if merged else 0))
 
+    def set_batch_chain(self, mode=1):
+        self._chk(self.lib.mfh_set_batch_chain(self._h, int(mode)))
+
     def set_mm_stream(self, map=0, persistent=False, sync_mode=0, spin_max=64):
         self._chk(self.lib.mfh_set_mm_stream(self._h, int(map), int(persistent), int(sync_mode), int(spin_max)))
 
@@ -812,6 +817,19 @@
         self._chk(fn(self._h, _ptr(d_ssp), nb, bits, stride, ctypes.cast(dl, ctypes.c_void_p), _ptr(out)))
         return out
 
+    def witness_poly_groups(self, d_ssp, groups, deltas, w_out, v_out=None):
+        p = self.params
+        stride = (p.m + 6) // 8
+        flat = [w for g in groups for w in g]
+        bits = b"".join(bytes(w[:stride]).ljust(stride, b"\0") for w in flat)
+        dl = (ctypes.c_uint32 * len(flat))(*[int(x) for x in deltas])
+        ng = len(groups)
+        cnt = (ctypes.c_uint32 * ng)(*[len(g) for g in groups])
+        pw = (ctypes.c_void_p * ng)(*[t.data_ptr() for t in w_out])
+        pv = None if v_out is None else (ctypes.c_void_p * ng)(*[None if t is None else t.data_ptr() for t in v_out])
+        self._chk(self.lib.mfh_witness_poly_mm_groups(self._h, _ptr(d_ssp), ng, ctypes.cast(cnt, ctypes.c_void_p), bits, stride, ctypes.cast(dl, ctypes.c_void_p),
+                                                      ctypes.cast(pw, ctypes.c_void_p), None if pv is None else ctypes.cast(pv, ctypes.c_void_p)))
+
     def prove_batch(self, d_crs, d_ssp, witness_bits_list, deltas, smudge_mags, smudge_signs, maglen=80, out=None):
         p = self.params
         nb = len(witness_bits_list)
diff --git a/c-lwe-snarks_amd/csrc/ctx.hpp b/c-lwe-snarks_amd/csrc/ctx.hpp
--- a/c-lwe-snarks_amd/csrc/ctx.hpp
+++ b/c-lwe-snarks_amd/csrc/ctx.hpp
@@ -115,6 +115,7 @@
   uint32_t enc_chunks = 0;
   uint32_t witness_per = 0;
   uint32_t batch_slabs = 0;
+  int batch_chain = 1;
   int batch_bw_merged = 1;
   int batch_merge = 1;
   uint32_t batch_ngl = 8;
@@ -270,6 +271,8 @@
                                    uint32_t *d_w);
 extern "C" int mfh_witness_poly_mm_cols(mfh_ctx *c, const uint32_t *d_ssp, uint32_t nstmt, const uint8_t *h_bits, size_t bits_stride, const uint32_t *h_delta,
                                         uint32_t col0, uint32_t ncols, uint32_t *d_w, size_t w_stride);
+extern "C" int mfh_witness_poly_mm_groups(mfh_ctx *c, const uint32_t *d_ssp, uint32_t ngroups, const uint32_t *counts, const uint8_t *h_bits, size_t bits_stride,
+                                          const uint32_t *h_delta, uint32_t *const *d_w, uint32_t *const *d_v);
 extern "C" int mfh_poly_h_multi(mfh_ctx *c, const uint32_t *d_v, uint32_t *d_h, uint32_t nb);
 int expand_mm_region(mfh_ctx *c, uint64_t off, uint32_t nrows, const uint8_t *c8, uint8_t *image);
 int encrypt_rows_mm(mfh_ctx *c, uint64_t off, size_t nrows, const uint64_t *sk, const uint32_t *msg, const uint64_t *err, uint8_t *c8);
diff --git a/c-lwe-snarks_amd/csrc/mfhip.hip b/c-lwe-snarks_amd/csrc/mfhip.hip
--- a/c-lwe-snarks_amd/csrc/mfhip.hip
+++ b/c-lwe-snarks_amd/csrc/mfhip.hip
@@ -982,6 +982,12 @@
   return MFH_OK;
 }
 
+int mfh_set_batch_chain(mfh_ctx *c, int mode) {
+  if (!c || mode < 0 || mode > 2) return MFH_EINVAL;
+  c->batch_chain = mode;
+  return MFH_OK;
+}
+
 int mfh_set_batch_image(mfh_ctx *c, int en) {
   if (!c) return MFH_EINVAL;
   c->batch_image = en != 0;
diff --git a/c-lwe-snarks_amd/csrc/snark.hip b/c-lwe-snarks_amd/csrc/snark.hip
--- a/c-lwe-snarks_amd/csrc/snark.hip
+++ b/c-lwe-snarks_amd/csrc/snark.hip
@@ -948,7 +948,9 @@
       }
     }
   }
-  const uint32_t nbuf = nsl > 1 ? nsg : 2;
+  constexpr uint32_t kChainSG = 8;
+  const bool batched = c->batch_chain != 0 && nsl == 1 && !pub && src.dense && !src.prefix && d % 128 == 0 && !c->batch_early_chain && !c->witness_per;
+  const uint32_t nbuf = nsl > 1 ? nsg : batched ? std::min(nsg, kChainSG) : 2;
   while (c->ev_sgdone.size() < nsg) {
     hipEvent_t e;
     HIP_TRY(c, hipEventCreateWithFlags(&e, hipEventDisableTiming));
@@ -973,9 +975,33 @@
   }
   hipStream_t const main_stream = c->stream, chain_stream = c->side2;
   auto whv_of = [&](uint32_t sgi, uint32_t *&W, uint32_t *&H, uint32_t *&V) {
+    if (batched) {
+      W = B.WHV + (size_t)(sgi % nbuf) * SG * d;
+      H = W + (size_t)nbuf * BSG * d;
+      V = H + (size_t)nbuf * BSG * d;
+      return;
+    }
     W = B.WHV + (size_t)(sgi % nbuf) * 3 * BSG * d;
     H = W + (size_t)BSG * d;
     V = H + (size_t)BSG * d;
+  };
+  const hipStream_t batch_stream = c->batch_chain == 2 ? main_stream : chain_stream;
+  auto launch_chain_batch = [&](uint32_t sg0) -> int {
+    const uint32_t ng = std::min(kChainSG, nsg - sg0), s0 = sg0 * SG, cnt = std::min(ng * SG, nproofs - s0);
+    uint32_t counts[kChainSG], *W[kChainSG], *V[kChainSG], *H0 = nullptr, *Hk = nullptr;
+    for (uint32_t k = 0; k < ng; k++) {
+      counts[k] = std::min(SG, nproofs - (s0 + k * SG));
+      whv_of(sg0 + k, W[k], Hk, V[k]);
+      if (k == 0) H0 = Hk;
+    }
+    OnStream chain(c, batch_stream);
+    int r = mfh_witness_poly_mm_groups(c, d_ssp, ng, counts, h_witness_bits + (size_t)s0 * bits_stride, bits_stride, h_delta + s0, W, V);
+    if (r) return r;
+    HIP_TRY(c, hipEventRecord(c->ev_wdone[0], batch_stream));
+    r = mfh_poly_h_multi(c, V[0], H0, cnt);
+    if (r) return r;
+    HIP_TRY(c, hipEventRecord(c->ev_cdone[0], batch_stream));
+    return MFH_OK;
   };
   auto launch_chain = [&](uint32_t sgi) -> int {
     const uint32_t s0 = sgi * SG, sg = std::min(SG, nproofs - s0);
@@ -991,7 +1017,8 @@
   };
   HIP_TRY(c, hipEventRecord(c->ev_chain, main_stream));
   HIP_TRY(c, hipStreamWaitEvent(chain_stream, c->ev_chain, 0));
-  rc = launch_chain(0);
+  if (!batched) rc = launch_chain(0);
+  else if (c->batch_chain == 1) rc = launch_chain_batch(0);
   if (rc) return rc;
   if (nsl > 1) {
     for (uint32_t k = 1; k < nsg; k++) {
@@ -1043,6 +1070,10 @@
   ImageGuard transient{c, false};
   rc = batch_transient_image(c, d_crs_c8, nproofs, 0, 1, transient);
   if (rc) return rc;
+  if (batched && c->batch_chain == 2) {
+    rc = launch_chain_batch(0);
+    if (rc) return rc;
+  }
   rc = batch_stage_host(c, B, nproofs, h_witness_bits, bits_stride, h_delta, h_smudge_mag, maglen, h_smudge_sign, SG);
   if (rc) return rc;
   rc = batch_ct_t(c, d_crs_c8, B);
@@ -1083,12 +1114,19 @@
       if (rc) return rc;
     }
     if (early && sgi >= 2) HIP_TRY(c, hipStreamWaitEvent(main_stream, c->ev_sgdone[sgi - 2], 0));
-    HIP_TRY(c, hipStreamWaitEvent(main_stream, c->ev_wdone[sgi % nbuf], 0));
+    HIP_TRY(c, hipStreamWaitEvent(main_stream, c->ev_wdone[batched ? 0 : sgi % nbuf], 0));
     bool on_side = false;
     rc = batch_rows_supergroup(c, d_crs_c8, 0, 1, sg, h_witness_bits + (size_t)s0 * bits_stride, bits_stride, co, sproofs, B, slot, h_delta + s0,
-                               c->ev_cdone[sgi % nbuf], 0, B.CW + (size_t)sgi * B.cw_stride, bw_done, sgi, early ? &on_side : nullptr);
+                               c->ev_cdone[batched ? 0 : sgi % nbuf], 0, B.CW + (size_t)sgi * B.cw_stride, bw_done, sgi, early ? &on_side : nullptr);
     if (rc) return rc;
-    if (early) HIP_TRY(c, hipEventRecord(c->ev_rdone[sgi % nbuf], main_stream));
+    if (batched) {
+      if (sgi + 1 < nsg && (sgi + 1) % kChainSG == 0) {
+        HIP_TRY(c, hipEventRecord(c->ev_rdone[0], main_stream));
+        HIP_TRY(c, hipStreamWaitEvent(batch_stream, c->ev_rdone[0], 0));
+        rc = launch_chain_batch(sgi + 1);
+        if (rc) return rc;
+      }
+    } else if (early) HIP_TRY(c, hipEventRecord(c->ev_rdone[sgi % nbuf], main_stream));
     else if (sgi + 1 < nsg) {
       HIP_TRY(c, hipEventRecord(c->ev_rdone[sgi % nbuf], main_stream));
       HIP_TRY(c, hipStreamWaitEvent(chain_stream, c->ev_rdone[sgi % nbuf], 0));
diff --git a/c-lwe-snarks_amd/csrc/witness.hip b/c-lwe-snarks_amd/csrc/witness.hip
--- a/c-lwe-snarks_amd/csrc/witness.hip
+++ b/c-lwe-snarks_amd/csrc/witness.hip
@@ -149,6 +149,19 @@
   uint32_t KS;
   uint64_t wstride;
 };
+struct WGroup {
+  const v4i *bitfrag;
+  const uint32_t *cnt_delta;
+  uint32_t *w_out, *v_out;
+  uint32_t nstmt;
+};
+struct WGroups {
+  WGroup g[8];
+  uint32_t G, npairs;
+};
+__host__ __device__ __forceinline__ constexpr uint32_t wgroup_pair(uint32_t b, uint32_t G) { return b / (8 * G) * 8 + b % 8; }
+__host__ __device__ __forceinline__ constexpr uint32_t wgroup_of(uint32_t b, uint32_t G) { return b / 8 % G; }
+constexpr uint32_t wgroup_grid(uint32_t npairs, uint32_t G) { return (npairs + 7) / 8 * 8 * G; }
 template <int MT>
 __global__ __launch_bounds__(256) void k_witness_mm(const v4i *__restrict__ sspfrag, const v4i *__restrict__ bitfrag, uint32_t nrowsel ,
                                                     uint32_t ksteps_per_chunk, uint32_t d, int *__restrict__ part, WCols wc) {
@@ -376,16 +389,19 @@
     }
   }
 }
-__global__ __launch_bounds__(512) void k_witness_mm8q(const v4i *__restrict__ sspfrag, const v4i *__restrict__ bitfrag, uint32_t nrowsel ,
-                                                      uint32_t ksteps_per_chunk, uint32_t d, int *__restrict__ part, const uint32_t *__restrict__ tpoly ,
-                                                      const uint32_t *__restrict__ cnt_delta, uint32_t nstmt, uint32_t *__restrict__ w_out, WCols wc) {
+__global__ __launch_bounds__(512) void k_witness_mm8q(const v4i *__restrict__ sspfrag, WGroups wg, uint32_t nrowsel , uint32_t ksteps_per_chunk,
+                                                      uint32_t d, int *__restrict__ part, const uint32_t *__restrict__ tpoly ,
+                                                      const uint32_t *__restrict__ v0 , WCols wc) {
   constexpr int MT = 8, RING = 4, PF = 4;
   __shared__ v4i bits[RING][MT][64];
   __shared__ uint32_t xch[2][3][16][64];
   const uint32_t tid = threadIdx.x, lane = tid & 63, wave = tid >> 6;
   const uint32_t r32 = lane & 31, h = lane >> 5;
   const uint32_t tile = wave >> 2, pl = wave & 3;
-  const uint32_t ktl = blockIdx.x * 2 + tile, kt = wc.kt0 + ktl;
+  const uint32_t pair = wgroup_pair(blockIdx.x, wg.G), grp = wgroup_of(blockIdx.x, wg.G);
+  if (pair >= wg.npairs) return;
+  const v4i *__restrict__ bitfrag = wg.g[grp].bitfrag;
+  const uint32_t ktl = pair * 2 + tile, kt = wc.kt0 + ktl;
   const uint32_t K0 = blockIdx.y * ksteps_per_chunk, K1 = min((nrowsel + 31) / 32, K0 + ksteps_per_chunk);
   v16i acc[MT];
 #pragma unroll
@@ -450,9 +466,12 @@
     }
     return;
   }
+  const uint32_t *__restrict__ cnt_delta = wg.g[grp].cnt_delta;
+  uint32_t *__restrict__ w_out = wg.g[grp].w_out, *__restrict__ v_out = wg.g[grp].v_out;
+  const uint32_t nstmt = wg.g[grp].nstmt;
   asm volatile("" : "+s"(cnt_delta), "+s"(tpoly));
   const uint32_t k = ktl * 32 + r32;
-  const uint64_t tk = tpoly[k], ws = wc.wstride, P = MFH_P;
+  const uint64_t tk = tpoly[k], v0k = v_out ? v0[k] : 0u, ws = wc.wstride, P = MFH_P;
 #pragma unroll
   for (int t = 0; t < MT; t++) {
     const uint32_t owner = t >> 1;
@@ -477,17 +496,23 @@
 #pragma unroll
           for (int o = 0; o < 4; o++)
             if (o != (int)owner) val += (uint64_t)xch[tile][o - (o > (int)owner)][e][lane] << (8 * o);
-          w_out[(uint64_t)b * ws + k] = (uint32_t)((val % P + tk * cnt_delta[2 * b + 1] % P) % P);
+          const uint64_t w = (val % P + tk * cnt_delta[2 * b + 1] % P) % P;
+          w_out[(uint64_t)b * ws + k] = (uint32_t)w;
+          if (v_out) v_out[(uint64_t)b * ws + k] = (uint32_t)((w + v0k) % P);
         }
       }
     }
     __syncthreads();
   }
 }
-__global__ void k_witness_bits(const uint8_t *__restrict__ bits, size_t bits_stride, uint32_t nstmt, uint32_t nrowsel, uint32_t ksteps, uint32_t MT,
-                               int8_t *__restrict__ bitfrag) {
+struct WBitsGroups {
+  uint32_t bits_off[8], frag_off[8] , nstmt[8], MT[8];
+};
+__global__ void k_witness_bits(const uint8_t *__restrict__ head, size_t bits_stride, WBitsGroups bg, uint32_t nrowsel, uint32_t ksteps, int8_t *__restrict__ bitfrag) {
   const uint32_t i = blockIdx.x * blockDim.x + threadIdx.x;
+  const uint32_t g = blockIdx.y, MT = bg.MT[g], nstmt = bg.nstmt[g];
   if (i >= ksteps * MT * 64) return;
+  const uint8_t *__restrict__ bits = head + bg.bits_off[g];
   const uint32_t lane = i & 63, t = (i >> 6) % MT, K = (i >> 6) / MT, stmt = 32 * t + (lane & 31), h = lane >> 5;
   const uint32_t r0 = K * 32 + 16 * h;
   uint32_t w = 0;
@@ -503,10 +528,11 @@
     const uint32_t n4 = (w >> (4 * q)) & 15;
     o[q] = (n4 & 1) | ((n4 & 2) << 7) | ((n4 & 4) << 14) | ((n4 & 8) << 21);
   }
-  reinterpret_cast<uint4 *>(bitfrag)[i] = uint4{o[0], o[1], o[2], o[3]};
+  reinterpret_cast<uint4 *>(bitfrag)[(size_t)bg.frag_off[g] + i] = uint4{o[0], o[1], o[2], o[3]};
 }
 __global__ void k_witness_mm_finish(const int *__restrict__ part, uint32_t nchunks, const uint32_t *__restrict__ t, const uint32_t *__restrict__ cnt_delta,
-                                    uint32_t nstmt, uint32_t mrows , uint32_t d, uint32_t *__restrict__ w_out, uint64_t wstride) {
+                                    uint32_t nstmt, uint32_t mrows , uint32_t d, uint32_t *__restrict__ w_out, uint64_t wstride,
+                                    const uint32_t *__restrict__ v0, uint32_t *__restrict__ v_out ) {
   const uint32_t k = blockIdx.x * blockDim.x + threadIdx.x, b = blockIdx.y;
   if (k >= d || b >= nstmt) return;
   const uint64_t corr = 128ull * cnt_delta[2 * b];
@@ -519,7 +545,9 @@
     val += (uint64_t)(g + (int64_t)corr) << (8 * w);
   }
   const uint64_t P = MFH_P;
-  w_out[(uint64_t)b * wstride + k] = (uint32_t)((val % P + (uint64_t)t[k] * delta % P) % P);
+  const uint64_t w = (val % P + (uint64_t)t[k] * delta % P) % P;
+  w_out[(uint64_t)b * wstride + k] = (uint32_t)w;
+  if (v_out) v_out[(uint64_t)b * wstride + k] = (uint32_t)((w + v0[k]) % P);
 }
 
 bool witness_args_ok(const mfh_ctx *c, uint32_t nstmt, uint32_t nmax, const void *in, const uint32_t *h_delta, const uint32_t *d_w) {
@@ -592,6 +620,106 @@
   else f(std::integral_constant<int, 4>{});
 }
 
+int witness_mm_groups(mfh_ctx *c, const uint32_t *d_ssp, uint32_t ng, const uint32_t *counts, const uint8_t *h_bits, size_t bits_stride, const uint32_t *h_delta,
+                      uint32_t *const *d_w, uint32_t *const *d_v, uint32_t col0, uint32_t ncols, size_t w_stride) {
+  mf::SspSrc src;
+  if (int rc = ssp_src(c, d_ssp, src)) return rc;
+  const uint32_t d = c->P.d, m = c->P.m, nc = ncols;
+  if (d % 128 || m < 2) { c->err = "mfh_witness_poly_mm: d must be a multiple of 128"; return MFH_EUNSUPPORTED; }
+  if ((uint64_t)col0 + ncols > d || w_stride < ncols) return MFH_EINVAL;
+  if (ncols == 0) return MFH_OK;
+  if (col0 % 128 || ncols % 128) { c->err = "mfh_witness_poly_mm_cols: the coefficient range must start and end at multiples of 128"; return MFH_EUNSUPPORTED; }
+  bool want_v = false;
+  for (uint32_t g = 0; g < ng; g++) want_v = want_v || (d_v && d_v[g]);
+  if (want_v && !src.dense) { c->err = "mfh_witness_poly_mm_groups: V is written for a dense SSP only"; return MFH_EUNSUPPORTED; }
+  uint32_t first[9] = {0};
+  for (uint32_t g = 0; g < ng; g++) first[g + 1] = first[g] + counts[g];
+  if (int rc = witness_deltas(c, first[ng], h_delta)) return rc;
+  HIP_TRY(c, hipSetDevice(c->device));
+  std::vector<MmPlan> P;
+  P.reserve(ng);
+  size_t head_off[9] = {0}, frag_off[9] = {0}, part_b = 0;
+  for (uint32_t g = 0; g < ng; g++) {
+    P.emplace_back(c, src.dense != nullptr, counts[g], bits_stride, nc);
+    head_off[g + 1] = head_off[g] + P[g].ws.bytes(MmPlan::HEAD);
+    frag_off[g + 1] = frag_off[g] + P[g].ws.bytes(MmPlan::BITFRAG);
+    part_b = std::max(part_b, P[g].ws.bytes(MmPlan::PART));
+  }
+  const uint32_t ksteps = P[0].ksteps, nrowsel = P[0].nrowsel;
+  const WwsCarve<4> ws({head_off[ng], frag_off[ng], part_b, P[0].ws.bytes(MmPlan::ROWKEYS)});
+  const WCols wc = {col0 / 32, ksteps, (uint64_t)w_stride};
+  const uint32_t *tpoly = src.t + col0, *v0 = src.dense ? src.dense + d + col0 : nullptr;
+  const size_t sfrag_b = (size_t)ksteps * 32 * d * 4;
+  if (src.dense && (c->ssp_frag_src != d_ssp || c->ssp_frag.cap < sfrag_b)) {
+    if (int rc = dev_reserve(c, c->ssp_frag, sfrag_b)) return rc;
+    hipLaunchKernelGGL(k_ssp_frag, dim3(ksteps * (d / 32)), dim3(256), 0, c->stream, d_ssp, nrowsel, d, c->ssp_frag.as<uint32_t>());
+    HIP_TRY(c, hipGetLastError());
+    c->ssp_frag_src = d_ssp;
+  }
+  if (int rc = ws.reserve(c)) return rc;
+  PinBuf &wpin = c->pin_wring[c->pin_wnext++ % 8];
+  uint8_t *stage = (uint8_t *)pin_acquire(c, wpin, head_off[ng]);
+  if (!stage) return MFH_ENOMEM;
+  WBitsGroups bg = {};
+  uint32_t mtmax = 1;
+  for (uint32_t g = 0; g < ng; g++) {
+    const uint8_t *gb = h_bits + (size_t)first[g] * bits_stride;
+    memcpy(stage + head_off[g], gb, P[g].packed);
+    uint32_t *cd = (uint32_t *)(stage + head_off[g] + P[g].cd_off);
+    for (uint32_t b = 0; b < counts[g]; b++) {
+      cd[2 * b] = witness_count(gb + (size_t)b * bits_stride, m);
+      cd[2 * b + 1] = h_delta[first[g] + b];
+    }
+    bg.bits_off[g] = (uint32_t)head_off[g];
+    bg.frag_off[g] = (uint32_t)(frag_off[g] / 16);
+    bg.nstmt[g] = counts[g];
+    bg.MT[g] = P[g].MT;
+    mtmax = std::max(mtmax, P[g].MT);
+  }
+  uint8_t *dev = ws.at<uint8_t>(c, MmPlan::HEAD);
+  HIP_TRY(c, hipMemcpyAsync(dev, stage, head_off[ng], hipMemcpyHostToDevice, c->stream));
+  pin_release(c, wpin);
+  const uint32_t *d_rk = ws.at<uint32_t>(c, MmPlan::ROWKEYS);
+  const uint8_t *fragbase = ws.at<uint8_t>(c, MmPlan::BITFRAG);
+  const v4i *sspfrag = c->ssp_frag.as<const v4i>();
+  int *d_part = ws.at<int>(c, MmPlan::PART);
+  hipLaunchKernelGGL(k_witness_bits, dim3((ksteps * mtmax * 64 + 255) / 256, ng), dim3(256), 0, c->stream, dev, bits_stride, bg, nrowsel, ksteps, (int8_t *)fragbase);
+  if (!src.dense) hipLaunchKernelGGL(k_prg_rowkeys, dim3((ksteps * 32 + 255) / 256), dim3(256), 0, c->stream, src.seed, ksteps * 32, (uint32_t *)d_rk);
+  auto group_of = [&](uint32_t g) {
+    return WGroup{(const v4i *)(fragbase + frag_off[g]), (const uint32_t *)(dev + head_off[g] + P[g].cd_off), d_w[g], d_v ? d_v[g] : nullptr, counts[g]};
+  };
+  WGroups fg = {};
+  fg.npairs = nc / 64;
+  for (uint32_t g = 0; g < ng; g++)
+    if (P[g].fused) fg.g[fg.G++] = group_of(g);
+  if (fg.G)
+    hipLaunchKernelGGL(k_witness_mm8q, dim3(wgroup_grid(fg.npairs, fg.G)), dim3(512), 0, c->stream, sspfrag, fg, nrowsel, P[0].kpc, nc, (int *)nullptr, tpoly, v0, wc);
+  for (uint32_t g = 0; g < ng; g++) {
+    const MmPlan &Q = P[g];
+    if (Q.fused) continue;
+    const WGroup one = group_of(g);
+    const dim3 grid(nc / (Q.MT == 8 ? 64 : 128), Q.ychunks);
+    if (Q.MT == 8 && src.dense) {
+      WGroups sg = {};
+      sg.g[0] = one;
+      sg.G = 1;
+      sg.npairs = nc / 64;
+      hipLaunchKernelGGL(k_witness_mm8q, dim3(wgroup_grid(sg.npairs, 1), Q.ychunks), dim3(512), 0, c->stream, sspfrag, sg, nrowsel, Q.kpc, nc, d_part, tpoly, v0, wc);
+    } else if (Q.MT == 8)
+      hipLaunchKernelGGL(k_witness_mm8q_prg, grid, dim3(512), 0, c->stream, d_rk, one.bitfrag, nrowsel, Q.kpc, nc, d_part, wc);
+    else
+      with_mt(Q.MT, [&](auto mt) {
+        constexpr int M = decltype(mt)::value;
+        if (src.dense) hipLaunchKernelGGL(k_witness_mm<M>, grid, dim3(256), 0, c->stream, sspfrag, one.bitfrag, nrowsel, Q.kpc, nc, d_part, wc);
+        else hipLaunchKernelGGL(k_witness_mm_prg<M>, grid, dim3(256), 0, c->stream, d_rk, one.bitfrag, nrowsel, Q.kpc, nc, d_part, wc);
+      });
+    hipLaunchKernelGGL(k_witness_mm_finish, dim3((nc + 255) / 256, counts[g]), dim3(256), 0, c->stream, d_part, Q.ychunks, tpoly, one.cnt_delta, counts[g], 32 * Q.MT, nc,
+                       one.w_out, (uint64_t)w_stride, v0, one.v_out);
+  }
+  HIP_TRY(c, hipGetLastError());
+  return MFH_OK;
+}
+
 }
 
 extern "C" {
@@ -697,61 +825,21 @@
 int mfh_witness_poly_mm_cols(mfh_ctx *c, const uint32_t *d_ssp, uint32_t nstmt, const uint8_t *h_bits, size_t bits_stride, const uint32_t *h_delta,
                              uint32_t col0, uint32_t ncols, uint32_t *d_w, size_t w_stride) {
   if (!witness_args_ok(c, nstmt, 256, h_bits, h_delta, d_w)) return MFH_EINVAL;
-  mf::SspSrc src;
-  if (int rc = ssp_src(c, d_ssp, src)) return rc;
-  const uint32_t d = c->P.d, m = c->P.m, nc = ncols;
-  if (d % 128 || m < 2) { c->err = "mfh_witness_poly_mm: d must be a multiple of 128"; return MFH_EUNSUPPORTED; }
-  if ((uint64_t)col0 + ncols > d || w_stride < ncols) return MFH_EINVAL;
-  if (ncols == 0) return MFH_OK;
-  if (col0 % 128 || ncols % 128) { c->err = "mfh_witness_poly_mm_cols: the coefficient range must start and end at multiples of 128"; return MFH_EUNSUPPORTED; }
-  if (int rc = witness_deltas(c, nstmt, h_delta)) return rc;
-  HIP_TRY(c, hipSetDevice(c->device));
-  const MmPlan P(c, src.dense != nullptr, nstmt, bits_stride, nc);
-  const WCols wc = {col0 / 32, P.ksteps, (uint64_t)w_stride};
-  const uint32_t *tpoly = src.t + col0;
-  const size_t sfrag_b = (size_t)P.ksteps * 32 * d * 4;
-  if (src.dense && (c->ssp_frag_src != d_ssp || c->ssp_frag.cap < sfrag_b)) {
-    if (int rc = dev_reserve(c, c->ssp_frag, sfrag_b)) return rc;
-    hipLaunchKernelGGL(k_ssp_frag, dim3(P.ksteps * (d / 32)), dim3(256), 0, c->stream, d_ssp, P.nrowsel, d, c->ssp_frag.as<uint32_t>());
-    HIP_TRY(c, hipGetLastError());
-    c->ssp_frag_src = d_ssp;
-  }
-  if (int rc = P.ws.reserve(c)) return rc;
-  const size_t head_b = P.ws.bytes(MmPlan::HEAD);
-  PinBuf &wpin = c->pin_wring[c->pin_wnext++ % 8];
-  uint8_t *stage = (uint8_t *)pin_acquire(c, wpin, head_b);
-  if (!stage) return MFH_ENOMEM;
-  memcpy(stage, h_bits, P.packed);
-  uint32_t *cd = (uint32_t *)(stage + P.cd_off);
-  for (uint32_t b = 0; b < nstmt; b++) {
-    cd[2 * b] = witness_count(h_bits + (size_t)b * bits_stride, m);
-    cd[2 * b + 1] = h_delta[b];
-  }
-  uint8_t *dev = P.ws.at<uint8_t>(c, MmPlan::HEAD);
-  HIP_TRY(c, hipMemcpyAsync(dev, stage, head_b, hipMemcpyHostToDevice, c->stream));
-  pin_release(c, wpin);
-  const uint32_t *d_cd = (const uint32_t *)(dev + P.cd_off), *d_rk = P.ws.at<uint32_t>(c, MmPlan::ROWKEYS);
-  const v4i *bitfrag = P.ws.at<v4i>(c, MmPlan::BITFRAG), *sspfrag = c->ssp_frag.as<const v4i>();
-  int *d_part = P.ws.at<int>(c, MmPlan::PART);
-  hipLaunchKernelGGL(k_witness_bits, dim3((P.ksteps * P.MT * 64 + 255) / 256), dim3(256), 0, c->stream, dev, bits_stride, nstmt, P.nrowsel, P.ksteps, P.MT, (int8_t *)bitfrag);
-  if (!src.dense) hipLaunchKernelGGL(k_prg_rowkeys, dim3((P.ksteps * 32 + 255) / 256), dim3(256), 0, c->stream, src.seed, P.ksteps * 32, (uint32_t *)d_rk);
-  const dim3 grid(nc / (P.MT == 8 ? 64 : 128), P.ychunks);
-  if (P.MT == 8 && src.dense)
-    hipLaunchKernelGGL(k_witness_mm8q, grid, dim3(512), 0, c->stream, sspfrag, bitfrag, P.nrowsel, P.kpc, nc, P.fused ? (int *)nullptr : d_part, tpoly, d_cd, nstmt,
-                       d_w, wc);
-  else if (P.MT == 8)
-    hipLaunchKernelGGL(k_witness_mm8q_prg, grid, dim3(512), 0, c->stream, d_rk, bitfrag, P.nrowsel, P.kpc, nc, d_part, wc);
-  else
-    with_mt(P.MT, [&](auto mt) {
-      constexpr int M = decltype(mt)::value;
-      if (src.dense) hipLaunchKernelGGL(k_witness_mm<M>, grid, dim3(256), 0, c->stream, sspfrag, bitfrag, P.nrowsel, P.kpc, nc, d_part, wc);
-      else hipLaunchKernelGGL(k_witness_mm_prg<M>, grid, dim3(256), 0, c->stream, d_rk, bitfrag, P.nrowsel, P.kpc, nc, d_part, wc);
-    });
-  if (!P.fused)
-    hipLaunchKernelGGL(k_witness_mm_finish, dim3((nc + 255) / 256, nstmt), dim3(256), 0, c->stream, d_part, P.ychunks, tpoly, d_cd, nstmt, 32 * P.MT, nc, d_w,
-                       (uint64_t)w_stride);
-  HIP_TRY(c, hipGetLastError());
-  return MFH_OK;
+  return witness_mm_groups(c, d_ssp, 1, &nstmt, h_bits, bits_stride, h_delta, &d_w, nullptr, col0, ncols, w_stride);
+}
+
+int mfh_witness_poly_mm_groups(mfh_ctx *c, const uint32_t *d_ssp, uint32_t ngroups, const uint32_t *counts, const uint8_t *h_bits, size_t bits_stride,
+                               const uint32_t *h_delta, uint32_t *const *d_w, uint32_t *const *d_v) {
+  if (!c || !counts || !d_w || !h_bits || !h_delta || !ngroups || ngroups > 8) return MFH_EINVAL;
+  for (uint32_t g = 0; g < ngroups; g++)
+    if (!witness_args_ok(c, counts[g], 256, h_bits, h_delta, d_w[g])) return MFH_EINVAL;
+  if (ssp_is_rows(c, d_ssp)) {
+    if (d_v) { c->err = "mfh_witness_poly_mm_groups: V is written for a dense SSP only"; return MFH_EUNSUPPORTED; }
+    for (uint32_t g = 0, s0 = 0; g < ngroups; s0 += counts[g++])
+      if (int rc = ssp_rows_witness(c, counts[g], h_bits + (size_t)s0 * bits_stride, bits_stride, h_delta + s0, d_w[g], c->P.d)) return rc;
+    return MFH_OK;
+  }
+  return witness_mm_groups(c, d_ssp, ngroups, counts, h_bits, bits_stride, h_delta, d_w, d_v, 0, c->P.d, c->P.d);
 }
 
 int mfh_witness_poly_mm(mfh_ctx *c, const uint32_t *d_ssp, uint32_t nstmt, const uint8_t *h_bits, size_t bits_stride, const uint32_t *h_delta, uint32_t *d_w) {
diff --git a/include/mfhip.h b/include/mfhip.h
--- a/include/mfhip.h
+++ b/include/mfhip.h
@@ -167,6 +167,7 @@
 int mfh_set_witness_per(mfh_ctx *ctx, uint32_t statements);
 int mfh_set_batch_launch(mfh_ctx *ctx, uint32_t groups_per_launch, int merge_regions);
 int mfh_set_batch_bw(mfh_ctx *ctx, int merged);
+int mfh_set_batch_chain(mfh_ctx *ctx, int mode);
 int mfh_set_mm_stream(mfh_ctx *ctx, int map, int persistent, int sync_mode, uint32_t spin_max);
 int mfh_set_mm_width(mfh_ctx *ctx, uint32_t per_xcd, int early_chain);
 int mfh_set_mm_chunk_rows(mfh_ctx *ctx, uint32_t rows);
@@ -196,6 +197,8 @@
                            uint32_t *d_w);
 int mfh_witness_poly_mm(mfh_ctx *ctx, const uint32_t *d_ssp, uint32_t nstmt, const uint8_t *h_bits, size_t bits_stride, const uint32_t *h_delta,
                         uint32_t *d_w);
+int mfh_witness_poly_mm_groups(mfh_ctx *ctx, const uint32_t *d_ssp, uint32_t ngroups, const uint32_t *counts, const uint8_t *h_bits, size_t bits_stride,
+                               const uint32_t *h_delta, uint32_t *const *d_w, uint32_t *const *d_v);
 int mfh_witness_poly_mm_cols(mfh_ctx *ctx, const uint32_t *d_ssp, uint32_t nstmt, const uint8_t *h_bits, size_t bits_stride, const uint32_t *h_delta,
                              uint32_t col0, uint32_t ncols, uint32_t *d_w, size_t w_stride);
 int mfh_witness_lanes(mfh_ctx *ctx, const uint32_t *d_ssp, const uint8_t *h_witness_bits, uint32_t rank, uint32_t world, uint64_t *d_lanes);
```

Measured after the change: 13570 (median of 5 runs). No clear change (+0.4%).
